# wolny/pytorch-3dunet

Measured on AMD Instinct MI355X. Metric: volumetric patches/sec (fwd+bwd), UNet3D f_maps=32 patch 64x128x128, higher is better.
Workload: dtype f32

## Files before the change

### include/u3d.h

```cpp
#ifndef U3D_H
#define U3D_H

#include <stddef.h>
#include <stdint.h>

#ifdef __cplusplus
extern "C" {
#endif

#define U3D_VERSION 128

#define U3D_OK 0
#define U3D_EINVAL (-1)
#define U3D_EHIP (-2)
#define U3D_EARCH (-3)
#define U3D_EWORKSPACE (-4)

typedef void* u3d_stream_t;

typedef struct {
    const float* p0;
    const float* p1;
    const int32_t* zmap;
    const int32_t* ymap;
// ... 6 lines not shown
int u3d_version(void);
const char* u3d_last_error(void);
int u3d_check_device(int device);
int u3d_set_tuning(int key, int value);
int u3d_set_profile_buffer(void* device_buffer, size_t bytes);
int u3d_debug_stream_pass(int device, u3d_stream_t stream, float* buf, long long n, int blocks, int passes, double min_seconds);
int u3d_debug_mfma_f32_rate(int device, u3d_stream_t stream, float* sink, int iters, int mode, double* flop_out);

size_t u3d_packed_weight_floats(int Cin, int Cout, int mode);
int u3d_pack_weights(int device, u3d_stream_t stream, const float* w, int Cout, int Cin, int mode, float* packed);
typedef struct {
    const float* w;
    float* packed;
    int64_t first;
    int32_t Cout, Cin, mode, cin_stride;
} u3d_pack_desc_t;
int u3d_pack_weights_batch(int device, u3d_stream_t stream, const u3d_pack_desc_t* descs_device, int n,
                           int64_t total_floats);
long long u3d_pack_weights_cells_blocks(const float* w, int Cin, int Cout, int mode, int cin_stride);
int u3d_pack_weights_batch_cells(int device, u3d_stream_t stream, const u3d_pack_desc_t* descs_device, int n, long long total_blocks);

int u3d_conv3d(int device, u3d_stream_t stream, const u3d_src_t* src, const float* packed_w, float* out,
               int N, int D, int H, int W, int Cout, int relu, double* out_stats, const u3d_src_t* gx,
               double* gstats);

int u3d_conv3d_residual(int device, u3d_stream_t stream, const u3d_src_t* src, const float* packed_w, float* out,
                        int N, int D, int H, int W, int Cout, int relu, double* out_stats, const float* residual);

long long u3d_conv3d_workspace_floats(int N, int D, int H, int W, int Cin, int Cout);
int u3d_conv3d_ex(int device, u3d_stream_t stream, const u3d_src_t* src, const float* packed_w, float* out, int N,
                  int D, int H, int W, int Cout, int relu, double* out_stats, const u3d_src_t* gx, double* gstats,
                  const float* residual, float* workspace, long long workspace_floats);

int u3d_conv3d_ex_reps(int device, u3d_stream_t stream, const u3d_src_t* src, const float* packed_w, float* out, int N,
                       int D, int H, int W, int Cout, int relu, double* out_stats, const u3d_src_t* gx, double* gstats,
                       const float* residual, float* workspace, long long workspace_floats, int stat_reps);

long long u3d_subpixel_packed_floats(int C1, int Cout);
long long u3d_subpixel_dgrad_packed_floats(int Cout, int C1);
int u3d_pack_subpixel_dgrad_weights(int device, u3d_stream_t stream, const float* w, int Cout, int Cin_total, int c_off,
                                    int C1, float* packed);
int u3d_subpixel_conv_dgrad(int device, u3d_stream_t stream, const float* dz, const float* packed, const float* x_low,
                            float* dlow, double* gstats, int N, int D1, int H1, int W1, int C1, int Cout);
int u3d_subpixel_conv_dgrad_reps(int device, u3d_stream_t stream, const float* dz, const float* packed, const float* x_low, float* dlow,
                                 double* gstats, int N, int D1, int H1, int W1, int C1, int Cout, int reps);
int u3d_pack_subpixel_weights(int device, u3d_stream_t stream, const float* w, int Cout, int Cin_total, int c_off, int C1,
                              float* packed);
long long u3d_subpixel_fwd_workspace_floats(int N, int D1, int H1, int W1, int C1, int Cout);
int u3d_subpixel_conv_fwd(int device, u3d_stream_t stream, const float* low, const float* affine,
                          long long affine_sample_stride, const float* packed, float* out, int N, int D1, int H1, int W1,
                          int C1, int Cout, float* workspace, long long workspace_floats);

size_t u3d_wgrad_workspace_floats(int N, int D, int H, int W, int Cin, int Cout);
int u3d_conv3d_wgrad(int device, u3d_stream_t stream, const u3d_src_t* src, const float* dz, float* dw, int N,
                     int D, int H, int W, int Cout, float* workspace, size_t workspace_floats);

int u3d_conv3d_variant(int N, int D, int H, int W, int Cin, int Cout, int src_kind, int has_workspace);
int u3d_conv3d_wgrad_variant(int N, int D, int H, int W, int Cin, int Cout, int src_kind);

int u3d_conv3d_wgrad_strided(int device, u3d_stream_t stream, const u3d_src_t* src, const float* dz, float* dw,
                             int dw_cin_stride, int N, int D, int H, int W, int Cout, float* workspace,
                             size_t workspace_floats);

typedef struct u3d_gn_bwd_job {
    const double* gstats_lo;
    const double* gstats_hi;
    const float* mean_rstd;
    const float* gamma;
    float* dgamma;
    float* dbeta;
    float* coef;
    float* coef_hi;
    double count;
    int32_t C0, C1, N, G;
    float hi_scale;
    int32_t reps_lo;
    int32_t reps_hi;
    int32_t reserved;
} u3d_gn_bwd_job_t;
int u3d_conv3d_wgrad_job_supported(int N, int C, int G);
int u3d_conv3d_wgrad_job(int device, u3d_stream_t stream, const u3d_src_t* src, const float* dz, float* dw, int dw_cin_stride,
                         int N, int D, int H, int W, int Cout, float* workspace, size_t workspace_floats,
                         const u3d_gn_bwd_job_t* job);

long long u3d_subpixel_wgrad_workspace_floats(int N, int D1, int H1, int W1, int C1, int Cout);
int u3d_subpixel_conv_wgrad(int device, u3d_stream_t stream, const float* low, const float* affine,
                            long long affine_sample_stride, const float* dz, float* dw, int dw_cin_stride, int N, int D1,
                            int H1, int W1, int C1, int Cout, float* workspace, long long workspace_floats);

int u3d_subpixel_conv_fwd_win(int device, u3d_stream_t stream, const float* low, const float* affine, long long affine_sample_stride,
                              const float* packed, float* out, int N, int D1, int H1, int W1, int C1, int Cout, const int* win);
int u3d_subpixel_conv_dgrad_win(int device, u3d_stream_t stream, const float* dz, const float* packed, const float* x_low, float* dlow,
                                double* gstats, int N, int D1, int H1, int W1, int C1, int Cout, const int* win);
int u3d_subpixel_conv_wgrad_win(int device, u3d_stream_t stream, const float* low, const float* affine, long long affine_sample_stride,
                                const float* dz, float* dw, int dw_cin_stride, int N, int D1, int H1, int W1, int C1, int Cout,
                                float* workspace, long long workspace_floats, const int* win);
int u3d_conv3d_box(int device, u3d_stream_t stream, const u3d_src_t* src, const float* packed_w, float* out, int N, int D, int H, int W,
                   int Cout, const int* out_box, const int* in_mask);
int u3d_conv3d_wgrad_box(int device, u3d_stream_t stream, const u3d_src_t* src, const float* dz, float* dw, int N, int D, int H, int W,
                         int Cout, float* workspace, size_t workspace_floats, const int* box);
int u3d_gn_bwd_apply_children(int device, u3d_stream_t stream, const float* dlow, const float* x, const float* coef, int Ctot, int coff,
                              int N, int D1, int H1, int W1, int C, int ez, int ey, int ex, int relu_mask, float* out);
int u3d_chan_stats_children(int device, u3d_stream_t stream, const float* x_low, int N, int D1, int H1, int W1, int C, int ez, int ey,
                            int ex, double* stats);
int u3d_nearest_childsum_add(int device, u3d_stream_t stream, const float* dv, const float* x_low, float* dlow, double* gstats, int N,
                             int D, int H, int W, int D1, int H1, int W1, int C, const int32_t* zlo, const int32_t* ylo,
                             const int32_t* xlo, int cz, int cy, int cx);

int u3d_conv3d_small_cin_fwd(int device, u3d_stream_t stream, const float* x, const float* affine, const float* w,
                             float* out, int N, int D, int H, int W, int Cin, int Cout, int relu, double* out_stats);
int u3d_conv3d_small_cin_fwd_reps(int device, u3d_stream_t stream, const float* x, const float* affine, const float* w, float* out, int N,
                                  int D, int H, int W, int Cin, int Cout, int relu, double* out_stats, int reps);
size_t u3d_small_cin_bwd_workspace_floats(int N, int D, int H, int W, int Cin, int Cout);
int u3d_conv3d_small_cin_bwd(int device, u3d_stream_t stream, const float* x, const float* affine, const float* dz,
                             const float* w, float* dw, double* gstats, int N, int D, int H, int W, int Cin, int Cout,
                             float* workspace, size_t workspace_floats);

int u3d_conv3d_naive(int device, u3d_stream_t stream, const u3d_src_t* src, const float* w, float* out, int N,
                     int D, int H, int W, int Cin, int Cout, int relu, int flip);

int u3d_chan_stats(int device, u3d_stream_t stream, const u3d_src_t* src, int N, int D, int H, int W,
                   double* stats);
int u3d_chan_stats_reps(int device, u3d_stream_t stream, const u3d_src_t* src, int N, int D, int H, int W, double* stats, int reps);
int u3d_gn_finalize(int device, u3d_stream_t stream, const double* stats0, int C0, double scale0,
                    const double* stats1, int C1, double scale1, int N, int G, double count, const float* gamma,
                    const float* beta, float eps, float* affine, float* mean_rstd);

int u3d_gn_bwd_finalize(int device, u3d_stream_t stream, const double* gstats, const float* mean_rstd,
                        const float* gamma, int N, int C, int G, double count, float* dgamma, float* dbeta,
                        float* coef);
int u3d_gn_finalize_split(int device, u3d_stream_t stream, const double* stats0, int C0, double scale0, const double* stats1, int C1,
                          double scale1, int N, int G, double count, const float* gamma, const float* beta, float eps, float* affine,
                          float* mean_rstd, int Csplit, float* affine_lo, float* affine_hi);
int u3d_gn_finalize_reps(int device, u3d_stream_t stream, const double* stats0, int C0, double scale0, int reps0, const double* stats1,
                         int C1, double scale1, int reps1, int N, int G, double count, const float* gamma, const float* beta, float eps,
                         float* affine, float* mean_rstd, int Csplit, float* affine_lo, float* affine_hi);
int u3d_gn_bwd_finalize_split_supported(int N, int C, int G);
int u3d_gn_bwd_finalize_split(int device, u3d_stream_t stream, const double* gstats_lo, int C0, const double* gstats_hi, int C1,
                              const float* mean_rstd, const float* gamma, int N, int G, double count, float* dgamma, float* dbeta,
                              float* coef, float hi_scale, float* coef_hi);

int u3d_gn_bwd_apply(int device, u3d_stream_t stream, const float* dg, int Cdg, int coff, const float* x, int Cx,
                     const float* coef, int Ctot, int64_t voxels_per_n, int N, int relu_mask, float* out);

int u3d_gn_bwd_apply_add(int device, u3d_stream_t stream, const float* dg, int Cdg, int coff, const float* x, int Cx,
                         const float* coef, int Ctot, int64_t voxels_per_n, int N, int relu_mask, const float* add,
                         float* out);

int u3d_gn_bwd_apply_up(int device, u3d_stream_t stream, const float* dg, int Cdg, int coff, const float* x1,
                        int C1, const float* coef, int Ctot, int N, int D, int H, int W, int D1, int H1, int W1,
                        const int32_t* zlo, const int32_t* ylo, const int32_t* xlo, int relu_mask, float* out);

int u3d_maxpool2_fwd(int device, u3d_stream_t stream, const float* x, int N, int D, int H, int W, int C,
                     float* out, uint8_t* argmax, double* out_stats);
int u3d_maxpool2_bwd_merge(int device, u3d_stream_t stream, const float* dg, const float* pooled,
                           const uint8_t* argmax, const float* coef, const float* skip_grad, const float* e,
                           int N, int D, int H, int W, int C, int relu_mask, float* out);
int u3d_maxpool2_bwd_merge_gn(int device, u3d_stream_t stream, const float* dg, const float* pooled,
                              const uint8_t* argmax, const float* coef, const float* skip_dg, int Cdg,
                              const float* skip_coef, int Ctot, const float* e, int N, int D, int H, int W, int C,
                              int relu_mask, float* out);

int u3d_conv1x1_head_fwd(int device, u3d_stream_t stream, const float* x, const float* w, const float* b, int N,
                         int64_t V, int Cin, int Cout, int act, float* logits, float* probs);
int u3d_conv1x1_head_bwd(int device, u3d_stream_t stream, const float* dlogits, const float* x, const float* w,
                         int N, int64_t V, int Cin, int Cout, int relu_mask, float* dx, double* acc);
// ... 316 lines not shown
```

### pytorch-3dunet_amd/csrc/u3d_bf16.hip

```cpp
#include "u3d_common.h"
#include "u3d_gn.h"
#include <type_traits>

typedef __bf16 bf16x8 __attribute__((ext_vector_type(8)));
typedef __bf16 bf16x4 __attribute__((ext_vector_type(4)));
typedef __bf16 bf16x2 __attribute__((ext_vector_type(2)));
typedef float f32x2 __attribute__((ext_vector_type(2)));
typedef unsigned u32x4 __attribute__((ext_vector_type(4)));
typedef unsigned u32x2 __attribute__((ext_vector_type(2)));

__device__ __forceinline__ bf16x8 u3d_stage_b16(const bf16x8& v, bool has_aff, bool ok, const f32x4& a0, const f32x4& b0, const f32x4& a1,
                                                const f32x4& b1) {
    const u32x4 raw = __builtin_bit_cast(u32x4, v);
    u32x4 o = raw;
    if (has_aff) {
#pragma unroll
        for (int e = 0; e < 4; ++e) {
            const f32x2 x = {__builtin_bit_cast(float, raw[e] << 16), __builtin_bit_cast(float, raw[e] & 0xffff0000u)};
            const f32x2 a = e < 2 ? f32x2{a0[2 * e], a0[2 * e + 1]} : f32x2{a1[2 * e - 4], a1[2 * e - 3]};
            const f32x2 b = e < 2 ? f32x2{b0[2 * e], b0[2 * e + 1]} : f32x2{b1[2 * e - 4], b1[2 * e - 3]};
            o[e] = __builtin_bit_cast(unsigned, __builtin_convertvector(__builtin_elementwise_fma(x, a, b), bf16x2));
        }
    }
    const unsigned m = ok ? 0xffffffffu : 0u;
    return __builtin_bit_cast(bf16x8, u32x4{o[0] & m, o[1] & m, o[2] & m, o[3] & m});
}

extern int g_u3d_tune[24];

namespace {

constexpr int HS = 12;

struct bf16_conv_params {
    const float* x;
    const float* affine;
    const bf16x8* wpk;
    float* y;
    const float* residual;
    const float* gx;
    double* out_stats;
    double* gstats;
    int N, D, H, W, C, K, relu;
    int tz, ty, tx;
    int off;
    const float* maskx;
    int ksplit;
    float* ws;
    long long wpart;
    int order;
    int b16;
    int t8mode, t8cs;
};

template <int ZW, int KS>
struct tile_geom {
    static constexpr bool FLAT = ZW == 3;
    static constexpr int TZ = FLAT ? 5 : 4 * ZW, TY = FLAT ? 10 : 8, TX = FLAT ? 10 : 8;
    static constexpr int HZ = TZ + KS - 1, HY = TY + KS - 1, HX = TX + KS - 1, MT = FLAT ? 4 : 2 * ZW;
    static_assert(HX <= HS, "halo rows are HS records long");
    static constexpr int NTAPS = KS * KS * KS;
    static constexpr int RING = KS == 3 ? 9 : 8;
    static constexpr int BDIST = 6;
    static constexpr int ADIST = 2;
    static constexpr int PLANE = HZ * HY * HS * 16 + 64;
    static constexpr int BUF = 2 * PLANE;
    static constexpr int ITEMS = HZ * HY * HX * 4;
    static constexpr int ITERS = (ITEMS + 255) / 256;
    static constexpr int NPARTS = KS * KS;
    static constexpr int PER_PART = (ITERS + NPARTS - 1) / NPARTS;
    static constexpr int ITEMS8 = HZ * HY * HX * 2;
    static constexpr int ITERS8 = (ITEMS8 + 255) / 256;
    static constexpr int PER_PART8 = (ITERS8 + NPARTS - 1) / NPARTS;
};

template <int NT, int ZW, int KS, typename T = float>
__device__ __forceinline__ void conv_tile_epilogue(const bf16_conv_params& p, f32x16 (&acc)[tile_geom<ZW, KS>::MT][NT], char* lds, int n, int nb,
                                                   int split, int z0, int y0, int x0, int t, int lane, int w) {
    using G = tile_geom<ZW, KS>;
    const int col = lane & 31, half = lane >> 5;
    if (p.ksplit > 1) {
        float* wsp = p.ws + (size_t)split * p.N * p.D * p.H * p.W * p.K;
        if constexpr (std::is_same<T, __bf16>::value) {
#pragma unroll
            for (int m = 0; m < G::MT; ++m) {
                int z, y, xx;
                bool row_ok = true;
                if constexpr (G::FLAT) {
                    const int v = (w * G::MT + m) * 32 + col, vz = v / (G::TY * G::TX), vr = v - vz * (G::TY * G::TX), vy = vr / G::TX;
                    z = z0 + vz, y = y0 + vy, xx = x0 + vr - vy * G::TX;
                    row_ok = v < G::TZ * G::TY * G::TX;
                } else {
                    z = z0 + w * ZW + (m >> 1), y = y0 + (m & 1) * 4 + (col & 3), xx = x0 + (col >> 2);
                }
                if (row_ok && z < p.D && y < p.H && xx < p.W) {
                    const size_t vox = (((size_t)n * p.D + z) * p.H + y) * p.W + xx;
#pragma unroll
                    for (int j = 0; j < NT; ++j)
#pragma unroll
                        for (int g = 0; g < 4; ++g)
                            *reinterpret_cast<f32x4*>(wsp + vox * p.K + (size_t)(nb * NT + j) * 32 + 8 * g + 4 * half) =
                                f32x4{acc[m][j][4 * g], acc[m][j][4 * g + 1], acc[m][j][4 * g + 2], acc[m][j][4 * g + 3]};
                }
            }
            return;
        }
        if constexpr (G::FLAT) return;
#pragma unroll
        for (int m = 0; m < G::MT; ++m) {
            const int z = z0 + w * ZW + (m >> 1);
#pragma unroll
// ... 2730 lines not shown
```

### pytorch-3dunet_amd/csrc/u3d_conv.hip

```cpp
#include <type_traits>
#include <utility>

#include "u3d_common.h"
#include "u3d_gn.h"
#include "u3d_subpix.h"

int g_u3d_tune[24] = {0};

namespace cv {
constexpr int TZ = 4, TY = 8, TX = 8;
constexpr int HZ = TZ + 2, HY = TY + 2, HX = TX + 2;
constexpr int CC = 16;
constexpr int CS = 16;
constexpr int RS = HX * CS + 4;
constexpr int PS = HY * RS;
constexpr int TILE_FLOATS = HZ * PS + 4;
constexpr int CNT_OFF = 2 * TILE_FLOATS;
constexpr int RED_OFF = CNT_OFF + 16;
constexpr int LDS_FLOATS = RED_OFF + 4 * 3 * 32 * 2;
constexpr int NITEMS = HZ * HY * HX * (CC / 4);
constexpr int NIT = (NITEMS + 255) / 256;
constexpr int NSTEP = 27 * (CC / 8);
constexpr int NSTEP_PAIRY = 36 * (CC / 8);
constexpr int NSTEP_N16 = 27;
constexpr int ST0 = 30;
constexpr int ISTORE = 5;
constexpr int PACK_PAD = 5;
static_assert(2 * (NIT - 1) < ST0 - 8 && ST0 + NIT <= NSTEP, "prefetch schedule must fit the k-loop");
}

struct ConvParams {
    u3d_src_t src;
    u3d_src_t gx;
    const float* wp;
    float* out;
    double* out_stats;
    double* gstats;
    const float* res;
    int N, D, H, W, Cout;
    int nchunks, ncb, ntot;
    int tz, ty, tx;
    int relu, vec, has_gx, ovec;
    int total;
    int gx_x2;
    int stagger;
    int stat_reps;
    int zfast;
    int ksplit, cps;
    long long part_stride;
    long long* dbg;
    int oz0, oy0, ox0, oz1, oy1, ox1;
    int mz, my, mx;
};

#define U3D_DBG_STAMP(slot)                                                   \
    do {                                                                      \
        if constexpr (DBG) {                                                  \
            if (l == 0) dbgw[slot] = (long long)__builtin_readcyclecounter(); \
        }                                                                     \
    } while (0)

__device__ __forceinline__ void u3d_flag_signal(int* c, int lane) {
    asm volatile("" ::: "memory");
    if (lane == 0) __hip_atomic_fetch_add(c, 1, __ATOMIC_RELAXED, __HIP_MEMORY_SCOPE_WORKGROUP);
    asm volatile("" ::: "memory");
}
__device__ __forceinline__ void u3d_flag_wait(int* c, int target) {
    while (__hip_atomic_load(c, __ATOMIC_RELAXED, __HIP_MEMORY_SCOPE_WORKGROUP) < target) __builtin_amdgcn_s_sleep(2);
    asm volatile("" ::: "memory");
}

template <int NT, bool VEC, bool DBG = false, int ABL = 0>
__global__ __launch_bounds__(256, 2) void conv3d_mfma_kernel(const ConvParams p) {
    using namespace cv;
    constexpr int RB = NT == 1 ? 6 : 3;
    extern __shared__ __attribute__((aligned(16))) float lds[];
    int* cnt = reinterpret_cast<int*>(lds + CNT_OFF);
    const int t = threadIdx.x;
    const int l = t & 63, w = t >> 6, m = l & 31, h = l >> 5;
    __builtin_amdgcn_s_setprio(3);
    long long* dbgw = nullptr;
    if constexpr (DBG) {
        dbgw = p.dbg + ((size_t)blockIdx.x * 4 + w) * 24;
        if (l == 0) {
            dbgw[0] = blockIdx.x;
            dbgw[1] = __builtin_amdgcn_s_getreg((31 << 11) | 4);
            dbgw[2] = __builtin_amdgcn_s_getreg((31 << 11) | 20);
            dbgw[7] = p.nchunks;
        }
    }
// ... 958 lines not shown
#pragma unroll
                            for (int e = 0; e < 4; ++e) val[e] = cok ? val[e] : 0.f;
                        }
                        q1 += val;
                        q2 += want_g ? val * xv[k] : val * val;
                    }
                }
                if (want_stats || want_g) {
                    if constexpr (CARRY) {
                        sq1 += q1;
                        sq2 += q2;
                    } else {
                        stat_reduce(q1, q2, n, nt, co - (PAIRY ? 0 : (cb * NT + nt) * 32));
                    }
                }
            }
        }
        if (ntiles == DBG_TILE) U3D_DBG_STAMP(22);
        ++ntiles;
        if (!has_next_tile || TN.n != T.n || TN.cb != T.cb) {
            if constexpr (CARRY) {
                if (want_stats || want_g) {
                    if constexpr (N16) {
#pragma unroll
                        for (int e = 0; e < 4; ++e) {
                            float a = sq1[e], b2 = sq2[e];
#pragma unroll
                            for (int msk = 8; msk > 0; msk >>= 1) {
                                a += __shfl_xor(a, msk);
                                b2 += __shfl_xor(b2, msk);
                            }
                            if (v16 == 0) {
                                double* r = &red[(((T.n & 1) * NT) * 32 + 4 * kq + e) * 2];
                                __hip_atomic_fetch_add(r, (double)a, __ATOMIC_RELAXED, __HIP_MEMORY_SCOPE_WORKGROUP);
                                __hip_atomic_fetch_add(r + 1, (double)b2, __ATOMIC_RELAXED, __HIP_MEMORY_SCOPE_WORKGROUP);
                            }
                        }
                    } else {
                        const int cq_ = (l >> 2) & 7;
                        stat_reduce(sq1, sq2, T.n, 0, PAIRY ? 4 * (cq_ & 3) : 4 * cq_);
                    }
                    sq1 = f32x4{0.f, 0.f, 0.f, 0.f};
                    sq2 = f32x4{0.f, 0.f, 0.f, 0.f};
                }
            }
            flush_stats(T.n, T.cb);
        }
        if (!has_next_tile) break;
        if constexpr (!ZEROC) {
#pragma unroll
            for (int mt = 0; mt < MT; ++mt)
#pragma unroll
                for (int nt = 0; nt < NT; ++nt)
#pragma unroll
                    for (int r = 0; r < 16; ++r) acc[mt][nt][r] = 0.f;
        }
        wi = nwi;
        dT = dTN;
        T = TN;
        wq = wqn;
    }
    if constexpr (DBG) {
        if (l == 0) dbgw[4] = ntiles;
    }
    U3D_DBG_STAMP(6);
}

namespace wg {
constexpr int TZ = 2, TY = 8, TX = 8;
constexpr int HZ = TZ + 2, HY = TY + 2, HX = TX + 2;
constexpr int CC = 32;
constexpr int CSg = 32, RSg = HX * CSg, PSg = HY * RSg;
constexpr int G_FLOATS = HZ * PSg;
constexpr int TV = TZ * TY * TX;
constexpr int DZ_FLOATS = TV * 32;
constexpr int DUMMY_OFF = G_FLOATS + DZ_FLOATS;
constexpr int BUF_FLOATS = G_FLOATS + DZ_FLOATS + 4;
constexpr int LDS_FLOATS = 2 * BUF_FLOATS;
constexpr int NTHR = 512;
constexpr int NITEMS_G = HZ * HY * HX * (CC / 4);
constexpr int NIT_G = (NITEMS_G + NTHR - 1) / NTHR;
constexpr int NIT_DZ = TV * 8 / NTHR;
constexpr int MAX_MAP_INTS = 4096;
}

struct WgradParams {
    u3d_src_t src;
    const float* dz;
    float* partial;
    int N, D, H, W, Cout;
    int nchunks, nkb, S;
    int tz, ty, tx, ntiles, tps;
    int vec, dzvec;
    int bz0, by0, bx0, bz1, by1, bx1;
};

template <bool VEC, bool REG = false, bool PAIR = false>
__global__ __launch_bounds__(512, 2) void conv3d_wgrad_kernel(const WgradParams p) {
    using namespace wg;
    constexpr int NA = PAIR ? 4 : 7;
    extern __shared__ __attribute__((aligned(16))) float lds[];
    int* zmapl = reinterpret_cast<int*>(lds + 2 * BUF_FLOATS);
    __builtin_amdgcn_s_setprio(3);
    const int t = threadIdx.x;
    const int l = t & 63, i = l & 31, h = l >> 5;
    const int w = __builtin_amdgcn_readfirstlane(t >> 6);
    const int tg = w & 3, hf = w >> 2;

    const int logical = u3d_xcd_remap(blockIdx.x, gridDim.x);
    const int kb = logical % p.nkb;
    const int chunk = (logical / p.nkb) % p.nchunks;
    const int s = logical / (p.nkb * p.nchunks);
    const int D = p.D, H = p.H, W = p.W;
    const int Ctot = p.src.C0 + p.src.C1;
    int* ymapl = zmapl + D;
    int* xmapl = ymapl + H;
    if (p.src.C1 > 0) {
        for (int k = t; k < D; k += NTHR) zmapl[k] = p.src.zmap[k];
        for (int k = t; k < H; k += NTHR) ymapl[k] = p.src.ymap[k];
        for (int k = t; k < W; k += NTHR) xmapl[k] = p.src.xmap[k];
        __syncthreads();
    }

    f32x16 acc[NA];
#pragma unroll
    for (int k = 0; k < NA; ++k)
#pragma unroll
        for (int r = 0; r < 16; ++r) acc[k][r] = 0.f;

    const int q = t & 7, tv = t >> 3;
    const int cq = chunk * CC + 4 * q;
    const int co = kb * 32 + 4 * q;
    const bool cok = cq < Ctot, from0 = cq < p.src.C0, dcok = co < p.Cout;
    const float* gbase = !cok ? p.src.p0 : (from0 ? p.src.p0 + cq : p.src.p1 + (cq - p.src.C0));
    const int Cs = (from0 || !cok) ? p.src.C0 : p.src.C1;
    const float* dzbase = p.dz + (dcok ? co : 0);

    constexpr int NPFC = NIT_G + NIT_DZ;
    int rel[NPFC], loff[NPFC];
    unsigned fz0 = 0, fz1 = 0, fy0 = 0, fy1 = 0, fx0 = 0, fx1 = 0, fdead = 0;
    if constexpr (REG) {
        const int vz = D % TZ ? D % TZ : TZ, vy = H % TY ? H % TY : TY, vx = W % TX ? W % TX : TX;
#pragma unroll
        for (int it = 0; it < NIT_G; ++it) {
            const int vox = tv + 64 * it;
            const int hz = vox / (HY * HX);
            const int rem = vox - hz * (HY * HX);
            const int hy = rem / HX;
            const int hx = rem - hy * HX;
            const bool in = vox < HZ * HY * HX;
            rel[it] = from0 ? ((hz - 1) * H + (hy - 1)) * W + (hx - 1)
                            : (((hz - 1) >> 1) * p.src.H1 + ((hy - 1) >> 1)) * p.src.W1 + ((hx - 1) >> 1);
            loff[it] = in ? hz * PSg + hy * RSg + hx * CSg + 4 * q : DUMMY_OFF;
            fz0 |= (in && hz == 0 ? 1u : 0u) << it;
            fz1 |= (in && hz > vz ? 1u : 0u) << it;
            fy0 |= (in && hy == 0 ? 1u : 0u) << it;
            fy1 |= (in && hy > vy ? 1u : 0u) << it;
            fx0 |= (in && hx == 0 ? 1u : 0u) << it;
            fx1 |= (in && hx > vx ? 1u : 0u) << it;
            fdead |= (in && cok ? 0u : 1u) << it;
        }
#pragma unroll
        for (int it = 0; it < NIT_DZ; ++it) {
            const int vox = tv + 64 * it;
            rel[NIT_G + it] = ((vox >> 6) * H + ((vox >> 3) & 7)) * W + (vox & 7);
            loff[NIT_G + it] = G_FLOATS + vox * 32 + 4 * q;
            fz1 |= ((vox >> 6) >= vz ? 1u : 0u) << (NIT_G + it);
            fy1 |= (((vox >> 3) & 7) >= vy ? 1u : 0u) << (NIT_G + it);
            fx1 |= ((vox & 7) >= vx ? 1u : 0u) << (NIT_G + it);
        }
        fdead |= (dcok ? 0u : 3u) << NIT_G;
    }
    auto tile_invalid = [&](int z0, int y0, int x0) {
        unsigned inv = fdead;
        inv |= z0 == 0 ? fz0 : 0u;
        inv |= z0 + TZ >= D ? fz1 : 0u;
        inv |= y0 == 0 ? fy0 : 0u;
        inv |= y0 + TY >= H ? fy1 : 0u;
        inv |= x0 == 0 ? fx0 : 0u;
        inv |= x0 + TX >= W ? fx1 : 0u;
        return inv;
    };
// ... 76 lines not shown
            const float* ap = p.src.affine + ((size_t)n * Ctot + (cok ? cq : 0)) * 2;
            const f32x4 lo = *reinterpret_cast<const f32x4*>(ap);
            const f32x4 hi = *reinterpret_cast<const f32x4*>(ap + 4);
            ga = f32x4{lo[0], lo[2], hi[0], hi[2]};
            gb = f32x4{lo[1], lo[3], hi[1], hi[3]};
        }
    };
    auto pf_load = [&](const TileC& c, int k) {
        bool ok;
        int idx, off;
        if constexpr (REG) {
            ok = ((c.inv >> k) & 1u) == 0;
            if (k < NIT_G) return *reinterpret_cast<const f32x4*>(gbase + (size_t)(ok ? c.base + rel[k] : 0) * Cs);
            return *reinterpret_cast<const f32x4*>(dzbase + (size_t)(ok ? c.dzb + rel[k] : 0) * p.Cout);
        }
        if (k < NIT_G) {
            g_item(c, k, off, ok, idx);
            return *reinterpret_cast<const f32x4*>(gbase + (size_t)idx * Cs);
        }
        dz_item(c, k - NIT_G, ok, idx);
        return *reinterpret_cast<const f32x4*>(dzbase + (size_t)idx * p.Cout);
    };
    auto pf_store = [&](float* buf, const TileC& c, int k, f32x4 raw, const f32x4& ga, const f32x4& gb) {
        bool ok;
        int idx, off;
        if constexpr (REG) {
            ok = ((c.inv >> k) & 1u) == 0;
            f32x4 val = k < NIT_G ? raw * ga + gb : raw;
#pragma unroll
            for (int e = 0; e < 4; ++e) val[e] = ok ? val[e] : 0.f;
            *reinterpret_cast<f32x4*>(&buf[loff[k]]) = val;
            return;
        }
        if (k < NIT_G) {
            g_item(c, k, off, ok, idx);
            f32x4 val = raw * ga + gb;
#pragma unroll
            for (int e = 0; e < 4; ++e) val[e] = ok ? val[e] : 0.f;
            *reinterpret_cast<f32x4*>(&buf[off]) = val;
        } else {
            dz_item(c, k - NIT_G, ok, idx);
#pragma unroll
            for (int e = 0; e < 4; ++e) raw[e] = ok ? raw[e] : 0.f;
            *reinterpret_cast<f32x4*>(&buf[G_FLOATS + (tv + 64 * (k - NIT_G)) * 32 + 4 * q]) = raw;
        }
    };
    auto stage_scalar = [&](float* buf, const TileC& c) {
        f32x4 ga, gb;
        u3d_load_affine(p.src.affine, c.n, Ctot, cq, false, ga, gb);
#pragma unroll 1
        for (int it = 0; it < NIT_G; ++it) {
            const int vox = tv + 64 * it;
            if (vox >= HZ * HY * HX) continue;
            const int hz = vox / (HY * HX), rem = vox - hz * (HY * HX), hy = rem / HX, hx = rem - hy * HX;
            const int gz = c.z0 - 1 + hz, gy = c.y0 - 1 + hy, gxx = c.x0 - 1 + hx;
            f32x4 val = {0.f, 0.f, 0.f, 0.f};
            if (gz >= 0 && gz < D && gy >= 0 && gy < H && gxx >= 0 && gxx < W) {
                int v0, v1;
                u3d_vox_index(p.src, c.n, gz, gy, gxx, D, H, W, v0, v1);
                val = u3d_load_quad(p.src, v0, v1, cq, false) * ga + gb;
            }
            *reinterpret_cast<f32x4*>(&buf[hz * PSg + hy * RSg + hx * CSg + 4 * q]) = val;
        }
#pragma unroll 1
        for (int it = 0; it < NIT_DZ; ++it) {
            const int vox = tv + 64 * it;
            const int z = c.z0 + (vox >> 6), y = c.y0 + ((vox >> 3) & 7), x = c.x0 + (vox & 7);
            f32x4 val = {0.f, 0.f, 0.f, 0.f};
            if (z < p.bz1 && y < p.by1 && x < p.bx1) {
                const float* sp = p.dz + ((size_t)((c.n * D + z) * H + y) * W + x) * p.Cout + co;
#pragma unroll
                for (int e = 0; e < 4; ++e)
                    if (co + e < p.Cout) val[e] = sp[e];
            }
            *reinterpret_cast<f32x4*>(&buf[G_FLOATS + vox * 32 + 4 * q]) = val;
        }
    };

    constexpr int NPF = NIT_G + NIT_DZ;
    constexpr int ST0 = 20;
    static_assert(2 * (NPF - 1) < ST0 && ST0 + NPF <= 32, "prefetch schedule must fit the 32 groups of a tile");
    const int tile_begin = s * p.tps, tile_end = min(p.ntiles, (s + 1) * p.tps);

    TileIdx tix = tile_decode(tile_begin);
    if (tile_begin < tile_end) {
        const TileC c = tile_coords(tix);
        if constexpr (VEC) {
            f32x4 ga, gb;
            load_affine(c.n, ga, gb);
            f32x4 v[NPF];
#pragma unroll
            for (int k = 0; k < NPF; ++k) v[k] = pf_load(c, k);
#pragma unroll
            for (int k = 0; k < NPF; ++k) pf_store(lds, c, k, v[k], ga, gb);
        } else {
            stage_scalar(lds, c);
        }
    }
    __syncthreads();

    int abase[NA];
#pragma unroll
    for (int k = 0; k < NA; ++k) {
        const int tap = PAIR ? 2 * (tg + 4 * k) + (i >> 4) : tg + 4 * k;
        const int toff = tap < 27 ? (tap / 9) * PSg + ((tap / 3) % 3) * RSg + (tap % 3) * CSg : 0;
        abase[k] = (PAIR ? (i & 15) : i) + h * CSg + hf * PSg + toff;
    }
    int bbase = G_FLOATS + (hf * 64 + h) * 32 + i;
    int cur = 0;
    __builtin_amdgcn_s_setprio(0);

    f32x4 gan = {1.f, 1.f, 1.f, 1.f}, gbn = {0.f, 0.f, 0.f, 0.f};
    int n_aff = -1;
    for (int tile = tile_begin; tile < tile_end; ++tile) {
        const bool has_next = tile + 1 < tile_end;
        if (has_next) tix = tile_next(tix);
        const TileC cn = tile_coords(tix);
        float* nbuf = lds + (cur ^ 1) * BUF_FLOATS;
        f32x4 v[NPF];
        if constexpr (VEC) {
            if (cn.n != n_aff) {
                load_affine(cn.n, gan, gbn);
                n_aff = cn.n;
            }
        }
        const float* gl = lds + cur * BUF_FLOATS;

        float aop[2][NA], bop[2];
        bop[0] = gl[bbase];
#pragma unroll
        for (int k = 0; k < NA; ++k) aop[0][k] = gl[abase[k]];
#pragma unroll
        for (int g = 0; g < 32; ++g) {
            if constexpr (VEC) {
                if (g % 2 == 0 && g / 2 < NPF) v[g / 2] = pf_load(cn, g / 2);
                if (g >= ST0 && g - ST0 < NPF) pf_store(nbuf, cn, g - ST0, v[g - ST0], gan, gbn);
            }
            if (g + 1 < 32) {
                const int row = (g + 1) >> 2, tq = (g + 1) & 3;
                const int goff = row * RSg + 2 * tq * CSg;
                bop[(g + 1) & 1] = gl[bbase + (row * 8 + 2 * tq) * 32];
#pragma unroll
                for (int k = 0; k < NA; ++k) aop[(g + 1) & 1][k] = gl[abase[k] + goff];
            }
            __builtin_amdgcn_sched_barrier(0);
#pragma unroll
            for (int k = 0; k < NA; ++k) acc[k] = __builtin_amdgcn_mfma_f32_32x32x2f32(aop[g & 1][k], bop[g & 1], acc[k], 0, 0, 0);
            __builtin_amdgcn_sched_barrier(0);
        }
        if constexpr (!VEC) {
            if (has_next) stage_scalar(nbuf, cn);
        }
        __syncthreads();
        cur ^= 1;
    }

    __builtin_amdgcn_s_setprio(3);
    float* red = lds;
    if (hf == 1) {
#pragma unroll
        for (int k = 0; k < NA; ++k)
#pragma unroll
            for (int r = 0; r < 16; ++r) red[((tg * 7 + k) * 16 + r) * 64 + l] = acc[k][r];
    }
    __syncthreads();
    if (hf == 0) {
        float* dst = p.partial + ((size_t)((s * p.nchunks + chunk) * p.nkb + kb) * 27) * 1024;
#pragma unroll
        for (int k = 0; k < NA; ++k) {
#pragma unroll
            for (int r = 0; r < 16; ++r) {
                const int row = (r & 3) + 8 * (r >> 2) + 4 * h;
                const int tap = PAIR ? 2 * (tg + 4 * k) + (row >> 4) : tg + 4 * k;
                const int c = PAIR ? (row & 15) : row;
                if (tap < 27) dst[((size_t)tap * 32 + c) * 32 + i] = acc[k][r] + red[((tg * 7 + k) * 16 + r) * 64 + l];
            }
        }
    }
}

template <int G>
__global__ __launch_bounds__(256) void wgrad_reduce_kernel(const float* __restrict__ partial, float* __restrict__ dw,
                                                           int S, int nchunks, int nkb, int Cin, int Cout, int cstride,
                                                           int has_job, u3d_gn_bwd_job_t job) {
    __shared__ float red[4][64];
    if (has_job && blockIdx.x == 0) {
        extern __shared__ double shb[];
        u3d_gn_bwd_finalize_body(job.gstats_lo, job.mean_rstd, job.gamma, job.N, job.C0 + job.C1, job.G, job.count, 1, 1, job.dgamma,
                                 job.dbeta, job.coef, job.gstats_hi, job.C0, job.hi_scale, job.coef_hi, shb, job.reps_lo, job.reps_hi);
        return;
    }
    const long long total = (long long)Cin * 27 * Cout;
    const int lane = G == 1 ? (int)threadIdx.x : (int)(threadIdx.x & 63), grp = G == 1 ? 0 : (int)(threadIdx.x >> 6);
    const long long idx = (long long)(blockIdx.x - (has_job ? 1 : 0)) * (G == 1 ? 256 : 64) + lane;
    float sum = 0.f;
    int k = 0, tap = 0, c = 0;
    if (idx < total) {
        k = (int)(idx % Cout);
        const long long r = idx / Cout;
        tap = (int)(r % 27);
        c = (int)(r / 27);
        const int chunk = c >> 5, kb = k >> 5;
        const size_t off = ((size_t)(chunk * nkb + kb) * 27 + tap) * 1024 + (c & 31) * 32 + (k & 31);
        const size_t sstride = (size_t)nchunks * nkb * 27 * 1024;
        const int per = (S + G - 1) / G;
        const int s0 = grp * per, s1 = min(S, s0 + per);
        float a0 = 0.f, a1 = 0.f, a2 = 0.f, a3 = 0.f;
        int s = s0;
        for (; s + 3 < s1; s += 4) {
            a0 += partial[(size_t)s * sstride + off];
            a1 += partial[(size_t)(s + 1) * sstride + off];
            a2 += partial[(size_t)(s + 2) * sstride + off];
            a3 += partial[(size_t)(s + 3) * sstride + off];
        }
        for (; s < s1; ++s) a0 += partial[(size_t)s * sstride + off];
        sum = (a0 + a1) + (a2 + a3);
    }
    if constexpr (G == 1) {
        if (idx < total) dw[((size_t)k * cstride + c) * 27 + tap] = sum;
    } else {
        red[grp][lane] = sum;
        __syncthreads();
        if (grp == 0 && idx < total)
            dw[((size_t)k * cstride + c) * 27 + tap] = (red[0][lane] + red[1][lane]) + (red[2][lane] + red[3][lane]);
    }
}

__device__ __forceinline__ int pack_image_of(long long idx, int nchunks, int ntot, long long& id) {
    const long long std_total = ((long long)nchunks * cv::NSTEP + cv::PACK_PAD) * ntot * 256;
    const long long pair_total = ((long long)nchunks * cv::NSTEP_PAIRY + cv::PACK_PAD) * 256;
    if (idx < std_total) {
        id = idx;
        return 0;
    }
    if (idx < std_total + pair_total) {
        id = idx - std_total;
        return 1;
    }
    id = idx - std_total - pair_total;
    return 2;
// ... 257 lines not shown
            const int f = fq * (sp::NFRAG / PK_SUBQ) + (i >> 6), lane = i & 63;
            const int st = sp::frag_tab().st[f];
            const int kl = 8 * (st & 1) + 4 * (lane >> 5), nl = lane & 31;
            f32x4 v;
#pragma unroll
            for (int j = 0; j < 4; ++j) v[j] = sp::frag_value(row_of(nl, kl + j), f);
            out4[(((long long)ch * sp::NFRAG + f) * ntot + ntg) * 64 + lane] = v;
        }
    } else {
        for (int i = t; i < spd::NFRAG / PK_SUBQ * 64; i += 256) {
            const int f = fq * (spd::NFRAG / PK_SUBQ) + (i >> 6), lane = i & 63;
            const int kl = 8 * (f & 1) + 4 * (lane >> 5), nl = lane & 31;
            f32x4 v;
#pragma unroll
            for (int j = 0; j < 4; ++j) v[j] = spd::frag_value(row_of(nl, kl + j), f);
            out4[(((long long)ch * spd::NFRAG + f) * ntot + ntg) * 64 + lane] = v;
        }
    }
}

__global__ void conv3d_naive_kernel(const u3d_src_t src, const float* __restrict__ w, float* __restrict__ out,
                                    int N, int D, int H, int W, int Cin, int Cout, int relu, int flip) {
    const long long total = (long long)N * D * H * W * Cout;
    for (long long idx = (long long)blockIdx.x * blockDim.x + threadIdx.x; idx < total;
         idx += (long long)gridDim.x * blockDim.x) {
        const int co = (int)(idx % Cout);
        long long v = idx / Cout;
        const int x = (int)(v % W);
        v /= W;
        const int y = (int)(v % H);
        v /= H;
        const int z = (int)(v % D);
        const int n = (int)(v / D);
        float sum = 0.f;
        for (int tap = 0; tap < 27; ++tap) {
            const int zz = z + tap / 9 - 1, yy = y + (tap / 3) % 3 - 1, xx = x + tap % 3 - 1;
            if (zz < 0 || zz >= D || yy < 0 || yy >= H || xx < 0 || xx >= W) continue;
            int v0, v1;
            u3d_vox_index(src, n, zz, yy, xx, D, H, W, v0, v1);
            for (int c = 0; c < Cin; ++c) {
                float g = u3d_load_elem(src, v0, v1, c);
                if (src.affine) {
                    const float* ab = src.affine + ((size_t)n * Cin + c) * 2;
                    g = g * ab[0] + ab[1];
                }
                const float wt = flip ? w[((size_t)c * Cout + co) * 27 + (26 - tap)] : w[((size_t)co * Cin + c) * 27 + tap];
                sum += g * wt;
            }
        }
        if (relu) sum = fmaxf(sum, 0.f);
        out[idx] = sum;
    }
}

static inline int cdiv(int a, int b) { return (a + b - 1) / b; }

static bool src_vec_ok(const u3d_src_t* s) {
    if (s->C0 % 4 != 0 || s->C1 % 4 != 0) return false;
    if (((uintptr_t)s->p0 & 15) != 0) return false;
    if (s->C1 > 0 && ((uintptr_t)s->p1 & 15) != 0) return false;
    if (s->affine && ((uintptr_t)s->affine & 15) != 0) return false;
    return true;
}

static int check_src(const u3d_src_t* s, const char* what) {
    U3D_REQUIRE(s != nullptr && s->p0 != nullptr && (s->C0 > 0 || s->C1 > 0) && s->C0 >= 0, "%s: null source", what);
    U3D_REQUIRE(s->C1 >= 0, "%s: negative C1", what);
    if (s->C1 > 0)
        U3D_REQUIRE(s->p1 && s->zmap && s->ymap && s->xmap && s->D1 > 0 && s->H1 > 0 && s->W1 > 0,
                    "%s: low-res source needs p1, index maps and dims", what);
    return 0;
}

static long long* g_u3d_prof_buf = nullptr;
static size_t g_u3d_prof_records = 0;

extern "C" int u3d_set_profile_buffer(void* device_buffer, size_t bytes) {
    g_u3d_prof_buf = static_cast<long long*>(device_buffer);
    g_u3d_prof_records = device_buffer ? bytes / (24 * sizeof(long long)) : 0;
    return 0;
}

extern "C" int u3d_set_tuning(int key, int value) {
    if (key < 0 || key >= 24) return u3d_set_err(U3D_EINVAL, "u3d_set_tuning: key out of range");
    g_u3d_tune[key] = value;
    return 0;
}

extern "C" size_t u3d_packed_weight_floats(int Cin, int Cout, int mode) {
    return (size_t)pack_total_floats(Cin, Cout, mode, nullptr, nullptr);
}

extern "C" int u3d_pack_weights(int device, u3d_stream_t stream, const float* w, int Cout, int Cin, int mode,
                                float* packed) {
    U3D_ENTER(device);
    U3D_REQUIRE(w && packed && Cout > 0 && Cin > 0 && (mode == 0 || mode == 1), "u3d_pack_weights: bad argument");
    int nchunks = 0, ntot = 0;
    const long long total = pack_total_floats(Cin, Cout, mode, &nchunks, &ntot);
    const int blocks = (int)((total + 255) / 256 > 4096 ? 4096 : (total + 255) / 256);
    hipLaunchKernelGGL(pack_weights_kernel, dim3(blocks), dim3(256), 0, (hipStream_t)stream, w, packed, Cout, Cin,
                       mode, nchunks, ntot, total);
    U3D_LAUNCH_CHECK();
    return 0;
}

extern "C" int u3d_pack_weights_batch(int device, u3d_stream_t stream, const u3d_pack_desc_t* descs_device, int n,
                                      int64_t total_floats) {
    U3D_ENTER(device);
    U3D_REQUIRE(descs_device && n > 0 && total_floats > 0, "u3d_pack_weights_batch: bad argument");
    U3D_REQUIRE(total_floats % 4 == 0, "u3d_pack_weights_batch: image sizes are multiples of 4 floats");
    long long blocks = (total_floats / 4 + 255) / 256;
    if (blocks > 8192) blocks = 8192;
    hipLaunchKernelGGL(pack_weights_batch_kernel, dim3((unsigned)blocks), dim3(256), 0, (hipStream_t)stream, descs_device, n,
                       (long long)total_floats);
    U3D_LAUNCH_CHECK();
    return 0;
}

extern "C" long long u3d_pack_weights_cells_blocks(const float* w, int Cin, int Cout, int mode, int cin_stride) {
    const int cs = cin_stride > 0 ? cin_stride : Cin;
    if (Cin <= 0 || Cout <= 0 || mode < 0 || mode > 3 || Cin % 4 != 0 || Cout % 4 != 0 || cs % 4 != 0 || ((uintptr_t)w & 15) != 0) return 0;
    return pack_cells_of(Cin, Cout, mode) + 1;
}

extern "C" int u3d_pack_weights_batch_cells(int device, u3d_stream_t stream, const u3d_pack_desc_t* descs_device, int n,
                                            long long total_blocks) {
    U3D_ENTER(device);
    U3D_REQUIRE(descs_device && n > 0 && total_blocks > 0 && total_blocks < 0x7fffffffLL, "u3d_pack_weights_batch_cells: bad argument");
    hipLaunchKernelGGL(pack_weights_cells_kernel, dim3((unsigned)total_blocks), dim3(256), 0, (hipStream_t)stream, descs_device, n);
    U3D_LAUNCH_CHECK();
    return 0;
}

static int device_cu_count(int device, int* out) {
    static int cached[64] = {0};
    if (device >= 0 && device < 64 && cached[device] > 0) {
        *out = cached[device];
        return 0;
    }
    int n = 0;
    U3D_HIP(hipDeviceGetAttribute(&n, hipDeviceAttributeMultiprocessorCount, device));
    if (n <= 0) n = 256;
    if (device >= 0 && device < 64) cached[device] = n;
    *out = n;
    return 0;
}

template <int NT>
static int conv_set_lds_nt() {
    const int bytes = cv::LDS_FLOATS * sizeof(float);
    U3D_HIP(hipFuncSetAttribute(reinterpret_cast<const void*>(conv3d_mfma_reg_kernel<NT, false, false>),
                                hipFuncAttributeMaxDynamicSharedMemorySize, bytes));
    U3D_HIP(hipFuncSetAttribute(reinterpret_cast<const void*>(conv3d_mfma_reg_kernel<NT, true, false>),
                                hipFuncAttributeMaxDynamicSharedMemorySize, bytes));
    U3D_HIP(hipFuncSetAttribute(reinterpret_cast<const void*>(conv3d_mfma_reg_kernel<NT, false, true>),
                                hipFuncAttributeMaxDynamicSharedMemorySize, bytes));
    U3D_HIP(hipFuncSetAttribute(reinterpret_cast<const void*>(conv3d_mfma_reg_kernel<NT, true, true>),
                                hipFuncAttributeMaxDynamicSharedMemorySize, bytes));
    U3D_HIP(hipFuncSetAttribute(reinterpret_cast<const void*>(conv3d_mfma_reg_kernel<NT, false, false, false, false>),
                                hipFuncAttributeMaxDynamicSharedMemorySize, bytes));
    U3D_HIP(hipFuncSetAttribute(reinterpret_cast<const void*>(conv3d_mfma_reg_kernel<NT, true, false, false, true, false, true>),
                                hipFuncAttributeMaxDynamicSharedMemorySize, bytes));
    U3D_HIP(hipFuncSetAttribute(reinterpret_cast<const void*>(conv3d_mfma_reg_kernel<NT, false, false, false, false, false, true>),
                                hipFuncAttributeMaxDynamicSharedMemorySize, bytes));
    U3D_HIP(hipFuncSetAttribute(reinterpret_cast<const void*>(conv3d_mfma_reg_kernel<NT, false, false, false, true, false, true>),
                                hipFuncAttributeMaxDynamicSharedMemorySize, bytes));
    if (NT == 1) {
// ... 290 lines not shown
        else                                                                                               \
            hipLaunchKernelGGL((conv3d_mfma_reg_kernel<NT_, false, false>), rgrid, rblock, shmem, st, p);  \
    } while (0)
        if (nt == 3)
            U3D_REG_LAUNCH(3);
        else if (nt == 2)
            U3D_REG_LAUNCH(2);
        else
            U3D_REG_LAUNCH(1);
#undef U3D_REG_LAUNCH
        U3D_LAUNCH_CHECK();
        return 0;
    }
    const bool vec = p.vec != 0;
    const dim3 grid((unsigned)nblk), block(256);
    p.dbg = (vec && g_u3d_prof_buf && (size_t)nblk * 4 <= g_u3d_prof_records) ? g_u3d_prof_buf : nullptr;
#define U3D_CONV_LAUNCH(NT_)                                                                     \
    do {                                                                                         \
        if (p.dbg && NT_ == 1 && g_u3d_tune[2] == 1)                                             \
            hipLaunchKernelGGL((conv3d_mfma_kernel<1, true, true, 1>), grid, block, shmem, st, p); \
        else if (p.dbg && NT_ == 1 && g_u3d_tune[2] == 2)                                        \
            hipLaunchKernelGGL((conv3d_mfma_kernel<1, true, true, 2>), grid, block, shmem, st, p); \
        else if (p.dbg && NT_ == 1 && g_u3d_tune[2] == 3)                                        \
            hipLaunchKernelGGL((conv3d_mfma_kernel<1, true, true, 3>), grid, block, shmem, st, p); \
        else if (p.dbg && NT_ == 1 && g_u3d_tune[2] == 7)                                        \
            hipLaunchKernelGGL((conv3d_mfma_kernel<1, true, true, 7>), grid, block, shmem, st, p); \
        else if (p.dbg)                                                                          \
            hipLaunchKernelGGL((conv3d_mfma_kernel<NT_, true, true>), grid, block, shmem, st, p); \
        else if (vec)                                                                            \
            hipLaunchKernelGGL((conv3d_mfma_kernel<NT_, true>), grid, block, shmem, st, p);      \
        else                                                                                     \
            hipLaunchKernelGGL((conv3d_mfma_kernel<NT_, false>), grid, block, shmem, st, p);     \
    } while (0)
    if (nt == 3)
        U3D_CONV_LAUNCH(3);
    else if (nt == 2)
        U3D_CONV_LAUNCH(2);
    else
        U3D_CONV_LAUNCH(1);
#undef U3D_CONV_LAUNCH
    U3D_LAUNCH_CHECK();
    return 0;
}

static void wgrad_plan(int N, int D, int H, int W, int Cin, int Cout, WgradParams& p) {
    p.nchunks = cdiv(Cin, 32);
    p.nkb = cdiv(Cout, 32);
    p.tz = cdiv(D, wg::TZ), p.ty = cdiv(H, wg::TY), p.tx = cdiv(W, wg::TX);
    p.ntiles = N * p.tz * p.ty * p.tx;
    const int pairs = p.nchunks * p.nkb;
    const int ncu = 256;
    long long best_cost = -1;
    int best_S = 1;
    for (int rounds = 1; rounds <= 8; ++rounds) {
        int S = (rounds * ncu) / pairs;
        if (S < 1) S = 1;
        if (S > p.ntiles) S = p.ntiles;
        const int tps = cdiv(p.ntiles, S);
        S = cdiv(p.ntiles, tps);
        const long long cost = (long long)cdiv(S * pairs, ncu) * (tps + 2);
        if (best_cost < 0 || cost < best_cost) {
            best_cost = cost;
            best_S = S;
        }
    }
    if (g_u3d_tune[1] > 0) best_S = g_u3d_tune[1] > p.ntiles ? p.ntiles : g_u3d_tune[1];
    p.tps = cdiv(p.ntiles, best_S);
    p.S = cdiv(p.ntiles, p.tps);
}

extern "C" size_t u3d_wgrad_workspace_floats(int N, int D, int H, int W, int Cin, int Cout) {
    WgradParams p;
    wgrad_plan(N, D, H, W, Cin, Cout, p);
    return (size_t)p.S * p.nchunks * p.nkb * 27 * 1024;
}

static int wgrad_set_lds_once(int device) {
    static bool done[64] = {false};
    if (device >= 0 && device < 64 && done[device]) return 0;
    U3D_HIP(hipFuncSetAttribute(reinterpret_cast<const void*>(conv3d_wgrad_kernel<true, true>),
                                hipFuncAttributeMaxDynamicSharedMemorySize, (wg::LDS_FLOATS + wg::MAX_MAP_INTS) * sizeof(float)));
    U3D_HIP(hipFuncSetAttribute(reinterpret_cast<const void*>(conv3d_wgrad_kernel<true, true, true>),
                                hipFuncAttributeMaxDynamicSharedMemorySize, (wg::LDS_FLOATS + wg::MAX_MAP_INTS) * sizeof(float)));
    U3D_HIP(hipFuncSetAttribute(reinterpret_cast<const void*>(conv3d_wgrad_kernel<true>),
                                hipFuncAttributeMaxDynamicSharedMemorySize, (wg::LDS_FLOATS + wg::MAX_MAP_INTS) * sizeof(float)));
    U3D_HIP(hipFuncSetAttribute(reinterpret_cast<const void*>(conv3d_wgrad_kernel<false>),
                                hipFuncAttributeMaxDynamicSharedMemorySize, (wg::LDS_FLOATS + wg::MAX_MAP_INTS) * sizeof(float)));
    if (device >= 0 && device < 64) done[device] = true;
    return 0;
}

static int conv3d_wgrad_impl(int device, u3d_stream_t stream, const u3d_src_t* src, const float* dz, float* dw, int cstride,
                             int N, int D, int H, int W, int Cout, float* workspace, size_t workspace_floats, const int* box = nullptr,
                             const u3d_gn_bwd_job_t* job = nullptr);

extern "C" int u3d_conv3d_wgrad_box(int device, u3d_stream_t stream, const u3d_src_t* src, const float* dz, float* dw, int N, int D,
                                    int H, int W, int Cout, float* workspace, size_t workspace_floats, const int* box) {
    U3D_REQUIRE(box != nullptr, "u3d_conv3d_wgrad_box: box is NULL");
    return conv3d_wgrad_impl(device, stream, src, dz, dw, 0, N, D, H, W, Cout, workspace, workspace_floats, box);
}

extern "C" int u3d_conv3d_wgrad(int device, u3d_stream_t stream, const u3d_src_t* src, const float* dz, float* dw,
                                int N, int D, int H, int W, int Cout, float* workspace, size_t workspace_floats) {
    return conv3d_wgrad_impl(device, stream, src, dz, dw, 0, N, D, H, W, Cout, workspace, workspace_floats);
}

extern "C" int u3d_conv3d_wgrad_strided(int device, u3d_stream_t stream, const u3d_src_t* src, const float* dz, float* dw,
                                        int dw_cin_stride, int N, int D, int H, int W, int Cout, float* workspace,
                                        size_t workspace_floats) {
    U3D_REQUIRE(src && dw_cin_stride >= src->C0 + src->C1, "u3d_conv3d_wgrad_strided: dw_cin_stride < channels of src");
    return conv3d_wgrad_impl(device, stream, src, dz, dw, dw_cin_stride, N, D, H, W, Cout, workspace, workspace_floats);
}

static size_t wgrad_job_lds_bytes(int N, int C, int G) { return sizeof(double) * (4 * (size_t)N * C + 2 * (size_t)N * G); }

extern "C" int u3d_conv3d_wgrad_job_supported(int N, int C, int G) {
    return (N > 0 && C > 0 && G > 0 && C % G == 0 && wgrad_job_lds_bytes(N, C, G) + 1024 <= 64 * 1024) ? 1 : 0;
}

extern "C" int u3d_conv3d_wgrad_job(int device, u3d_stream_t stream, const u3d_src_t* src, const float* dz, float* dw,
                                    int dw_cin_stride, int N, int D, int H, int W, int Cout, float* workspace,
                                    size_t workspace_floats, const u3d_gn_bwd_job_t* job) {
    U3D_REQUIRE(src && (dw_cin_stride == 0 || dw_cin_stride >= src->C0 + src->C1), "u3d_conv3d_wgrad_job: dw_cin_stride < channels of src");
    if (job) {
        U3D_REQUIRE(job->gstats_lo && job->mean_rstd && job->gamma && job->dgamma && job->dbeta && job->coef && job->C0 > 0 &&
                        job->C1 >= 0 && (job->C1 == 0) == (job->gstats_hi == nullptr) && (job->coef_hi == nullptr || job->C1 > 0) &&
                        job->reps_lo >= 0 && job->reps_lo <= 64 && job->reps_hi >= 0 && job->reps_hi <= 64,
                    "u3d_conv3d_wgrad_job: bad job");
        U3D_REQUIRE(u3d_conv3d_wgrad_job_supported(job->N, job->C0 + job->C1, job->G) == 1,
                    "u3d_conv3d_wgrad_job: the reduction of %d x %d channels in %d groups does not fit one block's LDS", job->N,
                    job->C0 + job->C1, job->G);
    }
    return conv3d_wgrad_impl(device, stream, src, dz, dw, dw_cin_stride, N, D, H, W, Cout, workspace, workspace_floats, nullptr, job);
}

static int conv3d_wgrad_impl(int device, u3d_stream_t stream, const u3d_src_t* src, const float* dz, float* dw, int cstride,
                             int N, int D, int H, int W, int Cout, float* workspace, size_t workspace_floats, const int* box,
                             const u3d_gn_bwd_job_t* job) {
    U3D_ENTER(device);
    if (int e = check_src(src, "u3d_conv3d_wgrad")) return e;
    U3D_REQUIRE(dz && dw && workspace && N > 0 && D > 0 && H > 0 && W > 0 && Cout > 0, "u3d_conv3d_wgrad: bad argument");
    U3D_REQUIRE((long long)N * D * H * W < (1ll << 31), "u3d_conv3d_wgrad: N*D*H*W must be < 2^31");
    WgradParams p;
    const int Cin = src->C0 + src->C1;
    p.bz0 = p.by0 = p.bx0 = 0, p.bz1 = D, p.by1 = H, p.bx1 = W;
    if (box) {
        U3D_REQUIRE(box[0] >= 0 && box[1] >= 0 && box[2] >= 0 && box[3] <= D && box[4] <= H && box[5] <= W && box[0] < box[3] &&
                        box[1] < box[4] && box[2] < box[5], "u3d_conv3d_wgrad_box: box outside the volume or empty");
        p.bz0 = box[0], p.by0 = box[1], p.bx0 = box[2], p.bz1 = box[3], p.by1 = box[4], p.bx1 = box[5];
    }
    wgrad_plan(N, p.bz1 - p.bz0, p.by1 - p.by0, p.bx1 - p.bx0, Cin, Cout, p);
    const size_t need = (size_t)p.S * p.nchunks * p.nkb * 27 * 1024;
    if (workspace_floats < need)
        return u3d_set_err(U3D_EWORKSPACE, "u3d_conv3d_wgrad: workspace %zu < %zu floats", workspace_floats, need);
    p.src = *src;
    p.dz = dz;
    p.partial = workspace;
    p.N = N, p.D = D, p.H = H, p.W = W, p.Cout = Cout;
    p.vec = src_vec_ok(src) ? 1 : 0;
    p.dzvec = (Cout % 4 == 0 && ((uintptr_t)dz & 15) == 0) ? 1 : 0;
    if (int e = wgrad_set_lds_once(device)) return e;
    const int nblk = p.S * p.nchunks * p.nkb;
    U3D_REQUIRE(D + H + W <= wg::MAX_MAP_INTS, "u3d_conv3d_wgrad: D+H+W must be <= %d", wg::MAX_MAP_INTS);
    const size_t shmem = (wg::LDS_FLOATS + (size_t)(D + H + W)) * sizeof(float);
    const bool reg = !box && (g_u3d_tune[3] != 2 || (D % wg::TZ == 0 && H % wg::TY == 0 && W % wg::TX == 0)) &&
                     (src->C1 == 0 || (D == 2 * src->D1 && H == 2 * src->H1 && W == 2 * src->W1));
    if (p.vec && p.dzvec && reg && Cin <= 16)
        hipLaunchKernelGGL((conv3d_wgrad_kernel<true, true, true>), dim3(nblk), dim3(wg::NTHR), shmem, (hipStream_t)stream, p);
    else if (p.vec && p.dzvec && reg)
        hipLaunchKernelGGL((conv3d_wgrad_kernel<true, true>), dim3(nblk), dim3(wg::NTHR), shmem, (hipStream_t)stream, p);
    else if (p.vec && p.dzvec)
        hipLaunchKernelGGL(conv3d_wgrad_kernel<true>, dim3(nblk), dim3(wg::NTHR), shmem, (hipStream_t)stream, p);
    else
        hipLaunchKernelGGL(conv3d_wgrad_kernel<false>, dim3(nblk), dim3(wg::NTHR), shmem, (hipStream_t)stream, p);
    U3D_LAUNCH_CHECK();
    const long long total = (long long)Cin * 27 * Cout;
    const bool one_group = p.S <= 16 && g_u3d_tune[23] != 1;
    const int rblocks = (int)((total + (one_group ? 255 : 63)) / (one_group ? 256 : 64));
    u3d_gn_bwd_job_t jb = {};
    size_t job_lds = 0;
    if (job) {
        jb = *job;
        if (!jb.gstats_hi) jb.C1 = 0, jb.hi_scale = 1.0f, jb.coef_hi = nullptr;
        if (jb.reps_lo < 1) jb.reps_lo = 1;
        if (jb.reps_hi < 1 || !jb.gstats_hi) jb.reps_hi = 1;
        job_lds = wgrad_job_lds_bytes(jb.N, jb.C0 + jb.C1, jb.G);
    }
    if (one_group)
        hipLaunchKernelGGL(wgrad_reduce_kernel<1>, dim3(rblocks + (job ? 1 : 0)), dim3(256), job_lds, (hipStream_t)stream, workspace, dw, p.S,
                           p.nchunks, p.nkb, Cin, Cout, cstride > 0 ? cstride : Cin, job ? 1 : 0, jb);
    else
        hipLaunchKernelGGL(wgrad_reduce_kernel<4>, dim3(rblocks + (job ? 1 : 0)), dim3(256), job_lds, (hipStream_t)stream, workspace, dw, p.S,
                           p.nchunks, p.nkb, Cin, Cout, cstride > 0 ? cstride : Cin, job ? 1 : 0, jb);
    U3D_LAUNCH_CHECK();
    return 0;
}

extern "C" int u3d_conv3d_variant(int N, int D, int H, int W, int Cin, int Cout, int src_kind, int has_workspace) {
    if (N <= 0 || D <= 0 || H <= 0 || W <= 0 || Cin <= 0 || Cout <= 0) return -1;
    if (Cin % 4 != 0 || Cout % 4 != 0) return 0;
    const long long ntiles = (long long)N * cdiv(D, cv::TZ) * cdiv(H, cv::TY) * cdiv(W, cv::TX);
    const int nchunks = cdiv(Cin, 16), ntot = cdiv(Cout, 32);
    if (has_workspace && splitk_shape(N, D, H, W, Cin, Cout) && g_u3d_tune[7] != 2) {
        if (splitk_count(g_u3d_ncu_seen, ntiles, ntot, nchunks, nullptr) >= 2) return 3;
    }
    const bool ragged = D % cv::TZ != 0 || H % cv::TY != 0 || W % cv::TX != 0;
    if (src_kind == 2 || g_u3d_tune[3] == 1 || (g_u3d_tune[3] == 2 && ragged)) return 0;
    return ragged ? 2 : 1;
}

extern "C" int u3d_conv3d_wgrad_variant(int N, int D, int H, int W, int Cin, int Cout, int src_kind) {
    if (N <= 0 || D <= 0 || H <= 0 || W <= 0 || Cin <= 0 || Cout <= 0) return -1;
    if (Cin % 4 != 0 || Cout % 4 != 0) return 0;
    const bool ragged = D % wg::TZ != 0 || H % wg::TY != 0 || W % wg::TX != 0;
    if (src_kind == 2 || (g_u3d_tune[3] == 2 && ragged)) return 0;
    return (ragged ? 2 : 1) | (Cin <= 16 ? 4 : 0);
}

extern "C" int u3d_conv3d_naive(int device, u3d_stream_t stream, const u3d_src_t* src, const float* w, float* out,
                                int N, int D, int H, int W, int Cin, int Cout, int relu, int flip) {
    U3D_ENTER(device);
    if (int e = check_src(src, "u3d_conv3d_naive")) return e;
    U3D_REQUIRE(w && out && Cin == src->C0 + src->C1, "u3d_conv3d_naive: bad argument");
    const long long total = (long long)N * D * H * W * Cout;
    const int blocks = (int)((total + 255) / 256 > 65536 ? 65536 : (total + 255) / 256);
    hipLaunchKernelGGL(conv3d_naive_kernel, dim3(blocks), dim3(256), 0, (hipStream_t)stream, *src, w, out, N, D, H,
                       W, Cin, Cout, relu, flip);
    U3D_LAUNCH_CHECK();
    return 0;
}
```

### pytorch-3dunet_amd/csrc/u3d_gn.h

```cpp
#pragma once
#include "u3d_common.h"

__device__ __forceinline__ double u3d_sum_replicas(const double* __restrict__ p, size_t stride, int reps) {
    double v = p[0];
    for (int r0 = 1; r0 < reps; r0 += 8) {
        double t[8];
#pragma unroll
        for (int j = 0; j < 8; ++j) t[j] = r0 + j < reps ? p[(size_t)(r0 + j) * stride] : 0.0;
#pragma unroll
        for (int j = 0; j < 8; ++j) v += t[j];
    }
    return v;
}

__device__ inline void u3d_gn_bwd_finalize_body(const double* __restrict__ gs, const float* __restrict__ mean_rstd,
                                                const float* __restrict__ gamma, int N, int C, int G, double count, int staged, int par,
                                                float* __restrict__ dgamma, float* __restrict__ dbeta, float* __restrict__ coef,
                                                const double* __restrict__ gs_hi, int C0, float hi_scale, float* __restrict__ coef_hi,
                                                double* shb, int reps = 1, int reps_hi = 1) {

#pragma clang fp contract(off)
    const double* src = gs;
    if (staged) {
        if (gs_hi) {
            const int C1 = C - C0;
            for (int i = threadIdx.x; i < N * C * 2; i += blockDim.x) {
                const int e = i & 1, nc = i >> 1, n = nc / C, c = nc - n * C;
                shb[i] = c < C0 ? u3d_sum_replicas(gs + ((size_t)n * C0 + c) * 2 + e, (size_t)N * C0 * 2, reps)
                                : u3d_sum_replicas(gs_hi + ((size_t)n * C1 + (c - C0)) * 2 + e, (size_t)N * C1 * 2, reps_hi);
            }
        } else {
            for (int i = threadIdx.x; i < N * C * 2; i += blockDim.x) shb[i] = u3d_sum_replicas(gs + i, (size_t)N * C * 2, reps);
        }
        __syncthreads();
        src = shb;
    }
    const int cpg = C / G;
    const double m = count * cpg;
    double* pa = shb + 2 * (size_t)N * C;
    double* pb = pa + (size_t)N * C;
    double* qr = pb + (size_t)N * C;
    if (par) {
        for (int i = threadIdx.x; i < N * C; i += blockDim.x) {
            const int n = i / C, c = i - n * C, g = c / cpg;
            const double mean = (double)mean_rstd[((size_t)n * G + g) * 2], rstd = (double)mean_rstd[((size_t)n * G + g) * 2 + 1];
            const double S1 = src[(size_t)i * 2], S2 = src[(size_t)i * 2 + 1], gm = (double)gamma[c];
            pa[i] = gm * S1;
            pb[i] = gm * rstd * (S2 - mean * S1);
        }
        __syncthreads();
    }
    for (int pair = threadIdx.x; pair < N * G; pair += blockDim.x) {
        const int n = pair / G, g = pair - n * G;
        const double mean = (double)mean_rstd[(size_t)pair * 2], rstd = (double)mean_rstd[(size_t)pair * 2 + 1];
        double A = 0.0, B = 0.0;
        for (int c = g * cpg; c < (g + 1) * cpg; ++c) {
            if (par) {
                A += pa[(size_t)n * C + c];
                B += pb[(size_t)n * C + c];
            } else {
                const double S1 = src[((size_t)n * C + c) * 2], S2 = src[((size_t)n * C + c) * 2 + 1];
                const double gm = (double)gamma[c];
                A += gm * S1;
                B += gm * rstd * (S2 - mean * S1);
            }
        }
        const double q = -rstd * rstd * B / m;
        const double r = -rstd * A / m + rstd * rstd * mean * B / m;
        if (par) {
            qr[(size_t)pair * 2] = q;
            qr[(size_t)pair * 2 + 1] = r;
        } else {
            for (int c = g * cpg; c < (g + 1) * cpg; ++c) {
                coef[((size_t)n * 3 + 0) * C + c] = (float)(rstd * (double)gamma[c]);
                coef[((size_t)n * 3 + 1) * C + c] = (float)q;
                coef[((size_t)n * 3 + 2) * C + c] = (float)r;
            }
        }
    }
    if (par) {
        __syncthreads();
        for (int i = threadIdx.x; i < N * C; i += blockDim.x) {
            const int n = i / C, c = i - n * C, pair = n * G + c / cpg;
            const double rstd = (double)mean_rstd[(size_t)pair * 2 + 1];
            const float fp = (float)(rstd * (double)gamma[c]), fq = (float)qr[(size_t)pair * 2], fr = (float)qr[(size_t)pair * 2 + 1];
            coef[((size_t)n * 3 + 0) * C + c] = fp;
            coef[((size_t)n * 3 + 1) * C + c] = fq;
            coef[((size_t)n * 3 + 2) * C + c] = fr;
            if (coef_hi && c >= C0) {
                const int C1 = C - C0;
                coef_hi[((size_t)n * 3 + 0) * C1 + (c - C0)] = fp;
                coef_hi[((size_t)n * 3 + 1) * C1 + (c - C0)] = fq * hi_scale;
                coef_hi[((size_t)n * 3 + 2) * C1 + (c - C0)] = fr * hi_scale;
            }
        }
    }
    for (int c = threadIdx.x; c < C; c += blockDim.x) {
        const int g = c / cpg;
        double dg = 0.0, db = 0.0;
        for (int n = 0; n < N; ++n) {
            const double mean = (double)mean_rstd[((size_t)n * G + g) * 2], rstd = (double)mean_rstd[((size_t)n * G + g) * 2 + 1];
            const double S1 = src[((size_t)n * C + c) * 2], S2 = src[((size_t)n * C + c) * 2 + 1];
            dg += rstd * (S2 - mean * S1);
            db += S1;
        }
        dgamma[c] = (float)dg;
        dbeta[c] = (float)db;
    }
}
```

### pytorch-3dunet_amd/csrc/u3d_ops.hip

```cpp
#include "u3d_common.h"
#include "u3d_gn.h"

#include <string.h>

extern int g_u3d_tune[24];

static thread_local char g_err[512] = "";

int u3d_set_err(int code, const char* fmt, ...) {
    va_list ap;
    va_start(ap, fmt);
    vsnprintf(g_err, sizeof(g_err), fmt, ap);
    va_end(ap);
    return code;
}

int u3d_device_guard::enter(int device) {
    hipError_t e = hipGetDevice(&prev);
    if (e != hipSuccess) return u3d_set_err(U3D_EHIP, "hipGetDevice failed: %s", hipGetErrorString(e));
    if (device >= 0 && prev != device) {
        e = hipSetDevice(device);
        if (e != hipSuccess) return u3d_set_err(U3D_EHIP, "hipSetDevice(%d) failed: %s", device, hipGetErrorString(e));
        switched = true;
    }
    return 0;
}

extern "C" int u3d_version(void) { return U3D_VERSION; }
extern "C" const char* u3d_last_error(void) { return g_err; }

extern "C" int u3d_check_device(int device) {
    hipDeviceProp_t prop;
    U3D_HIP(hipGetDeviceProperties(&prop, device));
    if (strncmp(prop.gcnArchName, "gfx950", 6) != 0)
        return u3d_set_err(U3D_EARCH, "device %d is %s, this library is built for gfx950 only", device, prop.gcnArchName);
    return 0;
}

__global__ __launch_bounds__(256) void debug_stream_pass_kernel(float* __restrict__ buf, long long n4, int passes, float one,
                                                               long long ticks_total) {
    f32x4* b = reinterpret_cast<f32x4*>(buf);
    constexpr long long PIECE = 4096;
    const long long npieces = (n4 + PIECE - 1) / PIECE;
    const long long mine = (npieces - blockIdx.x + gridDim.x - 1) / gridDim.x;
    const long long t0 = wall_clock64();
    long long done = 0;
    for (int p = 0; p < passes; ++p)
        for (long long pc = blockIdx.x; pc < npieces; pc += gridDim.x) {
            const long long lo = pc * PIECE, hi = lo + PIECE < n4 ? lo + PIECE : n4;
            for (long long i = lo + threadIdx.x; i < hi; i += 256) {
                f32x4 v = b[i];
                v *= one;
                b[i] = v;
            }
            ++done;
            if (ticks_total > 0) {
                const long long due = t0 + ticks_total * done / (mine * passes);
                while (wall_clock64() < due) __builtin_amdgcn_s_sleep(64);
            }
        }
}

extern "C" int u3d_debug_stream_pass(int device, u3d_stream_t stream, float* buf, long long n, int blocks, int passes,
                                     double min_seconds) {
    U3D_ENTER(device);
    U3D_REQUIRE(buf && n >= 4 && blocks > 0 && passes > 0 && min_seconds >= 0.0 && ((uintptr_t)buf & 15) == 0,
                "u3d_debug_stream_pass: bad argument");
    int khz = 0;
    U3D_HIP(hipDeviceGetAttribute(&khz, hipDeviceAttributeWallClockRate, device));
    const long long ticks = (long long)(min_seconds * 1e3 * (double)khz);
    hipLaunchKernelGGL(debug_stream_pass_kernel, dim3((unsigned)blocks), dim3(256), 0, (hipStream_t)stream, buf, n / 4, passes, 1.0f,
                       ticks);
    U3D_LAUNCH_CHECK();
    return 0;
}

__device__ __forceinline__ float dbg_hash_unit(unsigned x) {
    float s = 0.f;
    for (int i = 0; i < 4; ++i) {
        x ^= x >> 16, x *= 0x7feb352dU, x ^= x >> 15, x *= 0x846ca68bU, x ^= x >> 16;
        s += (float)(x & 0xffffff) * (1.0f / 16777216.0f);
    }
    return (s - 2.0f) * 1.7320508f;
}
__global__ __launch_bounds__(256) void debug_mfma_rate_kernel(float* __restrict__ sink, int iters, int mode) {
    f32x16 acc[2];
    for (int k = 0; k < 2; ++k)
        for (int r = 0; r < 16; ++r) acc[k][r] = 0.f;
// ... 324 lines not shown
}

extern "C" int u3d_gn_finalize_split(int device, u3d_stream_t stream, const double* stats0, int C0, double scale0,
                                     const double* stats1, int C1, double scale1, int N, int G, double count,
                                     const float* gamma, const float* beta, float eps, float* affine, float* mean_rstd,
                                     int Csplit, float* affine_lo, float* affine_hi) {
    return gn_finalize_impl(device, stream, stats0, C0, scale0, stats1, C1, scale1, N, G, count, gamma, beta, eps, affine, mean_rstd,
                            affine_lo, affine_hi, Csplit);
}

extern "C" int u3d_gn_finalize_reps(int device, u3d_stream_t stream, const double* stats0, int C0, double scale0, int reps0,
                                    const double* stats1, int C1, double scale1, int reps1, int N, int G, double count,
                                    const float* gamma, const float* beta, float eps, float* affine, float* mean_rstd,
                                    int Csplit, float* affine_lo, float* affine_hi) {
    return gn_finalize_impl(device, stream, stats0, C0, scale0, stats1, C1, scale1, N, G, count, gamma, beta, eps, affine, mean_rstd,
                            affine_lo, affine_hi, Csplit, reps0, reps1);
}

__global__ __launch_bounds__(256) void gn_bwd_finalize_kernel(const double* __restrict__ gs, const float* __restrict__ mean_rstd,
                                                              const float* __restrict__ gamma, int N, int C, int G,
                                                              double count, int staged, int par, float* __restrict__ dgamma,
                                                              float* __restrict__ dbeta, float* __restrict__ coef,
                                                              const double* __restrict__ gs_hi, int C0, float hi_scale,
                                                              float* __restrict__ coef_hi) {
    extern __shared__ double shb[];
    u3d_gn_bwd_finalize_body(gs, mean_rstd, gamma, N, C, G, count, staged, par, dgamma, dbeta, coef, gs_hi, C0, hi_scale, coef_hi, shb);
}

extern "C" int u3d_gn_bwd_finalize(int device, u3d_stream_t stream, const double* gstats, const float* mean_rstd,
                                   const float* gamma, int N, int C, int G, double count, float* dgamma,
                                   float* dbeta, float* coef) {
    U3D_ENTER(device);
    U3D_REQUIRE(gstats && mean_rstd && gamma && dgamma && dbeta && coef && N > 0 && C > 0 && G > 0 && C % G == 0,
                "u3d_gn_bwd_finalize: bad argument");
    const size_t bytes = sizeof(double) * 2 * (size_t)N * C;
    const int staged = bytes <= 48 * 1024 ? 1 : 0;
    const size_t par_bytes = 2 * bytes + sizeof(double) * 2 * (size_t)N * G;
    const int par = staged && par_bytes <= 64 * 1024 ? 1 : 0;
    hipLaunchKernelGGL(gn_bwd_finalize_kernel, dim3(1), dim3(256), par ? par_bytes : (staged ? bytes : 0), (hipStream_t)stream, gstats,
                       mean_rstd, gamma, N, C, G, count, staged, par, dgamma, dbeta, coef, (const double*)nullptr, C, 1.0f, (float*)nullptr);
    U3D_LAUNCH_CHECK();
    return 0;
}

extern "C" int u3d_gn_bwd_finalize_split_supported(int N, int C, int G) {
    const size_t bytes = sizeof(double) * 2 * (size_t)N * C;
    return (N > 0 && C > 0 && G > 0 && 2 * bytes + sizeof(double) * 2 * (size_t)N * G <= 64 * 1024) ? 1 : 0;
}

extern "C" int u3d_gn_bwd_finalize_split(int device, u3d_stream_t stream, const double* gstats_lo, int C0, const double* gstats_hi,
                                         int C1, const float* mean_rstd, const float* gamma, int N, int G, double count,
                                         float* dgamma, float* dbeta, float* coef, float hi_scale, float* coef_hi) {
    U3D_ENTER(device);
    const int C = C0 + C1;
    U3D_REQUIRE(gstats_lo && gstats_hi && mean_rstd && gamma && dgamma && dbeta && coef && N > 0 && C0 > 0 && C1 > 0 && G > 0 &&
                    C % G == 0, "u3d_gn_bwd_finalize_split: bad argument");
    U3D_REQUIRE(u3d_gn_bwd_finalize_split_supported(N, C, G) == 1, "u3d_gn_bwd_finalize_split: N * C = %d exceeds the staged path", N * C);
    const size_t bytes = sizeof(double) * 2 * (size_t)N * C;
    const size_t par_bytes = 2 * bytes + sizeof(double) * 2 * (size_t)N * G;
    hipLaunchKernelGGL(gn_bwd_finalize_kernel, dim3(1), dim3(256), par_bytes, (hipStream_t)stream, gstats_lo, mean_rstd, gamma, N, C, G,
                       count, 1, 1, dgamma, dbeta, coef, gstats_hi, C0, hi_scale, coef_hi);
    U3D_LAUNCH_CHECK();
    return 0;
}

template <bool VEC, typename T = float>
__global__ void gn_bwd_apply_kernel(const T* __restrict__ dg, int Cdg, int coff, const T* __restrict__ x,
                                    int Cx, const float* __restrict__ coef, int Ctot, long long Vn, int N,
                                    int relu_mask, const T* __restrict__ add, T* __restrict__ out) {
    if (VEC) {
        const int Q = Cx >> 2;
        const long long total = (long long)N * Vn * Q;
        for (long long idx = (long long)blockIdx.x * blockDim.x + threadIdx.x; idx < total;
             idx += (long long)gridDim.x * blockDim.x) {
            const int qd = (int)(idx % Q);
            const long long v = idx / Q;
            const int n = (int)(v / Vn);
            const int c = 4 * qd;
            const f32x4 d = u3d_ldq(dg + (size_t)v * Cdg + coff + c);
            const f32x4 xv = u3d_ldq(x + (size_t)v * Cx + c);
            const f32x4 p = *reinterpret_cast<const f32x4*>(coef + ((size_t)n * 3 + 0) * Ctot + coff + c);
            const f32x4 q = *reinterpret_cast<const f32x4*>(coef + ((size_t)n * 3 + 1) * Ctot + coff + c);
            const f32x4 r = *reinterpret_cast<const f32x4*>(coef + ((size_t)n * 3 + 2) * Ctot + coff + c);
            f32x4 o = p * d + q * xv + r;
            if (add) o += u3d_ldq(add + (size_t)v * Cx + c);
            if (relu_mask) {
#pragma unroll
                for (int e = 0; e < 4; ++e) o[e] = xv[e] > 0.f ? o[e] : 0.f;
            }
            u3d_stq(out + (size_t)v * Cx + c, o);
        }
    } else {
        const long long total = (long long)N * Vn * Cx;
        for (long long idx = (long long)blockIdx.x * blockDim.x + threadIdx.x; idx < total;
             idx += (long long)gridDim.x * blockDim.x) {
            const int c = (int)(idx % Cx);
            const long long v = idx / Cx;
            const int n = (int)(v / Vn);
            const float d = u3d_ld(dg + (size_t)v * Cdg + coff + c);
            const float xv = u3d_ld(x + idx);
            float o = coef[((size_t)n * 3 + 0) * Ctot + coff + c] * d + coef[((size_t)n * 3 + 1) * Ctot + coff + c] * xv +
                      coef[((size_t)n * 3 + 2) * Ctot + coff + c];
            if (add) o += u3d_ld(add + idx);
            if (relu_mask && !(xv > 0.f)) o = 0.f;
            u3d_st(out + idx, o);
        }
    }
}

__global__ __launch_bounds__(256) void gn_bwd_apply_oct_b16_kernel(const __bf16* __restrict__ dg, int Cdg, int coff,
                                                                   const __bf16* __restrict__ x, int Cx, const float* __restrict__ coef,
                                                                   int Ctot, long long Vn, int N, int relu_mask,
                                                                   const __bf16* __restrict__ add, __bf16* __restrict__ out) {
    typedef __bf16 b16x8 __attribute__((ext_vector_type(8)));
    const int Q = Cx >> 3;
    const long long total = (long long)N * Vn * Q;
    for (long long idx = (long long)blockIdx.x * blockDim.x + threadIdx.x; idx < total; idx += (long long)gridDim.x * blockDim.x) {
        const int qd = (int)(idx % Q);
        const long long v = idx / Q;
        const int n = (int)(v / Vn);
        const int c = 8 * qd;
        const b16x8 d8 = *reinterpret_cast<const b16x8*>(dg + (size_t)v * Cdg + coff + c);
        const b16x8 x8 = *reinterpret_cast<const b16x8*>(x + (size_t)v * Cx + c);
        b16x8 a8 = {};
        if (add) a8 = *reinterpret_cast<const b16x8*>(add + (size_t)v * Cx + c);
        const float* cp = coef + ((size_t)n * 3) * Ctot + coff + c;
        b16x8 o8;
#pragma unroll
        for (int hq = 0; hq < 2; ++hq) {
            const f32x4 p = *reinterpret_cast<const f32x4*>(cp + 4 * hq);
            const f32x4 q = *reinterpret_cast<const f32x4*>(cp + Ctot + 4 * hq);
            const f32x4 r = *reinterpret_cast<const f32x4*>(cp + 2 * (size_t)Ctot + 4 * hq);
#pragma unroll
            for (int e = 0; e < 4; ++e) {
                const float xv = (float)x8[4 * hq + e];
                float o = p[e] * (float)d8[4 * hq + e] + q[e] * xv + r[e];
                if (add) o += (float)a8[4 * hq + e];
                if (relu_mask) o = xv > 0.f ? o : 0.f;
                o8[4 * hq + e] = (__bf16)o;
            }
        }
        *reinterpret_cast<b16x8*>(out + (size_t)v * Cx + c) = o8;
    }
}

template <typename T>
static int gn_bwd_apply_impl(int device, u3d_stream_t stream, const T* dg, int Cdg, int coff, const T* x, int Cx,
                             const float* coef, int Ctot, int64_t voxels_per_n, int N, int relu_mask, const T* add,
                             T* out);

extern "C" int u3d_gn_bwd_apply(int device, u3d_stream_t stream, const float* dg, int Cdg, int coff, const float* x,
                                int Cx, const float* coef, int Ctot, int64_t voxels_per_n, int N, int relu_mask,
                                float* out) {
    return gn_bwd_apply_impl<float>(device, stream, dg, Cdg, coff, x, Cx, coef, Ctot, voxels_per_n, N, relu_mask, nullptr, out);
}

extern "C" int u3d_gn_bwd_apply_b16(int device, u3d_stream_t stream, const void* dg, int Cdg, int coff, const void* x, int Cx,
                                    const float* coef, int Ctot, int64_t voxels_per_n, int N, int relu_mask, const void* add,
                                    void* out) {
    return gn_bwd_apply_impl<__bf16>(device, stream, (const __bf16*)dg, Cdg, coff, (const __bf16*)x, Cx, coef, Ctot, voxels_per_n, N,
                                     relu_mask, (const __bf16*)add, (__bf16*)out);
}

extern "C" int u3d_gn_bwd_apply_add(int device, u3d_stream_t stream, const float* dg, int Cdg, int coff, const float* x,
                                    int Cx, const float* coef, int Ctot, int64_t voxels_per_n, int N, int relu_mask,
                                    const float* add, float* out) {
    if (add == nullptr) return u3d_set_err(U3D_EINVAL, "u3d_gn_bwd_apply_add: add is NULL");
    return gn_bwd_apply_impl<float>(device, stream, dg, Cdg, coff, x, Cx, coef, Ctot, voxels_per_n, N, relu_mask, add, out);
}

template <typename T>
static int gn_bwd_apply_impl(int device, u3d_stream_t stream, const T* dg, int Cdg, int coff, const T* x, int Cx,
                             const float* coef, int Ctot, int64_t voxels_per_n, int N, int relu_mask, const T* add,
// ... 1227 lines not shown
```

### pytorch-3dunet_amd/csrc/u3d_smallc.hip

```cpp
#include "u3d_common.h"

extern int g_u3d_tune[24];

typedef float f32x4s __attribute__((ext_vector_type(4)));

namespace sc {
constexpr int TZ = 4, TY = 8, TX = 8;
constexpr int HZ = 6, HY = 10, HX = 10;
constexpr int HV = HZ * HY * HX;
constexpr int MAXC = 4;
}

struct SmallFwdParams {
    const float* x;
    const float* affine;
    const float* w;
    float* out;
    double* out_stats;
    int N, D, H, W, Cin, Cout, relu;
    int tz, ty, tx, B;
    int reps;
};

template <int COUTP>
__global__ __launch_bounds__(256) void conv3d_small_fwd_kernel(const SmallFwdParams p) {
    using namespace sc;
    __shared__ __attribute__((aligned(16))) float xs[HV * MAXC];
    __shared__ __attribute__((aligned(16))) float ws[27 * MAXC * COUTP];
    __shared__ double sred[COUTP][2];
    const int t = threadIdx.x;
    const int n = blockIdx.y;
    const int Cin = p.Cin, D = p.D, H = p.H, W = p.W;
    for (int i = t; i < 27 * Cin * COUTP; i += 256) {
        const int k = i % COUTP;
        const int r = i / COUTP;
        const int c = r % Cin, tap = r / Cin;
        ws[i] = k < p.Cout ? p.w[((size_t)k * Cin + c) * 27 + tap] : 0.f;
    }
    if (t < COUTP) sred[t][0] = sred[t][1] = 0.0;
    float s1[COUTP], s2[COUTP];
#pragma unroll
    for (int k = 0; k < COUTP; ++k) s1[k] = s2[k] = 0.f;
    const int zl = t >> 6, yl = (t >> 3) & 7, xl = t & 7;
    const int ntiles = p.tz * p.ty * p.tx;
    for (int tile = blockIdx.x; tile < ntiles; tile += p.B) {
        int tt = tile;
        const int txi = tt % p.tx;
        tt /= p.tx;
        const int tyi = tt % p.ty;
        const int tzi = tt / p.ty;
        const int z0 = tzi * TZ, y0 = tyi * TY, x0 = txi * TX;
        __syncthreads();
        for (int i = t; i < HV * Cin; i += 256) {
            const int c = i % Cin;
            const int hv = i / Cin;
            const int hz = hv / (HY * HX), rem = hv - hz * (HY * HX), hy = rem / HX, hx = rem - hy * HX;
            const int gz = z0 - 1 + hz, gy = y0 - 1 + hy, gx = x0 - 1 + hx;
            float v = 0.f;
            if (gz >= 0 && gz < D && gy >= 0 && gy < H && gx >= 0 && gx < W) {
                v = p.x[((size_t)((n * D + gz) * H + gy) * W + gx) * Cin + c];
                if (p.affine) v = v * p.affine[((size_t)n * Cin + c) * 2] + p.affine[((size_t)n * Cin + c) * 2 + 1];
            }
            xs[hv * Cin + c] = v;
        }
        __syncthreads();
        float acc[COUTP];
#pragma unroll
        for (int k = 0; k < COUTP; ++k) acc[k] = 0.f;
        for (int tap = 0; tap < 27; ++tap) {
            const int hv = (zl + tap / 9) * (HY * HX) + (yl + (tap / 3) % 3) * HX + xl + tap % 3;
            for (int c = 0; c < Cin; ++c) {
                const float xv = xs[hv * Cin + c];
                const f32x4* wr = reinterpret_cast<const f32x4*>(&ws[(tap * Cin + c) * COUTP]);
#pragma unroll
                for (int k4 = 0; k4 < COUTP / 4; ++k4) {
                    const f32x4 wv = wr[k4];
#pragma unroll
                    for (int e = 0; e < 4; ++e) acc[4 * k4 + e] = fmaf(xv, wv[e], acc[4 * k4 + e]);
                }
            }
        }
        const int z = z0 + zl, y = y0 + yl, x = x0 + xl;
        if (z < D && y < H && x < W) {
            float* o = p.out + ((size_t)((n * D + z) * H + y) * W + x) * p.Cout;
#pragma unroll
// ... 563 lines not shown
```

### pytorch-3dunet_amd/csrc/u3d_subpix.hip

```cpp
#include "u3d_subpix.h"

extern int g_u3d_tune[24];


struct SubpixParams {
    const float* low;
    const float* affine;
    long long aff_nstride;
    const float* wp;
    float* out;
    int N, D1, H1, W1, C1, Cout, Do, Ho, Wo;
    int tz, ty, tx, nchunks, ncb;
    int ksplit, cps;
    long long part_stride;
    int oz, oy, ox;
};

__device__ __forceinline__ void sp_flag_signal(int* c, int lane) {
    asm volatile("" ::: "memory");
    if (lane == 0) __hip_atomic_fetch_add(c, 1, __ATOMIC_RELAXED, __HIP_MEMORY_SCOPE_WORKGROUP);
    asm volatile("" ::: "memory");
}
__device__ __forceinline__ void sp_flag_wait(int* c, int target) {
    while (__hip_atomic_load(c, __ATOMIC_RELAXED, __HIP_MEMORY_SCOPE_WORKGROUP) < target) __builtin_amdgcn_s_sleep(2);
    asm volatile("" ::: "memory");
}

template <class S>
__global__ __launch_bounds__(256, 2) void subpixel_fwd_kernel(const SubpixParams p) {
    using namespace sp;
    using SC = Sch<S>;
    constexpr int NFRAG = NFRAG_OF<S>, RING = S::RING, NACT = NACT_OF<S>;
    constexpr int LE = NACT >= 2 * NIT + 8 ? 2 : 1;
    constexpr int KS0 = NACT >= 40 ? 30 : NACT - NIT - 1;
    constexpr int KA = KS0 >= 6 ? KS0 - 6 : 0;
    static_assert(LE * (NIT - 1) < KS0 && KS0 + NIT <= NACT, "prefetch schedule must fit the k-loop");
    __shared__ __attribute__((aligned(16))) float lds[2 * TILE_FLOATS];
    __shared__ int cnt[16];
    const int t = threadIdx.x;
    const int l = t & 63, w = t >> 6, m = l & 31, h = l >> 5;
    __builtin_amdgcn_s_setprio(3);
    if (t < 16) cnt[t] = 0;
    __syncthreads();

    int logical = u3d_xcd_remap(blockIdx.x, gridDim.x);
    int ch0 = 0, nch = p.nchunks;
    float* const outp = p.out + (size_t)(p.ksplit > 1 ? logical % p.ksplit : 0) * p.part_stride;
    if (p.ksplit > 1) {
        ch0 = (logical % p.ksplit) * p.cps;
        nch = min(p.cps, p.nchunks - ch0);
        logical /= p.ksplit;
    }
    const int cb = logical % p.ncb;
    int tile = logical / p.ncb;
    const int txi = tile % p.tx;
    tile /= p.tx;
    const int tyi = tile % p.ty;
    tile /= p.ty;
    const int tzi = tile % p.tz;
    const int n = tile / p.tz;
    const int z0 = tzi * TZ, y0 = tyi * TY, x0 = txi * TX;
    const int D1 = p.D1, H1 = p.H1, W1 = p.W1, C1 = p.C1;

    int ldsoff[NIT], gv[NIT];
    const int q = t & 3;
#pragma unroll
    for (int it = 0; it < NIT; ++it) {
        const int item = t + 256 * it;
        const int vox = item >> 2;
        const bool in = item < NITEMS;
        const int hz = vox / (HY * HX);
        const int rem = vox - hz * (HY * HX);
        const int hy = rem / HX;
        const int hx = rem - hy * HX;
        ldsoff[it] = in ? hz * PS + hy * RS + hx * CS + 4 * q : HZ * PS;
        const int gz = z0 - 1 + hz, gy = y0 - 1 + hy, gx = x0 - 1 + hx;
        const bool ok = in && gz >= 0 && gz < D1 && gy >= 0 && gy < H1 && gx >= 0 && gx < W1;
        gv[it] = ok ? ((n * D1 + gz) * H1 + gy) * W1 + gx : -1;
    }

    f32x16 acc[8];
#pragma unroll
    for (int c = 0; c < 8; ++c)
#pragma unroll
        for (int r = 0; r < 16; ++r) acc[c][r] = 0.f;
// ... 961 lines not shown
```

### pytorch-3dunet_amd/pytorch3dunet_amd/_engine_conv.py

```python
from __future__ import annotations

import copy
import ctypes
import dataclasses
import os
import threading
from dataclasses import dataclass, field
from typing import List, Optional

import torch
import torch.nn.functional as F

from . import _native as nat
from ._native import U3DSrc

from ._engine_base import *
from ._engine_weights import Kind


class _SubLayers(dict):

    plus = frozenset()


@dataclass
class _ConvCall:
    dev: torch.device
    conv: torch.nn.Module
    src: VSrc
    affine: torch.Tensor
    y: torch.Tensor
    N: int
    D: int
    H: int
    W: int
    Ctot: int
    Cout: int
    relu: int
    stats: bool
    pool: _StatPool
    residual: Optional[torch.Tensor]
    sub: dict
    b16: bool
    affine_lo: Optional[torch.Tensor] = None
    affine_hi: Optional[torch.Tensor] = None

    def take_stats(self, reps: int = 1) -> Optional[StatTable]:
        return self.pool.table(self.N, self.Cout, reps) if self.stats else None

    @property
    def flops(self):
        return 54.0 * self.Ctot * self.Cout * self.N * self.D * self.H * self.W


@dataclass
class _BwdCall:
    cx: "_BwdCtx"
    rec: ConvRec
    dz: torch.Tensor
    src: VSrc
    N: int
    D: int
    H: int
    W: int
    Cout: int
    bf16: bool
    b16: bool
    job: object = None
    greps: int = 1

    @property
    def flops(self):
        return 54.0 * self.src.C * self.Cout * self.N * self.D * self.H * self.W


class ConvLayers:

    def _identity_affine(self, N, C, dev):
        key = ("ida", N, C, str(dev))
        t = self._const.get(key)
        if t is None:
            t = self._const[key] = torch.tensor([1.0, 0.0], dtype=_F32, device=dev).repeat(N, C, 1).contiguous()
        return t

    def _identity_coef(self, N, C, dev):
        key = ("idc", N, C, str(dev))
        t = self._const.get(key)
        if t is None:
            t = self._const[key] = torch.tensor([1.0, 0.0, 0.0], dtype=_F32, device=dev).view(1, 3, 1).repeat(N, 1, C).contiguous()
        return t

    def _unact(self, dev, g, y):
        if self.act in (ACT_LEAKY, ACT_ELU):
            nat.call("u3d_act_bwd", dev.index, _stream(dev), _p(g), _p(y), g.numel(), self.act, self.slope, _p(g))

    def _up_scale(self, dev):
        t = getattr(self, "_up_scale_t", None)
        if t is None or t.device != dev:
            t = self._up_scale_t = torch.tensor([1.0, 8.0, 8.0], dtype=_F32, device=dev).view(1, 3, 1)
        return t

    def _subpixel_layers(self, size):
        if not self.subpixel or getattr(self, "is2d", False) or any(ct is not None for ct in self.dec_up) or any(self.dec_interp):
            return _SubLayers()
        dims = [tuple(size)]
        for has_pool, _, _ in self.enc:
            if has_pool:
                dims.append(tuple(d // 2 for d in dims[-1]))
        out, plus = _SubLayers(), set()
        L = len(self.enc)
        for j, (c1, _) in enumerate(self.dec):
            skip_lvl, low_lvl = L - 2 - j, L - 1 - j
            if skip_lvl < 0 or low_lvl >= len(dims) or self._cat_bf16(c1):
                continue
            C0 = self.enc[skip_lvl][2].conv.out_channels
            C1 = c1.conv.in_channels - C0
            ratio = [a - 2 * b for a, b in zip(dims[skip_lvl], dims[low_lvl])]
            if (all(r in (0, 1) for r in ratio) and (self.subpixel_plus or not any(ratio)) and C0 > 0 and C1 > 0 and C0 % 4 == 0
                    and C1 % 4 == 0 and c1.conv.out_channels % 4 == 0):
                out[id(c1.conv.weight)] = (C0, C1)
                if any(ratio):
                    plus.add(id(c1.conv.weight))
        out.plus = frozenset(plus)
        return out

    def _stats_of(self, src: VSrc, st0: Optional[StatTable], st1: Optional[StatTable], pool: _StatPool, dev):
        if src.t1 is None:
            if st0 is None:
                st0 = pool.table(src.N, src.C0, self.stat_reps)
                s = src.struct()
                nat.call("u3d_chan_stats_reps", dev.index, _stream(dev), ctypes.byref(s), src.N, src.D, src.H, src.W, *_tab(st0))
            return st0, None
        if st0 is not None and st1 is not None and src.exact2x and self.fused_stats:
            return st0, dataclasses.replace(st1, scale=8.0)
        plus = src.plus
        if st0 is not None and plus is not None and any(plus) and self.fused_stats and src.C1 % 4 == 0 and src.t1.dtype == _F32:
            st1w = pool.table(src.N, src.C1)
            nat.call("u3d_chan_stats_children", dev.index, _stream(dev), _p(src.t1), src.N, src.D1, src.H1, src.W1, src.C1, *plus,
                     _p(st1w.t))
            return st0, st1w
        st = pool.table(src.N, src.C, self.stat_reps)
        s = src.struct()
        nat.call("u3d_chan_stats_reps", dev.index, _stream(dev), ctypes.byref(s), src.N, src.D, src.H, src.W, *_tab(st))
        return st, None

    def _norm_finalize(self, kind, mod, lo: StatTable, hi: Optional[StatTable], G, count, affine, dev, split=None):
        N, C0, sc0 = lo.N, lo.C, lo.scale
        C1, sc1 = (hi.C, hi.scale) if hi is not None else (0, 0.0)
        if kind == "g" and (lo.reps > 1 or (hi is not None and hi.reps > 1)):
            mean_rstd = _empty((N, G, 2), dtype=_F32, device=dev)
            sp = split if split is not None else (0, None, None)
            p1, r1 = _tab(hi)
            nat.call("u3d_gn_finalize_reps", dev.index, _stream(dev), _p(lo.t), C0, sc0, lo.reps, p1, C1, sc1, r1, N, G, count,
                     _p(mod.weight.detach()), _p(mod.bias.detach()), float(mod.eps), _p(affine), _p(mean_rstd), sp[0], _p(sp[1]), _p(sp[2]))
            return mean_rstd
        st0 = lo.folded().t
# ... 331 lines not shown
                        self._pindex[id(conv.weight)], small,
                        sub.get(id(conv.weight)) if (sub and src.t1 is not None and residual is None) else None,
                        not post, post_rec, spec.norm, bn_training, drop_rec, call.affine_lo, call.affine_hi)
            )
        return y, ystats

    _WGRAD_KERNELS = {
        "bf16": "_wgrad_bf16",
        "subpixel": "_wgrad_subpixel",
        "fp32_side": "_wgrad_fp32_side",
        "fp32": "_wgrad_fp32",
        "conv2d": "_wgrad_conv2d",
        "conv2d_bf16": "_wgrad_conv2d_bf16",
    }
    _DGRAD_KERNELS = {
        "subpixel": "_dgrad_subpixel",
        "f32s": "_dgrad_f32s",
        "bf16": "_dgrad_bf16",
        "fp32": "_dgrad_fp32",
        "conv2d": "_dgrad_conv2d",
        "conv2d_bf16": "_dgrad_conv2d_bf16",
    }

    def _wgrad_family(self, c: "_BwdCall") -> str:
        if getattr(self, "is2d", False):
            return "conv2d_bf16" if c.bf16 else "conv2d"
        if c.bf16 and c.Cout % 32 == 0:
            return "bf16"
        if c.rec.sub is not None:
            return "subpixel"
        if self.overlap_small_wgrad and c.N * c.D * c.H * c.W <= c.cx.SIDE_MAX_VOXELS and self.debug is None:
            return "fp32_side"
        return "fp32"

    def _dgrad_family(self, c: "_BwdCall") -> str:
        if getattr(self, "is2d", False):
            return "conv2d_bf16" if c.bf16 else "conv2d"
        if c.rec.sub is not None:
            return "subpixel"
        if c.src.t1 is None and not c.rec.small and self._split_dgrad(c.src.C, c.Cout):
            return "f32s"
        return "bf16" if c.bf16 else "fp32"

    def _wgrad_bf16(self, c: "_BwdCall"):
        cx, dev, src, rec = c.cx, c.cx.dev, c.src, c.rec
        need = nat.get_lib().u3d_wgrad_bf16_workspace_floats(c.N, c.D, c.H, c.W, src.C, c.Cout)
        ws = cx.ensure_ws(need)
        dw = cx.gview(rec.idx_w)
        job = c.job
        if job is not None and nat.get_lib().u3d_conv3d_wgrad_bf16_job_supported(c.N, c.D, c.H, c.W, src.C, c.Cout, 1 if c.b16 else 0, _p(dw),
                                                                                  job.N, job.C0 + job.C1, job.G) != 1:
            job = None
        nat.call("u3d_conv3d_wgrad_bf16" + ("_b16" if c.b16 else "") + "_job", dev.index, _stream(dev), _p(src.t0), _p(rec.affine), _p(c.dz),
                 _p(dw), c.N, c.D, c.H, c.W, src.C, c.Cout, _p(ws), ws.numel(), ctypes.byref(job) if job is not None else None,
                 flops=c.flops)
        if job is not None:
            c.job = None

    def _wgrad_subpixel(self, c: "_BwdCall"):
        cx, dev, src, rec, ws = c.cx, c.cx.dev, c.src, c.rec, c.cx.ws
        C0, C1 = rec.sub
        Ct = src.C
        dwv = cx.gview(rec.idx_w)
        plus = src.plus
        if any(plus):
            win = (ctypes.c_int * 9)(c.D, c.H, c.W, *plus, *plus)
            nat.call("u3d_subpixel_conv_wgrad_win", dev.index, _stream(dev), _p(src.t1), _p(rec.affine.view(-1)[2 * C0:]), Ct * 2,
                     _p(c.dz), _p(dwv[C0 * 27:]), Ct, c.N, src.D1, src.H1, src.W1, C1, c.Cout, _p(ws), ws.numel(), win,
                     flops=128.0 * C1 * c.Cout * c.N * src.D1 * src.H1 * src.W1)
            s_up = src.up_only_struct(rec.affine_hi if rec.affine_hi is not None else rec.affine[:, C0:].contiguous())
            slice_view = dwv.view(c.Cout, Ct, 27)[:, C0:, :]
            for box in slab_boxes((c.D, c.H, c.W), plus, 2):
                tmp = _empty((c.Cout, C1, 27), dtype=_F32, device=dev)
                nat.call("u3d_conv3d_wgrad_box", dev.index, _stream(dev), ctypes.byref(s_up), _p(c.dz), _p(tmp), c.N, c.D, c.H, c.W,
                         c.Cout, _p(ws), ws.numel(), (ctypes.c_int * 6)(*box),
                         flops=54.0 * C1 * c.Cout * c.N * (box[3] - box[0]) * (box[4] - box[1]) * (box[5] - box[2]))
                slice_view += tmp
        else:
            nat.call("u3d_subpixel_conv_wgrad", dev.index, _stream(dev), _p(src.t1), _p(rec.affine.view(-1)[2 * C0:]), Ct * 2,
                     _p(c.dz), _p(dwv[C0 * 27:]), Ct, c.N, src.D1, src.H1, src.W1, C1, c.Cout, _p(ws), ws.numel(),
                     flops=128.0 * C1 * c.Cout * c.N * src.D1 * src.H1 * src.W1)
        a0 = rec.affine_lo if rec.affine_lo is not None else rec.affine[:, :C0].contiguous()
        s0 = VSrc(src.t0).struct(a0)
        nat.call("u3d_conv3d_wgrad_job", dev.index, _stream(dev), ctypes.byref(s0), _p(c.dz), _p(dwv), Ct, c.N, c.D, c.H, c.W,
                 c.Cout, _p(ws), ws.numel(), ctypes.byref(c.job) if c.job is not None else None,
                 flops=54.0 * C0 * c.Cout * c.N * c.D * c.H * c.W)
        c.job = None

    def _wgrad_fp32_side(self, c: "_BwdCall"):
        cx, dev, src, rec = c.cx, c.cx.dev, c.src, c.rec
        s_aff = src.struct(rec.affine)
        need = nat.get_lib().u3d_wgrad_workspace_floats(c.N, c.D, c.H, c.W, src.C, c.Cout)
        side = cx.side_stream(need)
        side.wait_stream(torch.cuda.current_stream(dev))
        with torch.cuda.stream(side):
            nat.call("u3d_conv3d_wgrad", dev.index, _stream(dev), ctypes.byref(s_aff), _p(c.dz), _p(cx.gview(rec.idx_w)), c.N,
                     c.D, c.H, c.W, c.Cout, _p(cx.ws_side), cx.ws_side.numel(), flops=c.flops)
        c.dz.record_stream(side)
        cx.side_used = True

    def _wgrad_fp32(self, c: "_BwdCall"):
        cx, dev, src, rec, ws = c.cx, c.cx.dev, c.src, c.rec, c.cx.ws
        s_aff = src.struct(rec.affine)
        nat.call("u3d_conv3d_wgrad_job", dev.index, _stream(dev), ctypes.byref(s_aff), _p(c.dz), _p(cx.gview(rec.idx_w)), 0, c.N, c.D,
                 c.H, c.W, c.Cout, _p(ws), ws.numel(), ctypes.byref(c.job) if c.job is not None else None, flops=c.flops)
        c.job = None

    def _dgrad_subpixel(self, c: "_BwdCall"):
        cx, dev, src, rec, ws, pool = c.cx, c.cx.dev, c.src, c.rec, c.cx.ws, c.cx.pool
        Nn, Dd, Hh, Ww, Cout = c.N, c.D, c.H, c.W, c.Cout
        C0, C1 = rec.sub
        w, pair = rec.conv_w, tuple(rec.sub)
        dg0 = _empty((Nn, Dd, Hh, Ww, C0), dtype=_F32, device=dev)
        dlow = _empty_like(src.t1)
        split0 = self._split_dgrad(C0, Cout)
        plus = src.plus
        gst0 = pool.table(Nn, C0, 1 if split0 else c.greps)
        gst1 = pool.table(Nn, C1, 1 if any(plus) else c.greps)
        if split0:
            need = nat.get_lib().u3d_conv3d_bf16_workspace_floats(Nn, Dd, Hh, Ww, Cout, C0)
            kws = cx.ensure_ws(need) if need > 0 else None
            nat.call("u3d_conv3d_f32s", dev.index, _stream(dev), _p(c.dz), None, _p(self.images.get(w, Kind.F32S_DGRAD, dev, pair)),
                     _p(dg0), Nn, Dd, Hh, Ww, Cout, C0, 0, None, _p(src.t0), _p(gst0.t), None, _p(kws), need,
                     flops=54.0 * C0 * Cout * Nn * Dd * Hh * Ww)
        else:
            s_dz = VSrc(c.dz).struct()
            s_x0 = VSrc(src.t0).struct()
            nat.call("u3d_conv3d_ex_reps", dev.index, _stream(dev), ctypes.byref(s_dz), _p(self.images.get(w, Kind.SKIP_DGRAD, dev, pair)), _p(dg0),
                     Nn, Dd, Hh, Ww, C0, 0, None, ctypes.byref(s_x0), _p(gst0.t), None, _p(ws), ws.numel(), gst0.reps,
                     flops=54.0 * C0 * Cout * Nn * Dd * Hh * Ww)
        plus = src.plus
        if any(plus):
            win = (ctypes.c_int * 9)(Dd, Hh, Ww, *plus, *plus)
            nat.call("u3d_subpixel_conv_dgrad_win", dev.index, _stream(dev), _p(c.dz), _p(self.images.get(w, Kind.UP_DGRAD, dev, pair)), _p(src.t1),
                     _p(dlow), _p(gst1.t), Nn, src.D1, src.H1, src.W1, C1, Cout, win,
                     flops=128.0 * C1 * Cout * Nn * src.D1 * src.H1 * src.W1)
            dv = _empty((Nn, Dd, Hh, Ww, C1), dtype=_F32, device=dev)
            s_dz2 = VSrc(c.dz).struct()
            wpd1 = self.images.get(w, Kind.SLAB_DGRAD, dev, pair)
            mask = (ctypes.c_int * 3)(*(2 * e for e in plus))
            for box in slab_boxes((Dd, Hh, Ww), plus, 3):
                nat.call("u3d_conv3d_box", dev.index, _stream(dev), ctypes.byref(s_dz2), _p(wpd1), _p(dv), Nn, Dd, Hh, Ww, C1,
                         (ctypes.c_int * 6)(*box), mask,
                         flops=54.0 * C1 * Cout * Nn * (box[3] - box[0]) * (box[4] - box[1]) * (box[5] - box[2]))
            lz, ly, lx = src.los
            nat.call("u3d_nearest_childsum_add", dev.index, _stream(dev), _p(dv), _p(src.t1), _p(dlow), _p(gst1.t), Nn, Dd, Hh, Ww,
                     src.D1, src.H1, src.W1, C1, _p(lz), _p(ly), _p(lx), *plus)
            del dv
        else:
            nat.call("u3d_subpixel_conv_dgrad_reps", dev.index, _stream(dev), _p(c.dz), _p(self.images.get(w, Kind.UP_DGRAD, dev, pair)), _p(src.t1),
                     _p(dlow), _p(gst1.t), Nn, src.D1, src.H1, src.W1, C1, Cout, gst1.reps,
                     flops=128.0 * C1 * Cout * Nn * src.D1 * src.H1 * src.W1)
        return (dg0, dlow), (gst0, gst1)

    def _dgrad_f32s(self, c: "_BwdCall"):
        cx, dev, src, rec = c.cx, c.cx.dev, c.src, c.rec
        dg = _empty((c.N, c.D, c.H, c.W, src.C), dtype=_F32, device=dev)
        gst = cx.pool.table(c.N, src.C)
        need = nat.get_lib().u3d_conv3d_bf16_workspace_floats(c.N, c.D, c.H, c.W, c.Cout, src.C)
        kws = cx.ensure_ws(need) if need > 0 else None
        nat.call("u3d_conv3d_f32s", dev.index, _stream(dev), _p(c.dz), None, _p(self.images.get(rec.conv_w, Kind.F32S_DGRAD, dev)), _p(dg),
                 c.N, c.D, c.H, c.W, c.Cout, src.C, 0, None, _p(src.t0), _p(gst.t), None, _p(kws), need, flops=c.flops)
        return dg, (gst, None)

    def _dgrad_bf16(self, c: "_BwdCall"):
        cx, dev, src, rec = c.cx, c.cx.dev, c.src, c.rec
        dg = _empty((c.N, c.D, c.H, c.W, src.C), dtype=c.dz.dtype if c.b16 else _F32, device=dev)
        gst = cx.pool.table(c.N, src.C)
        need = nat.get_lib().u3d_conv3d_bf16_workspace_floats(c.N, c.D, c.H, c.W, c.Cout, src.C)
        kws = cx.ensure_ws(need) if need > 0 else None
        nat.call("u3d_conv3d_bf16_ex" + ("_b16" if c.b16 else ""), dev.index, _stream(dev), _p(c.dz), None,
                 _p(self.images.get(rec.conv_w, Kind.BF16_DGRAD, dev)), _p(dg), c.N, c.D, c.H, c.W, c.Cout, src.C, 0, None, _p(src.t0), _p(gst.t),
                 None, _p(kws), need, flops=c.flops)
        return dg, (gst, None)

    def _wgrad_conv2d(self, c: "_BwdCall"):
        cx, dev, src, rec, ws = c.cx, c.cx.dev, c.src, c.rec, c.cx.ws
        s_aff = src.struct(rec.affine)
        nat.call("u3d_conv2d_wgrad", dev.index, _stream(dev), ctypes.byref(s_aff), _p(c.dz), _p(cx.gview(rec.idx_w)), c.N, c.H, c.W,
                 c.Cout, _p(ws), ws.numel(), flops=18.0 * src.C * c.Cout * c.N * c.H * c.W)

    def _dgrad_conv2d(self, c: "_BwdCall"):
        cx, dev, src, rec, ws = c.cx, c.cx.dev, c.src, c.rec, c.cx.ws
        wpd = self.images.get(rec.conv_w, Kind.DGRAD2D, dev)
        dg = _empty((c.N, c.D, c.H, c.W, src.C), dtype=_F32, device=dev)
        gst = cx.pool.table(c.N, src.C, c.greps)
        s_dz = VSrc(c.dz).struct()
        s_x = src.struct()
        nat.call("u3d_conv2d_ex_reps", dev.index, _stream(dev), ctypes.byref(s_dz), _p(wpd), _p(dg), c.N, c.H, c.W, src.C, 0, None,
                 ctypes.byref(s_x), _p(gst.t), _p(ws), ws.numel(), gst.reps, flops=18.0 * src.C * c.Cout * c.N * c.H * c.W)
        return dg, (gst, None)

    def _wgrad_conv2d_bf16(self, c: "_BwdCall"):
        cx, dev, src, rec = c.cx, c.cx.dev, c.src, c.rec
        sfx = "_c16" if self._c16(src.C, c.Cout) else ""
        need = getattr(nat.get_lib(), f"u3d_wgrad2d_bf16{sfx}_workspace_floats")(c.N, c.H, c.W, src.C, c.Cout)
        ws = cx.ensure_ws(need)
        nat.call("u3d_conv2d_wgrad_bf16" + sfx, dev.index, _stream(dev), _p(src.t0), _p(rec.affine), _p(c.dz), _p(cx.gview(rec.idx_w)), c.N,
                 c.H, c.W, src.C, c.Cout, _p(ws), ws.numel(), flops=18.0 * src.C * c.Cout * c.N * c.H * c.W)

    def _dgrad_conv2d_bf16(self, c: "_BwdCall"):
        cx, dev, src, rec = c.cx, c.cx.dev, c.src, c.rec
        c16 = self._c16(src.C, c.Cout)
        sfx = "_c16" if c16 else ""
        wpd = self.images.get(rec.conv_w, Kind.BF16_DGRAD2D_C16 if c16 else Kind.BF16_DGRAD2D, dev)
        dg = _empty((c.N, c.D, c.H, c.W, src.C), dtype=_F32, device=dev)
        gst = cx.pool.table(c.N, src.C, c.greps)
        need = getattr(nat.get_lib(), f"u3d_conv2d_bf16{sfx}_workspace_floats")(c.N, c.H, c.W, c.Cout, src.C)
        kws = cx.ensure_ws(need) if need > 0 else None
        nat.call("u3d_conv2d_bf16" + sfx, dev.index, _stream(dev), _p(c.dz), None, _p(wpd), _p(dg), c.N, c.H, c.W, c.Cout, src.C, 0, None,
                 _p(src.t0), _p(gst.t), _p(kws), need, gst.reps, flops=18.0 * src.C * c.Cout * c.N * c.H * c.W)
        return dg, (gst, None)

    def _dgrad_fp32(self, c: "_BwdCall"):
        cx, dev, src, rec, ws = c.cx, c.cx.dev, c.src, c.rec, c.cx.ws
        wpd = self.images.get(rec.conv_w, Kind.DGRAD, dev)
        dg = _empty((c.N, c.D, c.H, c.W, src.C), dtype=_F32, device=dev)
        gst = cx.pool.table(c.N, src.C, c.greps)
        s_dz = VSrc(c.dz).struct()
        s_x = src.struct()
        nat.call("u3d_conv3d_ex_reps", dev.index, _stream(dev), ctypes.byref(s_dz), _p(wpd), _p(dg), c.N, c.D, c.H, c.W, src.C, 0, None,
                 ctypes.byref(s_x), _p(gst.t), None, _p(ws), ws.numel(), gst.reps, flops=c.flops)
        return dg, (gst, None)

    def _conv_bwd(self, cx, rec: ConvRec, dz_, need_dg=True):
        dev, pool, ws, gview = cx.dev, cx.pool, cx.ws, cx.gview
        src = rec.src
        Nn, Dd, Hh, Ww = src.N, src.D, src.H, src.W
        Cout = rec.y.shape[-1]
        if rec.drop is not None:
            kind, mask = rec.drop
            g = _empty_like(dz_)
            if kind == "d":
                nat.call("u3d_mul", dev.index, _stream(dev), _p(dz_), _p(mask), dz_.numel(), _p(g))
            else:
                nat.call("u3d_affine_act_fwd", dev.index, _stream(dev), _p(dz_), _p(mask), Nn, Dd * Hh * Ww, Cout, ACT_NONE, 0.0, _p(g))
            dz_ = g
        if rec.post is not None:
            z, _, inner, islope = rec.post
            Vz = Dd * Hh * Ww
            gst2 = pool.table(Nn, Cout)
            nat.call("u3d_pair_stats", dev.index, _stream(dev), _p(dz_), _p(z), Nn, Vz, Cout, _p(gst2.t))
            if rec.norm is None:
                nat.call("u3d_bias_grad", dev.index, _stream(dev), _p(gst2.t), Nn, Cout, _p(gview(rec.idx_gb)))
            else:
                coef2 = _empty((Nn, 3, Cout), dtype=_F32, device=dev)
                self._norm_bwd_finalize(cx, rec, (gst2, None), float(Vz), coef2)
                dz_ = self._plain_apply(cx, dz_, coef2, z, 1 if inner == ACT_RELU else 0)
                if inner in (ACT_LEAKY, ACT_ELU):
                    nat.call("u3d_act_bwd", dev.index, _stream(dev), _p(dz_), _p(z), dz_.numel(), inner, islope, _p(dz_))
        if self.debug is not None:
            self.debug[rec.name + ".dz"] = dz_.clone()
        if rec.small and not need_dg:
            gst = pool.table(Nn, src.C)
            if getattr(self, "is2d", False):
                nat.call("u3d_conv2d_small_cin_bwd", dev.index, _stream(dev), _p(src.t0), _p(rec.affine), _p(dz_),
                         _p(rec.conv_w.detach()), _p(gview(rec.idx_w)), _p(gst.t), Nn, Hh, Ww, src.C, Cout, _p(ws), ws.numel(),
                         flops=2 * 18.0 * src.C * Cout * Nn * Hh * Ww)
            else:
                nat.call("u3d_conv3d_small_cin_bwd", dev.index, _stream(dev), _p(src.t0), _p(rec.affine), _p(dz_),
                         _p(rec.conv_w.detach()), _p(gview(rec.idx_w)), _p(gst.t), Nn, Dd, Hh, Ww, src.C, Cout, _p(ws), ws.numel(),
                         flops=2 * 54.0 * src.C * Cout * Nn * Dd * Hh * Ww)
            if not rec.pre_norm:
                return None, self._identity_coef(Nn, src.C, dev), None
            coef = _empty((Nn, 3, src.C), dtype=_F32, device=dev)
            return None, coef, self._norm_bwd_finalize(cx, rec, (gst, None), float(Dd * Hh * Ww), coef)
        bf16 = rec.sub is None and not rec.small and self._bf16_routed(src, Cout)
        b16 = src.t0.dtype == torch.bfloat16
        assert not b16 or (bf16 and Cout % 64 == 0 and dz_.dtype == torch.bfloat16)
        call = _BwdCall(cx, rec, dz_, src, Nn, Dd, Hh, Ww, Cout, bf16, b16)
        if (self.stat_reps > 1 and rec.pre_norm and rec.norm == "g" and self._wgrad_family(call) in ("fp32", "subpixel")
                and nat.get_lib().u3d_conv3d_wgrad_job_supported(Nn, src.C, rec.G) == 1):
            call.greps = self.stat_reps
        dg, gst = getattr(self, self._DGRAD_KERNELS[self._dgrad_family(call)])(call)
        if self.debug is not None and rec.sub is None:
            self.debug[rec.name + ".dg"] = dg.clone()
        coef = coef_hi = None
        if rec.pre_norm:
            coef = _empty((Nn, 3, src.C), dtype=_F32, device=dev)
            call.job, coef_hi = self._norm_bwd_job(cx, rec, gst, float(Dd * Hh * Ww), coef)
        had_job = call.job is not None
        getattr(self, self._WGRAD_KERNELS[self._wgrad_family(call)])(call)
        if not rec.pre_norm:
            return dg, self._identity_coef(Nn, src.C, dev), None
        if not had_job or call.job is not None:
            coef_hi = self._norm_bwd_finalize(cx, rec, gst, float(Dd * Hh * Ww), coef)
        return dg, coef, coef_hi

    def _plain_apply(self, cx, dg, coef, x, relu_mask, add=None):
        dev = cx.dev
        out = _empty_like(x)
        Nn = x.shape[0]
        C = x.shape[-1]
        if x.dtype == torch.bfloat16:
            nat.call("u3d_gn_bwd_apply_b16", dev.index, _stream(dev), _p(dg), C, 0, _p(x), C, _p(coef), C, x.numel() // (Nn * C), Nn,
                     relu_mask, _p(add), _p(out))
            return out
        if add is None:
            nat.call("u3d_gn_bwd_apply", dev.index, _stream(dev), _p(dg), C, 0, _p(x), C, _p(coef), C, x.numel() // (Nn * C), Nn,
                     relu_mask, _p(out))
        else:
            nat.call("u3d_gn_bwd_apply_add", dev.index, _stream(dev), _p(dg), C, 0, _p(x), C, _p(coef), C,
                     x.numel() // (Nn * C), Nn, relu_mask, _p(add), _p(out))
        return out

    def _wgrad_workspace(self, tape, dev):
        return _empty(max(self._wgrad_workspace_floats(tape.convs), 4), dtype=_F32, device=dev)

    def _layer_ws_floats(self, N, D, H, W, Cin, Cout, sub=None, small=False, virtual=False):
        lib = nat.get_lib()
        if getattr(self, "is2d", False):
            if small:
                return max(lib.u3d_small_cin2d_bwd_workspace_floats(N, H, W, Cin, Cout), lib.u3d_wgrad2d_workspace_floats(N, H, W, Cin, Cout),
                           lib.u3d_conv2d_workspace_floats(N, H, W, Cout, Cin))
            if self._bf16_routed_weight(Cin, Cout, virtual):
                sfx = "_c16" if self._c16(Cin, Cout) else ""
                return max(getattr(lib, f"u3d_wgrad2d_bf16{sfx}_workspace_floats")(N, H, W, Cin, Cout),
                           getattr(lib, f"u3d_conv2d_bf16{sfx}_workspace_floats")(N, H, W, Cout, Cin))
            return max(lib.u3d_wgrad2d_workspace_floats(N, H, W, Cin, Cout), lib.u3d_conv2d_workspace_floats(N, H, W, Cout, Cin))
        if small:
            return lib.u3d_small_cin_bwd_workspace_floats(N, D, H, W, Cin, Cout)
        if sub is not None:
            boxes = slab_boxes((D, H, W), (D % 2, H % 2, W % 2), 2)
            return max([lib.u3d_wgrad_workspace_floats(N, D, H, W, sub[0], Cout),
                        lib.u3d_subpixel_wgrad_workspace_floats(N, D // 2, H // 2, W // 2, sub[1], Cout),
                        lib.u3d_conv3d_workspace_floats(N, D, H, W, Cout, sub[0])] +
                       [lib.u3d_wgrad_workspace_floats(N, b[3] - b[0], b[4] - b[1], b[5] - b[2], sub[1], Cout) for b in boxes])
        if not virtual and self._bf16_layer(Cin, Cout):
            need = lib.u3d_conv3d_bf16_workspace_floats(N, D, H, W, Cout, Cin)
            wg = lib.u3d_wgrad_bf16_workspace_floats(N, D, H, W, Cin, Cout)
            return max(need, wg)
        return max(lib.u3d_wgrad_workspace_floats(N, D, H, W, Cin, Cout), lib.u3d_conv3d_workspace_floats(N, D, H, W, Cout, Cin))

    def _wgrad_workspace_floats(self, convs):
        need = 0
        for r in convs:
            need = max(need, self._layer_ws_floats(r.src.N, r.src.D, r.src.H, r.src.W, r.src.C, r.y.shape[-1], r.sub, r.small,
                                                   r.src.t1 is not None))
        return int(need)
```

### pytorch-3dunet_amd/pytorch3dunet_amd/_engine_unet.py

```python
from __future__ import annotations

import copy
import ctypes
import dataclasses
import os
import threading
from dataclasses import dataclass, field
from typing import List, Optional

import torch
import torch.nn.functional as F

from . import _native as nat
from ._native import U3DSrc

from ._engine_base import *
from ._engine_conv import ConvLayers
from ._engine_weights import Kind, WeightImages



class UNet3DEngine(ConvLayers):

    def __init__(self, model):
        self.model = model
        self.grad_sync = None
        self.debug = None
        self.fused_stats = True
        self.is2d = bool(getattr(model, "native_2d", False))
        self.stem = self.is2d and bool(getattr(model, "native_2d_stem", False))
        self.stat_reps = max(1, min(64, int(os.environ.get("U3D_STAT_REPS", "8"))))
        self.small_cin = True
        self.overlap_small_wgrad = True
        self.subpixel = os.environ.get("U3D_SUBPIXEL", "1") != "0" and not self.is2d
        self.subpixel_plus = os.environ.get("U3D_SUBPIXEL_PLUS", "1") != "0"
        self.bf16 = bool(getattr(model, "compute_bf16", False))
        self.bf16_deconv = self.is2d and self.bf16 and bool(getattr(model, "native_2d_residual_bf16_deconv", False))
        self.split = bool(getattr(model, "compute_split", False)) and not self.bf16
        self.checkpoint_encoders = bool(getattr(model, "checkpoint_encoders", False))
        self.checkpoint_levels = getattr(model, "checkpoint_levels", None)
        self.lean_tape = False
        self.act_bf16 = False
        self._lock = threading.RLock()
        self.hip_graph = bool(getattr(model, "hip_graph", False))
        self._graph_steps: dict = {}
        self._graph_off_reason = None
        self._placed = None
        self._const: dict = {}
        spec = parse_order(getattr(model, "layer_order", "gcr")) or (False, ACT_RELU, 0.0)
        self.post_norm, self.act, self.slope = spec
        self.mask = 1 if self.act == ACT_RELU else 0
        self.params = module_params(model)
        self._pids = [id(p) for p in self.params]
        self._first_param_owner, self._first_param_name = next(
            ((mod, name) for mod in model.modules() for name, p in mod._parameters.items() if p is self.params[0]), (None, None))
        self._pindex = _PIndex({id(p): i for i, p in enumerate(self.params)})
        self._build_layer_table(model)
        self._virtual_w = self._virtual_weights()
        self.images = self._weight_images()
        n_enc = sum(p.numel() for p in module_params(model.encoders))
        self.n_enc_params = n_enc
        self.enc_level_offs = [0]
        for enc in model.encoders:
            self.enc_level_offs.append(self.enc_level_offs[-1] + sum(p.numel() for p in module_params(enc)))
        assert self.enc_level_offs[-1] == n_enc
        self.n_params = sum(p.numel() for p in self.params)
        offs, o = [], 0
        for p in self.params:
            offs.append(o)
            o += p.numel()
        self.poffs = offs

    MIN_BUCKET_FLOATS = int(os.environ.get("U3D_MIN_BUCKET_MB", "1")) * (1 << 20) // 4

    def _sync_encoder_level(self, cx, flat, level: int, pending_hi: int) -> int:
        lo = self.enc_level_offs[level]
        if level > 0 and pending_hi - lo < self.MIN_BUCKET_FLOATS:
            return pending_hi
        if pending_hi > lo:
            cx.join()
            self.grad_sync.launch(flat[lo:pending_hi])
        return lo

    def _weight_images(self) -> WeightImages:
        ws = [mod.weight for mod in self.model.modules()
              if (isinstance(mod, torch.nn.Conv3d) and mod.kernel_size == (3, 3, 3))
              or (isinstance(mod, torch.nn.Conv2d) and mod.kernel_size == (3, 3))]
        if self.is2d:
            bf16 = {id(w) for w in ws if self._bf16_routed_weight(w.shape[1], w.shape[0], id(w) in self._virtual_w)}
            small = {id(w) for w in ws if self._small2d(w.shape[1], w.shape[0], id(w) in self._virtual_w)}
            c16 = {id(w) for w in ws if id(w) in bf16 and self._c16(w.shape[1], w.shape[0])}
            return WeightImages(each=[w for w in ws if id(w) not in bf16 | small], each_bf16=[w for w in ws if id(w) in bf16 - c16],
                                each_bf16_c16=[w for w in ws if id(w) in c16])
        bf16 = {id(w) for w in ws if self._bf16_layer(w.shape[1], w.shape[0])} - self._virtual_w
        return WeightImages(
            f32=[w for w in ws if id(w) not in bf16 and not (self.small_cin and w.shape[1] <= 4 and w.shape[0] <= 32)],
            bf16=[w for w in ws if id(w) in bf16], t8=self._t8_weights() if self.bf16 else ())

    def _t8_weights(self) -> list:
        return []
# ... 107 lines not shown
                _, Ds, Hs, Ws, _ = sk.shape
                tabs = [_resample_tables(dev, self.dec_interp[j], a, b) for a, b in ((D1, Ds), (H1, Hs), (W1, Ws))]
                up = _empty((Nl, Ds, Hs, Ws, Cl), dtype=_F32, device=dev)
                nat.call("u3d_resample2_fwd", dev.index, _stream(dev), _p(cur), _p(tabs[0][0]), _p(tabs[1][0]), _p(tabs[2][0]),
                         _p(tabs[0][1]), _p(tabs[1][1]), _p(tabs[2][1]), Nl, D1, H1, W1, Ds, Hs, Ws, Cl, _p(up))
                if tape is not None:
                    tape.ups.append(UpRec(cur, None, tabs, (Ds, Hs, Ws)))
                cur, cur_st = up, None
            src = VSrc(sk, cur)
            st_in = stats_of(src, sk_st, cur_st, pool, dev)
            if self._cat_bf16(c1):
                cat = _empty((src.N, src.D, src.H, src.W, src.C), dtype=_F32, device=dev)
                nat.call("u3d_nearest_cat_fwd", dev.index, _stream(dev), _p(sk), _p(cur), _p(src.maps[0]), _p(src.maps[1]), _p(src.maps[2]),
                         src.N, src.D, src.H, src.W, src.D1, src.H1, src.W1, src.C0, src.C1, _p(cat))
                if tape is not None:
                    tape.cats[j] = src
                y1, s1 = self._single_conv_fwd(c1, f"dec{j}.c1", VSrc(cat), st_in, pool, tape)
                del cat
            else:
                y1, s1 = self._single_conv_fwd(c1, f"dec{j}.c1", src, st_in, pool, tape, sub=sub)
            src2 = VSrc(y1)
            y2, s2 = self._single_conv_fwd(c2, f"dec{j}.c2", src2, stats_of(src2, s1, None, pool, dev), pool, tape)
            cur, cur_st = y2, s2

        fc = m.final_conv
        Co, Cf = fc.out_channels, fc.in_channels
        V = D * H * W
        logits = _empty((N, Co, D, H, W), dtype=_F32, device=dev)
        act = 0
        probs = None
        if m.final_activation is not None:
            act = 1 if isinstance(m.final_activation, torch.nn.Sigmoid) else 2
            probs = _empty_like(logits)
        nat.call("u3d_conv1x1_head_fwd", dev.index, _stream(dev), _p(cur), _p(fc.weight.detach()), _p(fc.bias.detach()), N, V,
                 Cf, Co, act, _p(logits), _p(probs))
        if tape is not None:
            tape.head_x = cur
            if self.debug is not None:
                self.debug["tape"] = tape
        if self.is2d:
            logits = logits.view(N, Co, H, W)
            probs = probs.view(N, Co, H, W) if probs is not None else None
        return logits, probs, tape

    def backward(self, tape: Tape, dlogits: torch.Tensor, need_input_grad: bool):
        m = self.model
        dev = dlogits.device
        N, Cin, D, H, W = tape.dims
        V = D * H * W
        dlogits = dlogits.contiguous()
        flat = _empty(self.n_params, dtype=_F32, device=dev)

        def gview(idx):
            p = self.params[idx]
            return flat[self.poffs[idx] : self.poffs[idx] + p.numel()]

        fc = m.final_conv
        Co, Cf = fc.out_channels, fc.in_channels
        tot = self.stat_reps * (Co * Cf + Co) + sum(self.stat_reps * N * r.src.C * 2 for r in tape.convs)
        pool = getattr(tape, "bwd_pool", None)
        tape.bwd_pool = None
        if (pool is None or pool.buf.numel() < tot or pool.buf.device != dev or torch.cuda.is_current_stream_capturing()
                or not pool.claim()):
            pool = _StatPool(dev, tot)
        ws = self._wgrad_workspace(tape, dev)

        hreps = self.stat_reps
        hacc = pool.take(hreps * (Co * Cf + Co))
        dz = _empty_like(tape.head_x)
        nat.call("u3d_conv1x1_head_bwd_reps", dev.index, _stream(dev), _p(dlogits), _p(tape.head_x), _p(fc.weight.detach()), N, V,
                 Cf, Co, self.mask, _p(dz), _p(hacc), hreps)
        self._unact(dev, dz, tape.head_x)
        iw, ib = self._pindex[id(fc.weight)], self._pindex[id(fc.bias)]
        assert self.poffs[ib] == self.poffs[iw] + Co * Cf
        nat.call("u3d_cvt_f64_f32_sum", dev.index, _stream(dev), _p(hacc), _p(gview(iw)), Co * Cf + Co, hreps)

        n_levels = len(self.enc)
        n_dec = len(self.dec)
        mk = self.mask
        skip_grad = {}

        cx = _BwdCtx(dev, pool, ws, flat, self)

        def conv_bwd(rec: ConvRec, dz_, need_dg=True):
            return self._conv_bwd(cx, rec, dz_, need_dg)

        def plain_apply(dg, coef, x, relu_mask):
            return self._plain_apply(cx, dg, coef, x, relu_mask)

        recs = tape.convs
        enc_recs = [(recs[2 * i], recs[2 * i + 1]) for i in range(n_levels)]
        dec_recs = [(recs[2 * n_levels + 2 * j], recs[2 * n_levels + 2 * j + 1]) for j in range(n_dec)]

        for j in range(n_dec - 1, -1, -1):
            r1, r2 = dec_recs[j]
            dg2, coef2, _ = conv_bwd(r2, dz)
            dz1 = plain_apply(dg2, coef2, r2.src.t0, mk)
            self._unact(dev, dz1, r2.src.t0)
            del dg2
            dg1, coef1, coef_hi = conv_bwd(r1, dz1)
            src = tape.cats.get(j, r1.src)
            C0, C1, Ct = src.C0, src.C1, src.C
            lvl = n_levels - 2 - j
            dzl = _empty_like(src.t1)
            if r1.sub is not None:
                dg0, dlow = dg1
                skip_grad[lvl] = (dg0, C0, coef1, Ct)
                if any(src.plus):
                    nat.call("u3d_gn_bwd_apply_children", dev.index, _stream(dev), _p(dlow), _p(src.t1), _p(coef1), Ct, C0, src.N, src.D1,
                             src.H1, src.W1, C1, *src.plus, mk, _p(dzl))
                else:
                    coef_up = coef_hi if coef_hi is not None else coef1[:, :, C0:] * self._up_scale(dev)
                    nat.call("u3d_gn_bwd_apply", dev.index, _stream(dev), _p(dlow), C1, 0, _p(src.t1), C1, _p(coef_up), C1,
                             src.D1 * src.H1 * src.W1, src.N, mk, _p(dzl))
                del dg0, dlow
            else:
                skip_grad[lvl] = (dg1, Ct, coef1, Ct)
                lz, ly, lx = src.los
                nat.call("u3d_gn_bwd_apply_up", dev.index, _stream(dev), _p(dg1), Ct, C0, _p(src.t1), C1, _p(coef1), Ct, src.N,
                         src.D, src.H, src.W, src.D1, src.H1, src.W1, _p(lz), _p(ly), _p(lx),
                         0 if (self.dec_up[j] is not None or self.dec_interp[j] is not None) else mk, _p(dzl))
            del dg1
            if self.dec_up[j] is not None:
                up = tape.ups[j]
                xl = up.x_low
                Nl, D1, H1, W1, Cl = xl.shape
                Cs = up.weight.shape[1]
                acc = pool.take(up.weight.numel())
                dxl = _empty_like(xl)
                nat.call("u3d_convtr3d_bwd", dev.index, _stream(dev), _p(dzl), _p(xl), _p(up.weight.detach()), Nl, D1, H1, W1, Cl, Cs,
                         mk, _p(dxl), _p(acc), _p(self.images.get(up.weight, Kind.CONVTR_DGRAD, dev)), flops=4.0 * 27 * Cl * Cs * Nl * D1 * H1 * W1)
                nat.call("u3d_cvt_f64_f32", dev.index, _stream(dev), _p(acc), _p(gview(self._pindex[id(up.weight)])),
                         up.weight.numel())
                self._unact(dev, dxl, xl)
                dzl = dxl
            elif self.dec_interp[j] is not None:
                up = tape.ups[j]
                xl = up.x_low
                Nl, D1, H1, W1, Cl = xl.shape
                Ds, Hs, Ws = up.tdims
                tz, ty, tx = up.los
                dxl = _empty_like(xl)
                nat.call("u3d_resample2_bwd", dev.index, _stream(dev), _p(dzl), _p(tz[2]), _p(ty[2]), _p(tx[2]), _p(tz[0]), _p(ty[0]),
                         _p(tx[0]), _p(tz[1]), _p(ty[1]), _p(tx[1]), Nl, D1, H1, W1, Ds, Hs, Ws, Cl, _p(dxl))
                if self.act != ACT_NONE:
                    nat.call("u3d_act_bwd", dev.index, _stream(dev), _p(dxl), _p(xl), dxl.numel(), self.act, self.slope, _p(dxl))
                dzl = dxl
            else:
                self._unact(dev, dzl, src.t1)
            dz = dzl

        if self.grad_sync is not None:
            cx.join()
            self.grad_sync.launch(flat[self.n_enc_params :])

        dx0 = None
        pending_hi = self.n_enc_params
        for i in range(n_levels - 1, -1, -1):
            r1, r2 = enc_recs[i]
            dg2, coef2, _ = conv_bwd(r2, dz)
            dz1 = plain_apply(dg2, coef2, r2.src.t0, mk)
            self._unact(dev, dz1, r2.src.t0)
            del dg2
            dg1, coef1, _ = conv_bwd(r1, dz1, need_dg=(i > 0 or need_input_grad))
            if self.grad_sync is not None:
                pending_hi = self._sync_encoder_level(cx, flat, i, pending_hi)
            if i > 0:
                pooled, argmax, e_in = tape.pools[i - 1]
                Ne, De, He, We, Ce = e_in.shape
                out = _empty_like(e_in)
                sk = skip_grad.pop(i - 1, None)
                pdims = (Ne, He, We, Ce) if self.is2d else (Ne, De, He, We, Ce)
                sfx = "2d" if self.is2d else "2"
                if sk is None:
                    nat.call(f"u3d_maxpool{sfx}_bwd_merge", dev.index, _stream(dev), _p(dg1), _p(pooled), _p(argmax), _p(coef1), None,
                             _p(e_in), *pdims, mk, _p(out))
                else:
                    sdg, sCdg, scoef, sCt = sk
                    nat.call(f"u3d_maxpool{sfx}_bwd_merge_gn", dev.index, _stream(dev), _p(dg1), _p(pooled), _p(argmax), _p(coef1),
                             _p(sdg), sCdg, _p(scoef), sCt, _p(e_in), *pdims, mk, _p(out))
                    del sk, sdg, scoef
                self._unact(dev, out, e_in)
                dz = out
            elif need_input_grad:
                dx0 = plain_apply(dg1, coef1, tape.x0, 0)
            del dg1

        cx.join()
        if self.grad_sync is not None:
            self.grad_sync.finish()

        dx = None
        if dx0 is not None:
            if Cin == 1:
                dx = dx0.view(N, 1, D, H, W)
            else:
                dx = _empty((N, Cin, D, H, W), dtype=_F32, device=dev)
                nat.call("u3d_ndhwc_to_ncdhw", dev.index, _stream(dev), _p(dx0), _p(dx), N, Cin, V)
            if self.is2d:
                dx = dx.view(N, Cin, H, W)
        return flat, dx
```

### pytorch-3dunet_amd/pytorch3dunet_amd/_native.py

```python
from __future__ import annotations

import ctypes
import os
import threading
from ctypes import POINTER, c_char_p, c_double, c_float, c_int, c_int32, c_int64, c_size_t, c_void_p

_HERE = os.path.dirname(os.path.abspath(__file__))
LIB_PATH = os.environ.get("U3D_LIB_PATH") or os.path.join(_HERE, "lib", "libu3d_hip.so")

U3D_OK = 0


class U3DSrc(ctypes.Structure):

    _fields_ = [
        ("p0", c_void_p),
        ("p1", c_void_p),
        ("zmap", c_void_p),
        ("ymap", c_void_p),
        ("xmap", c_void_p),
        ("affine", c_void_p),
        ("C0", c_int32),
        ("C1", c_int32),
        ("D1", c_int32),
        ("H1", c_int32),
        ("W1", c_int32),
    ]


class U3DAdamDesc(ctypes.Structure):

    _fields_ = [("p", c_void_p), ("g", c_void_p), ("m", c_void_p), ("v", c_void_p), ("first", c_int64), ("numel", c_int64)]


class U3DGnBwdJob(ctypes.Structure):

    _fields_ = [("gstats_lo", c_void_p), ("gstats_hi", c_void_p), ("mean_rstd", c_void_p), ("gamma", c_void_p), ("dgamma", c_void_p),
                ("dbeta", c_void_p), ("coef", c_void_p), ("coef_hi", c_void_p), ("count", ctypes.c_double), ("C0", c_int32),
                ("C1", c_int32), ("N", c_int32), ("G", c_int32), ("hi_scale", ctypes.c_float), ("reps_lo", c_int32), ("reps_hi", c_int32), ("reserved", c_int32)]


class U3DPackDesc(ctypes.Structure):

    _fields_ = [("w", c_void_p), ("packed", c_void_p), ("first", c_int64), ("Cout", c_int32), ("Cin", c_int32),
                ("mode", c_int32), ("cin_stride", c_int32)]


_PROTOS = {
    "u3d_version": (c_int, []),
    "u3d_debug_stream_pass": (c_int, [c_int, c_void_p, c_void_p, c_int64, c_int, c_int, c_double]),
    "u3d_debug_mfma_f32_rate": (c_int, [c_int, c_void_p, c_void_p, c_int, c_int, POINTER(c_double)]),
    "u3d_last_error": (c_char_p, []),
    "u3d_check_device": (c_int, [c_int]),
    "u3d_set_tuning": (c_int, [c_int, c_int]),
    "u3d_set_profile_buffer": (c_int, [c_void_p, c_size_t]),
    "u3d_packed_weight_floats": (c_size_t, [c_int, c_int, c_int]),
    "u3d_pack_weights": (c_int, [c_int, c_void_p, c_void_p, c_int, c_int, c_int, c_void_p]),
    "u3d_pack_weights_batch": (c_int, [c_int, c_void_p, c_void_p, c_int, c_int64]),
    "u3d_pack_weights_cells_blocks": (c_int64, [c_void_p, c_int, c_int, c_int, c_int]),
    "u3d_pack_weights_batch_cells": (c_int, [c_int, c_void_p, c_void_p, c_int, c_int64]),
    "u3d_conv3d": (
        c_int,
        [c_int, c_void_p, POINTER(U3DSrc), c_void_p, c_void_p, c_int, c_int, c_int, c_int, c_int, c_int, c_void_p,
         POINTER(U3DSrc), c_void_p],
    ),
    "u3d_wgrad_workspace_floats": (c_size_t, [c_int, c_int, c_int, c_int, c_int, c_int]),
    "u3d_conv3d_variant": (c_int, [c_int, c_int, c_int, c_int, c_int, c_int, c_int, c_int]),
    "u3d_conv3d_wgrad_variant": (c_int, [c_int, c_int, c_int, c_int, c_int, c_int, c_int]),
    "u3d_conv3d_wgrad": (
        c_int,
        [c_int, c_void_p, POINTER(U3DSrc), c_void_p, c_void_p, c_int, c_int, c_int, c_int, c_int, c_void_p, c_size_t],
    ),
    "u3d_conv3d_small_cin_fwd": (
        c_int,
        [c_int, c_void_p, c_void_p, c_void_p, c_void_p, c_void_p, c_int, c_int, c_int, c_int, c_int, c_int, c_int, c_void_p],
    ),
    "u3d_conv3d_small_cin_fwd_reps": (
        c_int,
        [c_int, c_void_p, c_void_p, c_void_p, c_void_p, c_void_p, c_int, c_int, c_int, c_int, c_int, c_int, c_int, c_void_p, c_int],
    ),
    "u3d_small_cin_bwd_workspace_floats": (c_size_t, [c_int, c_int, c_int, c_int, c_int, c_int]),
    "u3d_conv3d_small_cin_bwd": (
        c_int,
        [c_int, c_void_p, c_void_p, c_void_p, c_void_p, c_void_p, c_void_p, c_void_p, c_int, c_int, c_int, c_int, c_int,
         c_int, c_void_p, c_size_t],
    ),
    "u3d_conv3d_naive": (
        c_int,
        [c_int, c_void_p, POINTER(U3DSrc), c_void_p, c_void_p, c_int, c_int, c_int, c_int, c_int, c_int, c_int, c_int],
    ),
    "u3d_chan_stats": (c_int, [c_int, c_void_p, POINTER(U3DSrc), c_int, c_int, c_int, c_int, c_void_p]),
    "u3d_chan_stats_reps": (c_int, [c_int, c_void_p, POINTER(U3DSrc), c_int, c_int, c_int, c_int, c_void_p, c_int]),
    "u3d_gn_finalize": (
        c_int,
        [c_int, c_void_p, c_void_p, c_int, c_double, c_void_p, c_int, c_double, c_int, c_int, c_double, c_void_p,
         c_void_p, c_float, c_void_p, c_void_p],
    ),
    "u3d_gn_bwd_finalize": (
        c_int,
        [c_int, c_void_p, c_void_p, c_void_p, c_void_p, c_int, c_int, c_int, c_double, c_void_p, c_void_p, c_void_p],
    ),
    "u3d_gn_finalize_split": (
        c_int,
        [c_int, c_void_p, c_void_p, c_int, c_double, c_void_p, c_int, c_double, c_int, c_int, c_double, c_void_p,
         c_void_p, c_float, c_void_p, c_void_p, c_int, c_void_p, c_void_p],
    ),
    "u3d_gn_bwd_finalize_split_supported": (c_int, [c_int, c_int, c_int]),
    "u3d_chan_stats_children": (c_int, [c_int, c_void_p, c_void_p, c_int, c_int, c_int, c_int, c_int, c_int, c_int, c_int, c_void_p]),
    "u3d_adam_step": (c_int, [c_int, c_void_p, c_void_p, c_int, c_int64, c_double, c_double, c_double, c_double, c_double, c_int64]),
    "u3d_gn_bwd_finalize_split": (
        c_int,
        [c_int, c_void_p, c_void_p, c_int, c_void_p, c_int, c_void_p, c_void_p, c_int, c_int, c_double, c_void_p, c_void_p,
         c_void_p, c_float, c_void_p],
    ),
    "u3d_gn_bwd_apply": (
        c_int,
        [c_int, c_void_p, c_void_p, c_int, c_int, c_void_p, c_int, c_void_p, c_int, c_int64, c_int, c_int, c_void_p],
    ),
    "u3d_gn_bwd_apply_up": (
        c_int,
        [c_int, c_void_p, c_void_p, c_int, c_int, c_void_p, c_int, c_void_p, c_int, c_int, c_int, c_int, c_int, c_int,
         c_int, c_int, c_void_p, c_void_p, c_void_p, c_int, c_void_p],
    ),
    "u3d_maxpool2_fwd": (c_int, [c_int, c_void_p, c_void_p, c_int, c_int, c_int, c_int, c_int, c_void_p, c_void_p, c_void_p]),
    "u3d_maxpool2_bwd_merge": (
        c_int,
        [c_int, c_void_p, c_void_p, c_void_p, c_void_p, c_void_p, c_void_p, c_void_p, c_int, c_int, c_int, c_int, c_int,
         c_int, c_void_p],
    ),
    "u3d_maxpool2_bwd_merge_gn": (
        c_int,
        [c_int, c_void_p, c_void_p, c_void_p, c_void_p, c_void_p, c_void_p, c_int, c_void_p, c_int, c_void_p, c_int, c_int,
         c_int, c_int, c_int, c_int, c_void_p],
    ),
    "u3d_conv1x1_head_fwd": (
        c_int,
        [c_int, c_void_p, c_void_p, c_void_p, c_void_p, c_int, c_int64, c_int, c_int, c_int, c_void_p, c_void_p],
    ),
    "u3d_conv1x1_head_bwd": (
        c_int,
        [c_int, c_void_p, c_void_p, c_void_p, c_void_p, c_int, c_int64, c_int, c_int, c_int, c_void_p, c_void_p],
    ),
    "u3d_conv1x1_head_bwd_reps": (
        c_int,
        [c_int, c_void_p, c_void_p, c_void_p, c_void_p, c_int, c_int64, c_int, c_int, c_int, c_void_p, c_void_p, c_int],
    ),
    "u3d_conv3d_wgrad_strided": (
        c_int,
        [c_int, c_void_p, POINTER(U3DSrc), c_void_p, c_void_p, c_int, c_int, c_int, c_int, c_int, c_int, c_void_p, c_size_t],
    ),
    "u3d_conv3d_ex_reps": (
        c_int,
        [c_int, c_void_p, POINTER(U3DSrc), c_void_p, c_void_p, c_int, c_int, c_int, c_int, c_int, c_int, c_void_p, POINTER(U3DSrc),
         c_void_p, c_void_p, c_void_p, c_int64, c_int],
    ),
    "u3d_gn_finalize_reps": (
        c_int,
        [c_int, c_void_p, c_void_p, c_int, c_double, c_int, c_void_p, c_int, c_double, c_int, c_int, c_int, c_double, c_void_p, c_void_p,
         c_float, c_void_p, c_void_p, c_int, c_void_p, c_void_p],
    ),
    "u3d_conv3d_wgrad_job_supported": (c_int, [c_int, c_int, c_int]),
    "u3d_conv3d_wgrad_job": (
        c_int,
        [c_int, c_void_p, POINTER(U3DSrc), c_void_p, c_void_p, c_int, c_int, c_int, c_int, c_int, c_int, c_void_p, c_size_t,
         POINTER(U3DGnBwdJob)],
    ),
    "u3d_subpixel_wgrad_workspace_floats": (c_int64, [c_int, c_int, c_int, c_int, c_int, c_int]),
    "u3d_subpixel_conv_wgrad": (
        c_int,
        [c_int, c_void_p, c_void_p, c_void_p, c_int64, c_void_p, c_void_p, c_int, c_int, c_int, c_int, c_int, c_int, c_int,
         c_void_p, c_int64],
    ),
    "u3d_convtr3d_subpixel_packed_floats": (c_int64, [c_int, c_int]),
    "u3d_pack_convtr3d_subpixel": (c_int, [c_int, c_void_p, c_void_p, c_int, c_int, c_void_p]),
    "u3d_convtr3d_fwd_subpixel": (
        c_int, [c_int, c_void_p, c_void_p, c_void_p, c_void_p, c_int, c_int, c_int, c_int, c_int, c_int],
    ),
    "u3d_subpixel_packed_floats": (c_int64, [c_int, c_int]),
    "u3d_subpixel_dgrad_packed_floats": (c_int64, [c_int, c_int]),
    "u3d_pack_subpixel_dgrad_weights": (c_int, [c_int, c_void_p, c_void_p, c_int, c_int, c_int, c_int, c_void_p]),
    "u3d_subpixel_conv_dgrad": (
        c_int,
        [c_int, c_void_p, c_void_p, c_void_p, c_void_p, c_void_p, c_void_p, c_int, c_int, c_int, c_int, c_int, c_int],
    ),
    "u3d_subpixel_conv_dgrad_reps": (
        c_int,
        [c_int, c_void_p, c_void_p, c_void_p, c_void_p, c_void_p, c_void_p, c_int, c_int, c_int, c_int, c_int, c_int, c_int],
    ),
    "u3d_pack_subpixel_weights": (c_int, [c_int, c_void_p, c_void_p, c_int, c_int, c_int, c_int, c_void_p]),
    "u3d_subpixel_conv_fwd_win": (c_int, [c_int, c_void_p, c_void_p, c_void_p, c_int64, c_void_p, c_void_p, c_int, c_int, c_int, c_int,
                                          c_int, c_int, POINTER(c_int)]),
    "u3d_subpixel_conv_dgrad_win": (c_int, [c_int, c_void_p, c_void_p, c_void_p, c_void_p, c_void_p, c_void_p, c_int, c_int, c_int, c_int,
                                            c_int, c_int, POINTER(c_int)]),
    "u3d_subpixel_conv_wgrad_win": (c_int, [c_int, c_void_p, c_void_p, c_void_p, c_int64, c_void_p, c_void_p, c_int, c_int, c_int, c_int,
                                            c_int, c_int, c_int, c_void_p, c_int64, POINTER(c_int)]),
    "u3d_conv3d_box": (c_int, [c_int, c_void_p, POINTER(U3DSrc), c_void_p, c_void_p, c_int, c_int, c_int, c_int, c_int, POINTER(c_int),
                               POINTER(c_int)]),
    "u3d_conv3d_wgrad_box": (c_int, [c_int, c_void_p, POINTER(U3DSrc), c_void_p, c_void_p, c_int, c_int, c_int, c_int, c_int, c_void_p,
                                     c_size_t, POINTER(c_int)]),
    "u3d_gn_bwd_apply_children": (c_int, [c_int, c_void_p, c_void_p, c_void_p, c_void_p, c_int, c_int, c_int, c_int, c_int, c_int, c_int,
                                          c_int, c_int, c_int, c_int, c_void_p]),
    "u3d_nearest_childsum_add": (c_int, [c_int, c_void_p, c_void_p, c_void_p, c_void_p, c_void_p, c_int, c_int, c_int, c_int, c_int, c_int,
                                         c_int, c_int, c_void_p, c_void_p, c_void_p, c_int, c_int, c_int]),
    "u3d_subpixel_fwd_workspace_floats": (c_int64, [c_int, c_int, c_int, c_int, c_int, c_int]),
    "u3d_subpixel_conv_fwd": (
        c_int,
        [c_int, c_void_p, c_void_p, c_void_p, c_int64, c_void_p, c_void_p, c_int, c_int, c_int, c_int, c_int, c_int,
         c_void_p, c_int64],
    ),
    "u3d_conv3d_workspace_floats": (c_int64, [c_int, c_int, c_int, c_int, c_int, c_int]),
    "u3d_conv3d_ex": (
        c_int,
        [c_int, c_void_p, POINTER(U3DSrc), c_void_p, c_void_p, c_int, c_int, c_int, c_int, c_int, c_int, c_void_p,
         POINTER(U3DSrc), c_void_p, c_void_p, c_void_p, c_int64],
    ),
    "u3d_conv3d_residual": (
        c_int,
        [c_int, c_void_p, POINTER(U3DSrc), c_void_p, c_void_p, c_int, c_int, c_int, c_int, c_int, c_int, c_void_p, c_void_p],
    ),
    "u3d_gn_bwd_apply_add": (
        c_int,
        [c_int, c_void_p, c_void_p, c_int, c_int, c_void_p, c_int, c_void_p, c_int, c_int64, c_int, c_int, c_void_p, c_void_p],
    ),
    "u3d_conv1x1_fwd": (c_int, [c_int, c_void_p, c_void_p, c_void_p, c_void_p, c_void_p, c_int, c_int64, c_int, c_int, c_void_p]),
    "u3d_conv1x1_bwd": (c_int, [c_int, c_void_p, c_void_p, c_void_p, c_void_p, c_int, c_int64, c_int, c_int, c_void_p, c_void_p]),
    "u3d_pack_convtr_weights": (c_int, [c_int, c_void_p, c_void_p, c_int, c_int, c_int, c_void_p]),
    "u3d_convtr3d_fwd": (c_int, [c_int, c_void_p, c_void_p, c_void_p, c_void_p, c_int, c_int, c_int, c_int, c_int, c_int, c_void_p]),
    "u3d_convtr3d_bwd": (
        c_int,
        [c_int, c_void_p, c_void_p, c_void_p, c_void_p, c_int, c_int, c_int, c_int, c_int, c_int, c_int, c_void_p, c_void_p,
         c_void_p],
    ),
    "u3d_nearest_add_fwd": (
        c_int,
        [c_int, c_void_p, c_void_p, c_void_p, c_void_p, c_void_p, c_void_p, c_int, c_int, c_int, c_int, c_int, c_int, c_int,
         c_int, c_void_p, c_void_p],
    ),
    "u3d_nearest_sum_bwd": (
        c_int,
        [c_int, c_void_p, c_void_p, c_void_p, c_void_p, c_void_p, c_int, c_int, c_int, c_int, c_int, c_int, c_int, c_int,
         c_void_p],
    ),
    "u3d_se_gate_fwd": (
        c_int,
        [c_int, c_void_p, c_void_p, c_double, c_void_p, c_void_p, c_void_p, c_void_p, c_int, c_int, c_int, c_void_p, c_void_p,
         c_void_p],
    ),
    "u3d_se_apply_fwd": (
# ... 364 lines not shown
```

Before: 120.9.

## Fuse GroupNorm-backward apply into the weight-gradient kernel as a passenger workload

Adds an APPLY variant of the wgrad kernel that first computes the GroupNorm-backward finalize coefficients into LDS. It then streams the elementwise GN-backward apply (dg, x, coef to out), interleaved with the MFMA groups, and finishes any leftover portion after the main loop. The goal is to remove a separate memory-bound apply kernel launch by hiding its loads and stores under the compute-bound wgrad. In exchange the kernel needs more LDS (up to 160KB) and more registers, and the added global traffic can compete with the tile prefetch.

```diff
diff --git a/include/u3d.h b/include/u3d.h
--- a/include/u3d.h
+++ b/include/u3d.h
@@ -112,6 +112,21 @@
 int u3d_conv3d_wgrad_job(int device, u3d_stream_t stream, const u3d_src_t* src, const float* dz, float* dw, int dw_cin_stride,
                          int N, int D, int H, int W, int Cout, float* workspace, size_t workspace_floats,
                          const u3d_gn_bwd_job_t* job);
+
+typedef struct u3d_gn_apply_job {
+    const float* dg;
+    const float* x;
+    const float* coef;
+    const float* add;
+    float* out;
+    int64_t voxels_per_n;
+    int32_t Cdg, coff, Cx, Ctot, N, relu_mask;
+} u3d_gn_apply_job_t;
+int u3d_conv3d_wgrad_apply_supported(const u3d_src_t* src, const float* dz, int N, int D, int H, int W, int Cout,
+                                     const u3d_gn_bwd_job_t* job, const u3d_gn_apply_job_t* apply);
+int u3d_conv3d_wgrad_job_apply(int device, u3d_stream_t stream, const u3d_src_t* src, const float* dz, float* dw, int dw_cin_stride,
+                               int N, int D, int H, int W, int Cout, float* workspace, size_t workspace_floats,
+                               const u3d_gn_bwd_job_t* job, const u3d_gn_apply_job_t* apply);
 
 long long u3d_subpixel_wgrad_workspace_floats(int N, int D1, int H1, int W1, int C1, int Cout);
 int u3d_subpixel_conv_wgrad(int device, u3d_stream_t stream, const float* low, const float* affine,
diff --git a/pytorch-3dunet_amd/csrc/u3d_bf16.hip b/pytorch-3dunet_amd/csrc/u3d_bf16.hip
--- a/pytorch-3dunet_amd/csrc/u3d_bf16.hip
+++ b/pytorch-3dunet_amd/csrc/u3d_bf16.hip
@@ -26,7 +26,7 @@
     return __builtin_bit_cast(bf16x8, u32x4{o[0] & m, o[1] & m, o[2] & m, o[3] & m});
 }
 
-extern int g_u3d_tune[24];
+extern int g_u3d_tune[26];
 
 namespace {
 
diff --git a/pytorch-3dunet_amd/csrc/u3d_conv.hip b/pytorch-3dunet_amd/csrc/u3d_conv.hip
--- a/pytorch-3dunet_amd/csrc/u3d_conv.hip
+++ b/pytorch-3dunet_amd/csrc/u3d_conv.hip
@@ -5,7 +5,7 @@
 #include "u3d_gn.h"
 #include "u3d_subpix.h"
 
-int g_u3d_tune[24] = {0};
+int g_u3d_tune[26] = {0};
 
 namespace cv {
 constexpr int TZ = 4, TY = 8, TX = 8;
@@ -1130,7 +1130,22 @@
 constexpr int NIT_G = (NITEMS_G + NTHR - 1) / NTHR;
 constexpr int NIT_DZ = TV * 8 / NTHR;
 constexpr int MAX_MAP_INTS = 4096;
-}
+constexpr int APPLY_LDS_BYTES = 160 * 1024;
+}
+
+struct WgradApply {
+    const float *dg, *x, *add;
+    const float* coefsrc;
+    float* out;
+    long long total;
+    long long vq;
+    unsigned per;
+    unsigned dg_step;
+    int lq;
+    int Cdg, coff, Ctot, N, relu_mask;
+    int npt;
+    int tab_hi, tab_floats;
+};
 
 struct WgradParams {
     u3d_src_t src;
@@ -1141,11 +1156,14 @@
     int tz, ty, tx, ntiles, tps;
     int vec, dzvec;
     int bz0, by0, bx0, bz1, by1, bx1;
+    u3d_gn_bwd_job_t job;
+    WgradApply ap;
 };
 
-template <bool VEC, bool REG = false, bool PAIR = false>
+template <bool VEC, bool REG = false, bool PAIR = false, bool APPLY = false>
 __global__ __launch_bounds__(512, 2) void conv3d_wgrad_kernel(const WgradParams p) {
     using namespace wg;
+    static_assert(!APPLY || (VEC && REG), "the passenger rides in the constant-offset variants only");
     constexpr int NA = PAIR ? 4 : 7;
     extern __shared__ __attribute__((aligned(16))) float lds[];
     int* zmapl = reinterpret_cast<int*>(lds + 2 * BUF_FLOATS);
@@ -1388,8 +1406,72 @@
     static_assert(2 * (NPF - 1) < ST0 && ST0 + NPF <= 32, "prefetch schedule must fit the 32 groups of a tile");
     const int tile_begin = s * p.tps, tile_end = min(p.ntiles, (s + 1) * p.tps);
 
+    const float* ctab = lds + 2 * BUF_FLOATS + ((p.D + p.H + p.W + 3) & ~3);
+    unsigned ap_cnt = 0, ap_k = 0;
+    unsigned aloc = t, dgo = 0;
+    unsigned ap_b1 = ~0u, ap_b2 = ~0u, ap_b3 = ~0u;
+    const char *ap_x = nullptr, *ap_dg = nullptr, *ap_add = nullptr;
+    char* ap_out = nullptr;
+    int ap_cofs = 0;
+    if constexpr (APPLY) {
+        const long long start = (long long)logical * p.ap.per;
+        const long long left = p.ap.total - start;
+        ap_cnt = left <= 0 ? 0u : (left < (long long)p.ap.per ? (unsigned)left : p.ap.per);
+        const long long s0 = ap_cnt ? start : 0;
+        ap_x = reinterpret_cast<const char*>(p.ap.x + s0 * 4);
+        ap_out = reinterpret_cast<char*>(p.ap.out + s0 * 4);
+        ap_add = p.ap.add ? reinterpret_cast<const char*>(p.ap.add + s0 * 4) : nullptr;
+        ap_dg = reinterpret_cast<const char*>(p.ap.dg + (s0 >> p.ap.lq) * p.ap.Cdg + p.ap.coff);
+        const int qd = t & ((1 << p.ap.lq) - 1);
+        dgo = (unsigned)(((t >> p.ap.lq) * p.ap.Cdg + 4 * qd) * 4);
+        ap_cofs = p.ap.coff + 4 * qd;
+        const long long n0 = s0 / p.ap.vq;
+        ctab += n0 * 3 * p.ap.Ctot;
+        auto bound = [&](long long n) {
+            const long long b = n * p.ap.vq - s0;
+            return (n >= p.ap.N || b > 0xffffffffll) ? ~0u : (unsigned)b;
+        };
+        ap_b1 = bound(n0 + 1), ap_b2 = bound(n0 + 2), ap_b3 = bound(n0 + 3);
+    }
+    auto ap_load = [&](const char* base, unsigned off, unsigned loc) {
+        return *reinterpret_cast<const f32x4*>(base + (loc < ap_cnt ? off : 0u));
+    };
+    auto ap_finish = [&](const f32x4& d, const f32x4& xv, const f32x4& av, bool has_add, unsigned loc) {
+        const int n = (loc >= ap_b1 ? 1 : 0) + (loc >= ap_b2 ? 1 : 0) + (loc >= ap_b3 ? 1 : 0);
+        const float* cp = ctab + n * (3 * p.ap.Ctot) + ap_cofs;
+        const f32x4 cp_ = *reinterpret_cast<const f32x4*>(cp);
+        const f32x4 cq_ = *reinterpret_cast<const f32x4*>(cp + p.ap.Ctot);
+        const f32x4 cr_ = *reinterpret_cast<const f32x4*>(cp + 2 * p.ap.Ctot);
+        const f32x4 o = u3d_gn_bwd_apply_quad(cp_, cq_, cr_, d, xv, av, has_add, p.ap.relu_mask);
+        if (loc < ap_cnt) *reinterpret_cast<f32x4*>(ap_out + loc * 16u) = o;
+    };
+
     TileIdx tix = tile_decode(tile_begin);
-    if (tile_begin < tile_end) {
+    if constexpr (APPLY) {
+        const bool have = tile_begin < tile_end;
+        const TileC c = tile_coords(tix);
+        f32x4 ga, gb;
+        f32x4 v[NIT_G + NIT_DZ];
+        if (have) {
+            load_affine(c.n, ga, gb);
+#pragma unroll
+            for (int k = 0; k < NIT_G + NIT_DZ; ++k) v[k] = pf_load(c, k);
+        }
+        float* tab = lds + 2 * BUF_FLOATS + ((p.D + p.H + p.W + 3) & ~3);
+        if (p.ap.coefsrc) {
+            for (int k = t; k < p.ap.tab_floats; k += NTHR) tab[k] = p.ap.coefsrc[k];
+        } else {
+            const u3d_gn_bwd_job_t& job = p.job;
+            u3d_gn_bwd_finalize_body(job.gstats_lo, job.mean_rstd, job.gamma, job.N, job.C0 + job.C1, job.G, job.count, 1, 1, job.dgamma,
+                                     job.dbeta, job.coef, job.gstats_hi, job.C0, job.hi_scale, job.coef_hi,
+                                     reinterpret_cast<double*>(lds + BUF_FLOATS), job.reps_lo, job.reps_hi, logical == 0 ? 1 : 0, tab,
+                                     p.ap.tab_hi);
+        }
+        if (have) {
+#pragma unroll
+            for (int k = 0; k < NIT_G + NIT_DZ; ++k) pf_store(lds, c, k, v[k], ga, gb);
+        }
+    } else if (tile_begin < tile_end) {
         const TileC c = tile_coords(tix);
         if constexpr (VEC) {
             f32x4 ga, gb;
@@ -1436,8 +1518,24 @@
         bop[0] = gl[bbase];
 #pragma unroll
         for (int k = 0; k < NA; ++k) aop[0][k] = gl[abase[k]];
+        const int ap_n = APPLY && ap_k < ap_cnt ? p.ap.npt : 0;
+        const f32x4 zero4 = {0.f, 0.f, 0.f, 0.f};
+        f32x4 pd[2] = {zero4, zero4}, px[2] = {zero4, zero4};
 #pragma unroll
         for (int g = 0; g < 32; ++g) {
+            if constexpr (APPLY) {
+                if (g == 1 && ap_n >= 1) pd[0] = ap_load(ap_dg, dgo, aloc);
+                if (g == 3 && ap_n >= 1) px[0] = ap_load(ap_x, aloc * 16u, aloc);
+                if (g == 5 && ap_n >= 2) pd[1] = ap_load(ap_dg, dgo + p.ap.dg_step, aloc + NTHR);
+                if (g == 7 && ap_n >= 2) px[1] = ap_load(ap_x, (aloc + NTHR) * 16u, aloc + NTHR);
+                if (g == 29 && ap_n >= 1) ap_finish(pd[0], px[0], zero4, false, aloc);
+                if (g == 30 && ap_n >= 2) ap_finish(pd[1], px[1], zero4, false, aloc + NTHR);
+                if (g == 31) {
+                    aloc += NTHR * ap_n;
+                    dgo += p.ap.dg_step * ap_n;
+                    ap_k += NTHR * ap_n;
+                }
+            }
             if constexpr (VEC) {
                 if (g % 2 == 0 && g / 2 < NPF) v[g / 2] = pf_load(cn, g / 2);
                 if (g >= ST0 && g - ST0 < NPF) pf_store(nbuf, cn, g - ST0, v[g - ST0], gan, gbn);
@@ -1462,6 +1560,24 @@
     }
 
     __builtin_amdgcn_s_setprio(3);
+    if constexpr (APPLY) {
+        while (ap_k < ap_cnt) {
+            f32x4 d[4], xv[4], av[4];
+#pragma unroll
+            for (int u = 0; u < 4; ++u) {
+                const unsigned loc = aloc + NTHR * u;
+                d[u] = ap_load(ap_dg, dgo + p.ap.dg_step * u, loc);
+                xv[u] = ap_load(ap_x, loc * 16u, loc);
+                av[u] = f32x4{0.f, 0.f, 0.f, 0.f};
+                if (ap_add) av[u] = ap_load(ap_add, loc * 16u, loc);
+            }
+#pragma unroll
+            for (int u = 0; u < 4; ++u) ap_finish(d[u], xv[u], av[u], ap_add != nullptr, aloc + NTHR * u);
+            aloc += 4 * NTHR;
+            dgo += 4 * p.ap.dg_step;
+            ap_k += 4 * NTHR;
+        }
+    }
     float* red = lds;
     if (hf == 1) {
 #pragma unroll
@@ -1885,7 +2001,7 @@
 }
 
 extern "C" int u3d_set_tuning(int key, int value) {
-    if (key < 0 || key >= 24) return u3d_set_err(U3D_EINVAL, "u3d_set_tuning: key out of range");
+    if (key < 0 || key >= 26) return u3d_set_err(U3D_EINVAL, "u3d_set_tuning: key out of range");
     g_u3d_tune[key] = value;
     return 0;
 }
@@ -2342,6 +2458,10 @@
                                 hipFuncAttributeMaxDynamicSharedMemorySize, (wg::LDS_FLOATS + wg::MAX_MAP_INTS) * sizeof(float)));
     U3D_HIP(hipFuncSetAttribute(reinterpret_cast<const void*>(conv3d_wgrad_kernel<true, true, true>),
                                 hipFuncAttributeMaxDynamicSharedMemorySize, (wg::LDS_FLOATS + wg::MAX_MAP_INTS) * sizeof(float)));
+    U3D_HIP(hipFuncSetAttribute(reinterpret_cast<const void*>(conv3d_wgrad_kernel<true, true, false, true>),
+                                hipFuncAttributeMaxDynamicSharedMemorySize, wg::APPLY_LDS_BYTES));
+    U3D_HIP(hipFuncSetAttribute(reinterpret_cast<const void*>(conv3d_wgrad_kernel<true, true, true, true>),
+                                hipFuncAttributeMaxDynamicSharedMemorySize, wg::APPLY_LDS_BYTES));
     U3D_HIP(hipFuncSetAttribute(reinterpret_cast<const void*>(conv3d_wgrad_kernel<true>),
                                 hipFuncAttributeMaxDynamicSharedMemorySize, (wg::LDS_FLOATS + wg::MAX_MAP_INTS) * sizeof(float)));
     U3D_HIP(hipFuncSetAttribute(reinterpret_cast<const void*>(conv3d_wgrad_kernel<false>),
@@ -2352,7 +2472,7 @@
 
 static int conv3d_wgrad_impl(int device, u3d_stream_t stream, const u3d_src_t* src, const float* dz, float* dw, int cstride,
                              int N, int D, int H, int W, int Cout, float* workspace, size_t workspace_floats, const int* box = nullptr,
-                             const u3d_gn_bwd_job_t* job = nullptr);
+                             const u3d_gn_bwd_job_t* job = nullptr, const u3d_gn_apply_job_t* apply = nullptr);
 
 extern "C" int u3d_conv3d_wgrad_box(int device, u3d_stream_t stream, const u3d_src_t* src, const float* dz, float* dw, int N, int D,
                                     int H, int W, int Cout, float* workspace, size_t workspace_floats, const int* box) {
@@ -2378,9 +2498,56 @@
     return (N > 0 && C > 0 && G > 0 && C % G == 0 && wgrad_job_lds_bytes(N, C, G) + 1024 <= 64 * 1024) ? 1 : 0;
 }
 
-extern "C" int u3d_conv3d_wgrad_job(int device, u3d_stream_t stream, const u3d_src_t* src, const float* dz, float* dw,
-                                    int dw_cin_stride, int N, int D, int H, int W, int Cout, float* workspace,
-                                    size_t workspace_floats, const u3d_gn_bwd_job_t* job) {
+static bool wgrad_is_reg(const u3d_src_t* src, int D, int H, int W) {
+    return (g_u3d_tune[3] != 2 || (D % wg::TZ == 0 && H % wg::TY == 0 && W % wg::TX == 0)) &&
+           (src->C1 == 0 || (D == 2 * src->D1 && H == 2 * src->H1 && W == 2 * src->W1));
+}
+
+static bool wgrad_apply_ok(const u3d_src_t* src, const float* dz, int N, int D, int H, int W, int Cout, const u3d_gn_bwd_job_t* job,
+                           const u3d_gn_apply_job_t* a, const char** why) {
+    const char* dummy;
+    if (!why) why = &dummy;
+    *why = "bad argument";
+    if (!src || !dz || !job || !a || N <= 0 || D <= 0 || H <= 0 || W <= 0 || Cout <= 0) return false;
+    if (!a->dg || !a->x || !a->coef || !a->out || a->Cdg <= 0 || a->Cx <= 0 || a->coff < 0 || a->coff + a->Cx > a->Cdg ||
+        a->Ctot < a->coff + a->Cx || a->voxels_per_n <= 0 || a->N <= 0)
+        return false;
+    *why = "the weight gradient does not run the constant-offset 16-byte variant";
+    if (!src_vec_ok(src) || Cout % 4 != 0 || ((uintptr_t)dz & 15) != 0 || !wgrad_is_reg(src, D, H, W)) return false;
+    if (D + H + W > wg::MAX_MAP_INTS) return false;
+    *why = "the apply is not the 16-byte form with a power-of-two quad count per voxel (<= 512) and N <= 4";
+    if (a->Cdg % 4 || a->Cx % 4 || a->coff % 4 || a->Ctot % 4) return false;
+    if ((((uintptr_t)a->dg | (uintptr_t)a->x | (uintptr_t)a->out | (uintptr_t)a->add | (uintptr_t)a->coef) & 15) != 0) return false;
+    const int Q = a->Cx / 4;
+    if ((Q & (Q - 1)) != 0 || Q > 512 || a->N > 4) return false;
+    *why = "apply->coef is neither the job's coef nor its coef_hi (with matching N and channel count)";
+    const int C1 = job->gstats_hi ? job->C1 : 0;
+    const bool lo = a->coef == job->coef && a->Ctot == job->C0 + C1;
+    const bool hi = job->coef_hi && C1 > 0 && a->coef == job->coef_hi && a->Ctot == C1;
+    if (a->N != job->N || !(lo || hi)) return false;
+    *why = "the job's tables do not fit the LDS beside the staging buffers";
+    if (u3d_conv3d_wgrad_job_supported(job->N, job->C0 + C1, job->G) != 1) return false;
+    const size_t lds = (wg::LDS_FLOATS + (size_t)((D + H + W + 3) & ~3) + 3 * (size_t)a->N * a->Ctot) * sizeof(float);
+    if (lds > (size_t)wg::APPLY_LDS_BYTES) return false;
+    return true;
+}
+
+static long long wgrad_apply_per(long long total, long long nblk) { return ((total + nblk - 1) / nblk + 511) / 512 * 512; }
+static bool wgrad_apply_per_ok(long long per, const u3d_gn_apply_job_t* a) {
+    return (per + 4 * 512) * 4ll * (a->Cdg > a->Cx ? a->Cdg : a->Cx) < (1ll << 32);
+}
+
+extern "C" int u3d_conv3d_wgrad_apply_supported(const u3d_src_t* src, const float* dz, int N, int D, int H, int W, int Cout,
+                                                const u3d_gn_bwd_job_t* job, const u3d_gn_apply_job_t* apply) {
+    if (g_u3d_tune[24] == 1) return 0;
+    if (!wgrad_apply_ok(src, dz, N, D, H, W, Cout, job, apply, nullptr)) return 0;
+    WgradParams p;
+    wgrad_plan(N, D, H, W, src->C0 + src->C1, Cout, p);
+    const long long total = (long long)apply->N * apply->voxels_per_n * (apply->Cx / 4);
+    return wgrad_apply_per_ok(wgrad_apply_per(total, (long long)p.S * p.nchunks * p.nkb), apply) ? 1 : 0;
+}
+
+static int wgrad_job_check(const u3d_src_t* src, int dw_cin_stride, const u3d_gn_bwd_job_t* job) {
     U3D_REQUIRE(src && (dw_cin_stride == 0 || dw_cin_stride >= src->C0 + src->C1), "u3d_conv3d_wgrad_job: dw_cin_stride < channels of src");
     if (job) {
         U3D_REQUIRE(job->gstats_lo && job->mean_rstd && job->gamma && job->dgamma && job->dbeta && job->coef && job->C0 > 0 &&
@@ -2391,12 +2558,37 @@
                     "u3d_conv3d_wgrad_job: the reduction of %d x %d channels in %d groups does not fit one block's LDS", job->N,
                     job->C0 + job->C1, job->G);
     }
+    return 0;
+}
+
+extern "C" int u3d_conv3d_wgrad_job(int device, u3d_stream_t stream, const u3d_src_t* src, const float* dz, float* dw,
+                                    int dw_cin_stride, int N, int D, int H, int W, int Cout, float* workspace,
+                                    size_t workspace_floats, const u3d_gn_bwd_job_t* job) {
+    if (int e = wgrad_job_check(src, dw_cin_stride, job)) return e;
     return conv3d_wgrad_impl(device, stream, src, dz, dw, dw_cin_stride, N, D, H, W, Cout, workspace, workspace_floats, nullptr, job);
+}
+
+extern "C" int u3d_conv3d_wgrad_job_apply(int device, u3d_stream_t stream, const u3d_src_t* src, const float* dz, float* dw,
+                                          int dw_cin_stride, int N, int D, int H, int W, int Cout, float* workspace,
+                                          size_t workspace_floats, const u3d_gn_bwd_job_t* job, const u3d_gn_apply_job_t* apply) {
+    if (int e = wgrad_job_check(src, dw_cin_stride, job)) return e;
+    if (apply) {
+        const char* why = nullptr;
+        U3D_REQUIRE(wgrad_apply_ok(src, dz, N, D, H, W, Cout, job, apply, &why), "u3d_conv3d_wgrad_job_apply: %s", why);
+    }
+    return conv3d_wgrad_impl(device, stream, src, dz, dw, dw_cin_stride, N, D, H, W, Cout, workspace, workspace_floats, nullptr, job,
+                             apply);
+}
+
+__global__ __launch_bounds__(256) void wgrad_gn_job_kernel(u3d_gn_bwd_job_t job) {
+    extern __shared__ double shb[];
+    u3d_gn_bwd_finalize_body(job.gstats_lo, job.mean_rstd, job.gamma, job.N, job.C0 + job.C1, job.G, job.count, 1, 1, job.dgamma, job.dbeta,
+                             job.coef, job.gstats_hi, job.C0, job.hi_scale, job.coef_hi, shb, job.reps_lo, job.reps_hi);
 }
 
 static int conv3d_wgrad_impl(int device, u3d_stream_t stream, const u3d_src_t* src, const float* dz, float* dw, int cstride,
                              int N, int D, int H, int W, int Cout, float* workspace, size_t workspace_floats, const int* box,
-                             const u3d_gn_bwd_job_t* job) {
+                             const u3d_gn_bwd_job_t* job, const u3d_gn_apply_job_t* apply) {
     U3D_ENTER(device);
     if (int e = check_src(src, "u3d_conv3d_wgrad")) return e;
     U3D_REQUIRE(dz && dw && workspace && N > 0 && D > 0 && H > 0 && W > 0 && Cout > 0, "u3d_conv3d_wgrad: bad argument");
@@ -2422,10 +2614,51 @@
     if (int e = wgrad_set_lds_once(device)) return e;
     const int nblk = p.S * p.nchunks * p.nkb;
     U3D_REQUIRE(D + H + W <= wg::MAX_MAP_INTS, "u3d_conv3d_wgrad: D+H+W must be <= %d", wg::MAX_MAP_INTS);
-    const size_t shmem = (wg::LDS_FLOATS + (size_t)(D + H + W)) * sizeof(float);
-    const bool reg = !box && (g_u3d_tune[3] != 2 || (D % wg::TZ == 0 && H % wg::TY == 0 && W % wg::TX == 0)) &&
-                     (src->C1 == 0 || (D == 2 * src->D1 && H == 2 * src->H1 && W == 2 * src->W1));
-    if (p.vec && p.dzvec && reg && Cin <= 16)
+    size_t shmem = (wg::LDS_FLOATS + (size_t)(D + H + W)) * sizeof(float);
+    const bool reg = !box && wgrad_is_reg(src, D, H, W);
+    u3d_gn_bwd_job_t jb = {};
+    size_t job_lds = 0;
+    if (job) {
+        jb = *job;
+        if (!jb.gstats_hi) jb.C1 = 0, jb.hi_scale = 1.0f, jb.coef_hi = nullptr;
+        if (jb.reps_lo < 1) jb.reps_lo = 1;
+        if (jb.reps_hi < 1 || !jb.gstats_hi) jb.reps_hi = 1;
+        job_lds = wgrad_job_lds_bytes(jb.N, jb.C0 + jb.C1, jb.G);
+    }
+    p.job = jb;
+    p.ap = WgradApply{};
+    if (apply) {
+        U3D_REQUIRE(p.vec && p.dzvec && reg && job, "u3d_conv3d_wgrad_job_apply: not the constant-offset variant");
+        WgradApply& a = p.ap;
+        const int Q = apply->Cx / 4;
+        a.dg = apply->dg, a.x = apply->x, a.add = apply->add, a.out = apply->out;
+        a.vq = (long long)apply->voxels_per_n * Q;
+        a.total = a.vq * apply->N;
+        const long long per = wgrad_apply_per(a.total, nblk);
+        U3D_REQUIRE(wgrad_apply_per_ok(per, apply),
+                    "u3d_conv3d_wgrad_job_apply: the apply's tensors are too large for 32-bit offsets inside a block's range");
+        a.per = (unsigned)per;
+        a.lq = 0;
+        while ((1 << a.lq) < Q) ++a.lq;
+        a.dg_step = (unsigned)((512 >> a.lq) * apply->Cdg * 4);
+        a.Cdg = apply->Cdg, a.coff = apply->coff, a.Ctot = apply->Ctot, a.N = apply->N, a.relu_mask = apply->relu_mask;
+        a.npt = apply->add ? 0 : (Cout <= 32 ? 2 : 1);
+        a.tab_hi = (jb.coef_hi && apply->coef == jb.coef_hi) ? 1 : 0;
+        a.tab_floats = 3 * apply->N * apply->Ctot;
+        a.coefsrc = nullptr;
+        if (g_u3d_tune[25] == 1) {
+            hipLaunchKernelGGL(wgrad_gn_job_kernel, dim3(1), dim3(256), job_lds, (hipStream_t)stream, jb);
+            U3D_LAUNCH_CHECK();
+            a.coefsrc = apply->coef;
+        }
+        shmem = (wg::LDS_FLOATS + (size_t)((D + H + W + 3) & ~3) + (size_t)a.tab_floats) * sizeof(float);
+        job = nullptr;
+    }
+    if (apply && Cin <= 16)
+        hipLaunchKernelGGL((conv3d_wgrad_kernel<true, true, true, true>), dim3(nblk), dim3(wg::NTHR), shmem, (hipStream_t)stream, p);
+    else if (apply)
+        hipLaunchKernelGGL((conv3d_wgrad_kernel<true, true, false, true>), dim3(nblk), dim3(wg::NTHR), shmem, (hipStream_t)stream, p);
+    else if (p.vec && p.dzvec && reg && Cin <= 16)
         hipLaunchKernelGGL((conv3d_wgrad_kernel<true, true, true>), dim3(nblk), dim3(wg::NTHR), shmem, (hipStream_t)stream, p);
     else if (p.vec && p.dzvec && reg)
         hipLaunchKernelGGL((conv3d_wgrad_kernel<true, true>), dim3(nblk), dim3(wg::NTHR), shmem, (hipStream_t)stream, p);
@@ -2437,15 +2670,7 @@
     const long long total = (long long)Cin * 27 * Cout;
     const bool one_group = p.S <= 16 && g_u3d_tune[23] != 1;
     const int rblocks = (int)((total + (one_group ? 255 : 63)) / (one_group ? 256 : 64));
-    u3d_gn_bwd_job_t jb = {};
-    size_t job_lds = 0;
-    if (job) {
-        jb = *job;
-        if (!jb.gstats_hi) jb.C1 = 0, jb.hi_scale = 1.0f, jb.coef_hi = nullptr;
-        if (jb.reps_lo < 1) jb.reps_lo = 1;
-        if (jb.reps_hi < 1 || !jb.gstats_hi) jb.reps_hi = 1;
-        job_lds = wgrad_job_lds_bytes(jb.N, jb.C0 + jb.C1, jb.G);
-    }
+    if (!job) job_lds = 0;
     if (one_group)
         hipLaunchKernelGGL(wgrad_reduce_kernel<1>, dim3(rblocks + (job ? 1 : 0)), dim3(256), job_lds, (hipStream_t)stream, workspace, dw, p.S,
                            p.nchunks, p.nkb, Cin, Cout, cstride > 0 ? cstride : Cin, job ? 1 : 0, jb);
diff --git a/pytorch-3dunet_amd/csrc/u3d_gn.h b/pytorch-3dunet_amd/csrc/u3d_gn.h
--- a/pytorch-3dunet_amd/csrc/u3d_gn.h
+++ b/pytorch-3dunet_amd/csrc/u3d_gn.h
@@ -1,5 +1,19 @@
 #pragma once
 #include "u3d_common.h"
+
+__device__ __forceinline__ f32x4 u3d_gn_bwd_apply_quad(const f32x4& p, const f32x4& q, const f32x4& r, const f32x4& d, const f32x4& x,
+                                                       const f32x4& add, bool has_add, int relu_mask) {
+#pragma clang fp contract(off)
+    f32x4 o;
+#pragma unroll
+    for (int e = 0; e < 4; ++e) {
+        const float t = q[e] * x[e];
+        float v = __builtin_fmaf(p[e], d[e], t) + r[e];
+        if (has_add) v = v + add[e];
+        o[e] = (relu_mask && !(x[e] > 0.f)) ? 0.f : v;
+    }
+    return o;
+}
 
 __device__ __forceinline__ double u3d_sum_replicas(const double* __restrict__ p, size_t stride, int reps) {
     double v = p[0];
@@ -17,7 +31,8 @@
                                                 const float* __restrict__ gamma, int N, int C, int G, double count, int staged, int par,
                                                 float* __restrict__ dgamma, float* __restrict__ dbeta, float* __restrict__ coef,
                                                 const double* __restrict__ gs_hi, int C0, float hi_scale, float* __restrict__ coef_hi,
-                                                double* shb, int reps = 1, int reps_hi = 1) {
+                                                double* shb, int reps = 1, int reps_hi = 1, int write_global = 1,
+                                                float* tab = nullptr, int tab_hi = 0) {
 
 #pragma clang fp contract(off)
     const double* src = gs;
@@ -84,17 +99,30 @@
             const int n = i / C, c = i - n * C, pair = n * G + c / cpg;
             const double rstd = (double)mean_rstd[(size_t)pair * 2 + 1];
             const float fp = (float)(rstd * (double)gamma[c]), fq = (float)qr[(size_t)pair * 2], fr = (float)qr[(size_t)pair * 2 + 1];
-            coef[((size_t)n * 3 + 0) * C + c] = fp;
-            coef[((size_t)n * 3 + 1) * C + c] = fq;
-            coef[((size_t)n * 3 + 2) * C + c] = fr;
-            if (coef_hi && c >= C0) {
-                const int C1 = C - C0;
-                coef_hi[((size_t)n * 3 + 0) * C1 + (c - C0)] = fp;
-                coef_hi[((size_t)n * 3 + 1) * C1 + (c - C0)] = fq * hi_scale;
-                coef_hi[((size_t)n * 3 + 2) * C1 + (c - C0)] = fr * hi_scale;
+            const int C1 = C - C0;
+            const float fqh = fq * hi_scale, frh = fr * hi_scale;
+            if (write_global) {
+                coef[((size_t)n * 3 + 0) * C + c] = fp;
+                coef[((size_t)n * 3 + 1) * C + c] = fq;
+                coef[((size_t)n * 3 + 2) * C + c] = fr;
+                if (coef_hi && c >= C0) {
+                    coef_hi[((size_t)n * 3 + 0) * C1 + (c - C0)] = fp;
+                    coef_hi[((size_t)n * 3 + 1) * C1 + (c - C0)] = fqh;
+                    coef_hi[((size_t)n * 3 + 2) * C1 + (c - C0)] = frh;
+                }
+            }
+            if (tab && !tab_hi) {
+                tab[(n * 3 + 0) * C + c] = fp;
+                tab[(n * 3 + 1) * C + c] = fq;
+                tab[(n * 3 + 2) * C + c] = fr;
+            } else if (tab && c >= C0) {
+                tab[(n * 3 + 0) * C1 + (c - C0)] = fp;
+                tab[(n * 3 + 1) * C1 + (c - C0)] = fqh;
+                tab[(n * 3 + 2) * C1 + (c - C0)] = frh;
             }
         }
     }
+    if (!write_global) return;
     for (int c = threadIdx.x; c < C; c += blockDim.x) {
         const int g = c / cpg;
         double dg = 0.0, db = 0.0;
diff --git a/pytorch-3dunet_amd/csrc/u3d_ops.hip b/pytorch-3dunet_amd/csrc/u3d_ops.hip
--- a/pytorch-3dunet_amd/csrc/u3d_ops.hip
+++ b/pytorch-3dunet_amd/csrc/u3d_ops.hip
@@ -3,7 +3,7 @@
 
 #include <string.h>
 
-extern int g_u3d_tune[24];
+extern int g_u3d_tune[26];
 
 static thread_local char g_err[512] = "";
 
@@ -494,13 +494,9 @@
             const f32x4 p = *reinterpret_cast<const f32x4*>(coef + ((size_t)n * 3 + 0) * Ctot + coff + c);
             const f32x4 q = *reinterpret_cast<const f32x4*>(coef + ((size_t)n * 3 + 1) * Ctot + coff + c);
             const f32x4 r = *reinterpret_cast<const f32x4*>(coef + ((size_t)n * 3 + 2) * Ctot + coff + c);
-            f32x4 o = p * d + q * xv + r;
-            if (add) o += u3d_ldq(add + (size_t)v * Cx + c);
-            if (relu_mask) {
-#pragma unroll
-                for (int e = 0; e < 4; ++e) o[e] = xv[e] > 0.f ? o[e] : 0.f;
-            }
-            u3d_stq(out + (size_t)v * Cx + c, o);
+            f32x4 av = {0.f, 0.f, 0.f, 0.f};
+            if (add) av = u3d_ldq(add + (size_t)v * Cx + c);
+            u3d_stq(out + (size_t)v * Cx + c, u3d_gn_bwd_apply_quad(p, q, r, d, xv, av, add != nullptr, relu_mask));
         }
     } else {
         const long long total = (long long)N * Vn * Cx;
diff --git a/pytorch-3dunet_amd/csrc/u3d_smallc.hip b/pytorch-3dunet_amd/csrc/u3d_smallc.hip
--- a/pytorch-3dunet_amd/csrc/u3d_smallc.hip
+++ b/pytorch-3dunet_amd/csrc/u3d_smallc.hip
@@ -1,6 +1,6 @@
 #include "u3d_common.h"
 
-extern int g_u3d_tune[24];
+extern int g_u3d_tune[26];
 
 typedef float f32x4s __attribute__((ext_vector_type(4)));
 
diff --git a/pytorch-3dunet_amd/csrc/u3d_subpix.hip b/pytorch-3dunet_amd/csrc/u3d_subpix.hip
--- a/pytorch-3dunet_amd/csrc/u3d_subpix.hip
+++ b/pytorch-3dunet_amd/csrc/u3d_subpix.hip
@@ -1,6 +1,6 @@
 #include "u3d_subpix.h"
 
-extern int g_u3d_tune[24];
+extern int g_u3d_tune[26];
 
 
 struct SubpixParams {
diff --git a/pytorch-3dunet_amd/pytorch3dunet_amd/_engine_conv.py b/pytorch-3dunet_amd/pytorch3dunet_amd/_engine_conv.py
--- a/pytorch-3dunet_amd/pytorch3dunet_amd/_engine_conv.py
+++ b/pytorch-3dunet_amd/pytorch3dunet_amd/_engine_conv.py
@@ -68,10 +68,22 @@
     b16: bool
     job: object = None
     greps: int = 1
+    apply: "ApplyReq" = None
 
     @property
     def flops(self):
         return 54.0 * self.src.C * self.Cout * self.N * self.D * self.H * self.W
+
+
+APPLY_MIN_NUMEL = (1 << 21, 1 << 23)
+
+
+class ApplyReq:
+    __slots__ = ("x", "relu_mask", "add", "low", "dg", "coef", "out")
+
+    def __init__(self, x, relu_mask, add=None, low=False):
+        self.x, self.relu_mask, self.add, self.low = x, relu_mask, add, low
+        self.dg = self.coef = self.out = None
 
 
 class ConvLayers:
@@ -569,9 +581,15 @@
                      flops=128.0 * C1 * c.Cout * c.N * src.D1 * src.H1 * src.W1)
         a0 = rec.affine_lo if rec.affine_lo is not None else rec.affine[:, :C0].contiguous()
         s0 = VSrc(src.t0).struct(a0)
-        nat.call("u3d_conv3d_wgrad_job", dev.index, _stream(dev), ctypes.byref(s0), _p(c.dz), _p(dwv), Ct, c.N, c.D, c.H, c.W,
-                 c.Cout, _p(ws), ws.numel(), ctypes.byref(c.job) if c.job is not None else None,
-                 flops=54.0 * C0 * c.Cout * c.N * c.D * c.H * c.W)
+        desc, out = self._apply_desc(c, s0)
+        if desc is not None:
+            nat.call("u3d_conv3d_wgrad_job_apply", dev.index, _stream(dev), ctypes.byref(s0), _p(c.dz), _p(dwv), Ct, c.N, c.D, c.H, c.W,
+                     c.Cout, _p(ws), ws.numel(), ctypes.byref(c.job), ctypes.byref(desc), flops=54.0 * C0 * c.Cout * c.N * c.D * c.H * c.W)
+            c.apply.out = out
+        else:
+            nat.call("u3d_conv3d_wgrad_job", dev.index, _stream(dev), ctypes.byref(s0), _p(c.dz), _p(dwv), Ct, c.N, c.D, c.H, c.W,
+                     c.Cout, _p(ws), ws.numel(), ctypes.byref(c.job) if c.job is not None else None,
+                     flops=54.0 * C0 * c.Cout * c.N * c.D * c.H * c.W)
         c.job = None
 
     def _wgrad_fp32_side(self, c: "_BwdCall"):
@@ -589,9 +607,33 @@
     def _wgrad_fp32(self, c: "_BwdCall"):
         cx, dev, src, rec, ws = c.cx, c.cx.dev, c.src, c.rec, c.cx.ws
         s_aff = src.struct(rec.affine)
-        nat.call("u3d_conv3d_wgrad_job", dev.index, _stream(dev), ctypes.byref(s_aff), _p(c.dz), _p(cx.gview(rec.idx_w)), 0, c.N, c.D,
-                 c.H, c.W, c.Cout, _p(ws), ws.numel(), ctypes.byref(c.job) if c.job is not None else None, flops=c.flops)
+        desc, out = self._apply_desc(c, s_aff)
+        if desc is not None:
+            nat.call("u3d_conv3d_wgrad_job_apply", dev.index, _stream(dev), ctypes.byref(s_aff), _p(c.dz), _p(cx.gview(rec.idx_w)), 0, c.N,
+                     c.D, c.H, c.W, c.Cout, _p(ws), ws.numel(), ctypes.byref(c.job), ctypes.byref(desc), flops=c.flops)
+            c.apply.out = out
+        else:
+            nat.call("u3d_conv3d_wgrad_job", dev.index, _stream(dev), ctypes.byref(s_aff), _p(c.dz), _p(cx.gview(rec.idx_w)), 0, c.N, c.D,
+                     c.H, c.W, c.Cout, _p(ws), ws.numel(), ctypes.byref(c.job) if c.job is not None else None, flops=c.flops)
         c.job = None
+
+    def _apply_desc(self, c: "_BwdCall", s):
+        a = c.apply
+        if a is None or c.job is None or a.x.dtype != _F32 or not self._apply_rides(c, a):
+            return None, None
+        Nn, Cx = a.x.shape[0], a.x.shape[-1]
+        out = _empty_like(a.x)
+        d = nat.U3DGnApplyJob()
+        d.dg, d.x, d.coef, d.add, d.out = _p(a.dg), _p(a.x), _p(a.coef), _p(a.add), _p(out)
+        d.voxels_per_n, d.N, d.relu_mask = a.x.numel() // (Nn * Cx), Nn, a.relu_mask
+        d.Cdg, d.coff, d.Cx, d.Ctot = a.dg.shape[-1], 0, Cx, a.coef.shape[-1]
+        if nat.get_lib().u3d_conv3d_wgrad_apply_supported(ctypes.byref(s), _p(c.dz), c.N, c.D, c.H, c.W, c.Cout, ctypes.byref(c.job),
+                                                         ctypes.byref(d)) != 1:
+            return None, None
+        return d, out
+
+    def _apply_rides(self, c: "_BwdCall", a: ApplyReq) -> bool:
+        return a.x.numel() >= APPLY_MIN_NUMEL[1 if a.low else 0]
 
     def _dgrad_subpixel(self, c: "_BwdCall"):
         cx, dev, src, rec, ws, pool = c.cx, c.cx.dev, c.src, c.rec, c.cx.ws, c.cx.pool
@@ -710,7 +752,7 @@
                  ctypes.byref(s_x), _p(gst.t), None, _p(ws), ws.numel(), gst.reps, flops=c.flops)
         return dg, (gst, None)
 
-    def _conv_bwd(self, cx, rec: ConvRec, dz_, need_dg=True):
+    def _conv_bwd(self, cx, rec: ConvRec, dz_, need_dg=True, apply: ApplyReq = None):
         dev, pool, ws, gview = cx.dev, cx.pool, cx.ws, cx.gview
         src = rec.src
         Nn, Dd, Hh, Ww = src.N, src.D, src.H, src.W
@@ -767,6 +809,12 @@
             coef = _empty((Nn, 3, src.C), dtype=_F32, device=dev)
             call.job, coef_hi = self._norm_bwd_job(cx, rec, gst, float(Dd * Hh * Ww), coef)
         had_job = call.job is not None
+        if apply is not None and had_job:
+            fam = self._wgrad_family(call)
+            if fam == "fp32" and not apply.low:
+                apply.dg, apply.coef, call.apply = dg, coef, apply
+            elif fam == "subpixel" and apply.low and coef_hi is not None:
+                apply.dg, apply.coef, call.apply = dg[1], coef_hi, apply
         getattr(self, self._WGRAD_KERNELS[self._wgrad_family(call)])(call)
         if not rec.pre_norm:
             return dg, self._identity_coef(Nn, src.C, dev), None
diff --git a/pytorch-3dunet_amd/pytorch3dunet_amd/_engine_unet.py b/pytorch-3dunet_amd/pytorch3dunet_amd/_engine_unet.py
--- a/pytorch-3dunet_amd/pytorch3dunet_amd/_engine_unet.py
+++ b/pytorch-3dunet_amd/pytorch3dunet_amd/_engine_unet.py
@@ -15,7 +15,7 @@
 from ._native import U3DSrc
 
 from ._engine_base import *
-from ._engine_conv import ConvLayers
+from ._engine_conv import ApplyReq, ConvLayers
 from ._engine_weights import Kind, WeightImages
 
 
@@ -289,8 +289,15 @@
 
         cx = _BwdCtx(dev, pool, ws, flat, self)
 
-        def conv_bwd(rec: ConvRec, dz_, need_dg=True):
-            return self._conv_bwd(cx, rec, dz_, need_dg)
+        def conv_bwd(rec: ConvRec, dz_, need_dg=True, apply=None):
+            return self._conv_bwd(cx, rec, dz_, need_dg, apply)
+
+        def inner_bwd(r2: ConvRec, dz_):
+            req = ApplyReq(r2.src.t0, mk)
+            dg2, coef2, _ = conv_bwd(r2, dz_, apply=req)
+            dz1 = req.out if req.out is not None else plain_apply(dg2, coef2, r2.src.t0, mk)
+            self._unact(dev, dz1, r2.src.t0)
+            return dz1
 
         def plain_apply(dg, coef, x, relu_mask):
             return self._plain_apply(cx, dg, coef, x, relu_mask)
@@ -301,19 +308,19 @@
 
         for j in range(n_dec - 1, -1, -1):
             r1, r2 = dec_recs[j]
-            dg2, coef2, _ = conv_bwd(r2, dz)
-            dz1 = plain_apply(dg2, coef2, r2.src.t0, mk)
-            self._unact(dev, dz1, r2.src.t0)
-            del dg2
-            dg1, coef1, coef_hi = conv_bwd(r1, dz1)
+            dz1 = inner_bwd(r2, dz)
+            low = ApplyReq(r1.src.t1, mk, low=True) if (r1.sub is not None and not any(r1.src.plus)) else None
+            dg1, coef1, coef_hi = conv_bwd(r1, dz1, apply=low)
             src = tape.cats.get(j, r1.src)
             C0, C1, Ct = src.C0, src.C1, src.C
             lvl = n_levels - 2 - j
-            dzl = _empty_like(src.t1)
+            dzl = low.out if (low is not None and low.out is not None) else _empty_like(src.t1)
             if r1.sub is not None:
                 dg0, dlow = dg1
                 skip_grad[lvl] = (dg0, C0, coef1, Ct)
-                if any(src.plus):
+                if low is not None and low.out is not None:
+                    pass
+                elif any(src.plus):
                     nat.call("u3d_gn_bwd_apply_children", dev.index, _stream(dev), _p(dlow), _p(src.t1), _p(coef1), Ct, C0, src.N, src.D1,
                              src.H1, src.W1, C1, *src.plus, mk, _p(dzl))
                 else:
@@ -365,10 +372,7 @@
         pending_hi = self.n_enc_params
         for i in range(n_levels - 1, -1, -1):
             r1, r2 = enc_recs[i]
-            dg2, coef2, _ = conv_bwd(r2, dz)
-            dz1 = plain_apply(dg2, coef2, r2.src.t0, mk)
-            self._unact(dev, dz1, r2.src.t0)
-            del dg2
+            dz1 = inner_bwd(r2, dz)
             dg1, coef1, _ = conv_bwd(r1, dz1, need_dg=(i > 0 or need_input_grad))
             if self.grad_sync is not None:
                 pending_hi = self._sync_encoder_level(cx, flat, i, pending_hi)
diff --git a/pytorch-3dunet_amd/pytorch3dunet_amd/_native.py b/pytorch-3dunet_amd/pytorch3dunet_amd/_native.py
--- a/pytorch-3dunet_amd/pytorch3dunet_amd/_native.py
+++ b/pytorch-3dunet_amd/pytorch3dunet_amd/_native.py
@@ -38,6 +38,12 @@
     _fields_ = [("gstats_lo", c_void_p), ("gstats_hi", c_void_p), ("mean_rstd", c_void_p), ("gamma", c_void_p), ("dgamma", c_void_p),
                 ("dbeta", c_void_p), ("coef", c_void_p), ("coef_hi", c_void_p), ("count", ctypes.c_double), ("C0", c_int32),
                 ("C1", c_int32), ("N", c_int32), ("G", c_int32), ("hi_scale", ctypes.c_float), ("reps_lo", c_int32), ("reps_hi", c_int32), ("reserved", c_int32)]
+
+
+class U3DGnApplyJob(ctypes.Structure):
+
+    _fields_ = [("dg", c_void_p), ("x", c_void_p), ("coef", c_void_p), ("add", c_void_p), ("out", c_void_p), ("voxels_per_n", c_int64),
+                ("Cdg", c_int32), ("coff", c_int32), ("Cx", c_int32), ("Ctot", c_int32), ("N", c_int32), ("relu_mask", c_int32)]
 
 
 class U3DPackDesc(ctypes.Structure):
@@ -164,6 +170,13 @@
         c_int,
         [c_int, c_void_p, POINTER(U3DSrc), c_void_p, c_void_p, c_int, c_int, c_int, c_int, c_int, c_int, c_void_p, c_size_t,
          POINTER(U3DGnBwdJob)],
+    ),
+    "u3d_conv3d_wgrad_apply_supported": (
+        c_int, [POINTER(U3DSrc), c_void_p, c_int, c_int, c_int, c_int, c_int, POINTER(U3DGnBwdJob), POINTER(U3DGnApplyJob)]),
+    "u3d_conv3d_wgrad_job_apply": (
+        c_int,
+        [c_int, c_void_p, POINTER(U3DSrc), c_void_p, c_void_p, c_int, c_int, c_int, c_int, c_int, c_int, c_void_p, c_size_t,
+         POINTER(U3DGnBwdJob), POINTER(U3DGnApplyJob)],
     ),
     "u3d_subpixel_wgrad_workspace_floats": (c_int64, [c_int, c_int, c_int, c_int, c_int, c_int]),
     "u3d_subpixel_conv_wgrad": (
```

Result: no change. 122.0 (median of 6 runs) (+1.0%).
